# TUI-NICR/nicr-multitask-scene-analysis

Hardware: AMD Instinct MI355X
Metric: Mpix/s panoptic merge+metrics, 640x480xB (higher is better)
Workload: dtype f32; 1 GPU; configs[1]: center-NMS + offset grouping + panoptic merge + mIoU/PQ accumulators (configs[3]); batch_per_gpu=32, global_batch=32, classes=40, height=480, width=640, centers_per_image=24, batches_in_flight=2, parallelism=dp1 (images sharded, accumulators all-reduced once per run, timed)

## Files before the change

include/nmsa.h:

```cpp
#ifndef NMSA_H
#define NMSA_H

#include <stddef.h>
#include <stdint.h>

#ifdef __cplusplus
extern "C" {
#endif

typedef void* nmsa_stream_t;

enum {
    NMSA_OK = 0,
    NMSA_ERR_ARG = -1,
    NMSA_ERR_LAUNCH = -2,
    NMSA_ERR_WORKSPACE = -3,
    NMSA_ERR_UNSUPPORTED = -4
};

enum { NMSA_F32 = 0, NMSA_BF16 = 1, NMSA_F16 = 2 };
enum { NMSA_U8 = 0, NMSA_I16 = 1, NMSA_I32 = 2, NMSA_I64 = 3 };
#define NMSA_ELEM_F32 8

#define NMSA_MAX_INSTANCE_IDS 256

int nmsa_version(void);
const char* nmsa_strerror(int code);
int nmsa_last_hip_error(void);
int nmsa_device_geometry(int* cus_host, int* xcds_host, size_t* lds_per_cu_host);

size_t nmsa_center_nms_workspace_bytes(int B, int H, int W);
int nmsa_center_nms_topk(const float* center, const uint8_t* fg,
                         int B, int H, int W,
                         float threshold, int ksize, int topk, int apply_fg,
                         int max_centers,
                         int32_t* centers_yx, int32_t* n_centers, float* scores,
                         uint8_t* center_mask,
                         void* workspace, size_t workspace_bytes,
                         nmsa_stream_t stream);

int nmsa_group_offsets(const float* offset, const uint8_t* fg,
                       const int32_t* centers_yx, const int32_t* n_centers,
                       int B, int H, int W, int max_centers,
                       float scale_y, float scale_x,
                       int use_dist_thr, float dist_thr,
                       uint8_t* inst, int32_t* area,
                       nmsa_stream_t stream);

int nmsa_semantic_argmax(const void* logits, int logits_dtype,
                         int B, int C, int H, int W,
                         uint8_t* idx_u8, int64_t* idx_i64, float* score,
                         nmsa_stream_t stream);

int nmsa_semantic_softmax(const void* logits, int logits_dtype,
                          int B, int C, int H, int W, float* probs,
                          nmsa_stream_t stream);

int nmsa_panoptic_fused(const void* logits, int logits_dtype, const float* offset,
                        const int32_t* centers_yx, const int32_t* n_centers,
                        const uint8_t* is_thing,
                        int B, int C, int H, int W, int max_centers,
                        float scale_y, float scale_x,
                        int use_dist_thr, float dist_thr,
                        uint8_t* sem_u8, uint8_t* inst, uint8_t* fg_out, float* score,
                        uint32_t* votes, int votes_are_zero, int vote_rows_hint,
                        nmsa_stream_t stream);

int nmsa_panoptic_assign(uint32_t* votes, int B, int n_vote_classes, int clear_votes,
                         int64_t max_instances_per_category, int64_t void_label,
                         int64_t* pan_of_inst, int32_t* area,
                         int64_t* ids_pan, int64_t* ids_ins, int32_t* n_ids,
                         nmsa_stream_t stream);

int nmsa_panoptic_paint(const uint8_t* sem_u8, const uint8_t* inst,
                        const int64_t* pan_of_inst, const uint8_t* is_thing,
                        int B, int C, int H, int W,
                        int64_t max_instances_per_category, int64_t void_label,
                        int64_t* pan, int64_t* pan_sem,
                        nmsa_stream_t stream);

int nmsa_panoptic_merge(const void* sem, int sem_dtype, const void* ins, int ins_dtype,
                        const uint8_t* thing_seg, const uint8_t* is_thing_class,
                        int B, int n_classes, int H, int W,
                        int64_t max_instances_per_category, int64_t void_label,
                        uint32_t* votes, int64_t* pan_of_inst,
                        int64_t* pan, int64_t* ids_pan, int64_t* ids_ins, int32_t* n_ids,
                        nmsa_stream_t stream);

size_t nmsa_panoptic_merge_wide_workspace_bytes(int B, int n_classes, int max_segments);
int nmsa_panoptic_merge_wide(const void* sem, int sem_dtype, const void* ins, int ins_dtype,
                             const uint8_t* thing_seg, const uint8_t* is_thing_class,
                             int B, int n_classes, int H, int W,
                             int64_t max_instances_per_category, int64_t void_label,
                             int max_segments,
                             int64_t* pan, int64_t* ids_pan, int64_t* ids_ins, int32_t* n_ids,
                             int32_t* status, void* workspace, size_t workspace_bytes,
                             nmsa_stream_t stream);

int nmsa_resize_nearest(const void* src, int elem_type, int planes, int Hs, int Ws,
                        int y0, int x0, int h, int w, int Ho, int Wo, void* dst,
                        nmsa_stream_t stream);
int nmsa_resize_bilinear(const void* src, int dtype, int planes, int Hs, int Ws,
                         int y0, int x0, int h, int w, int Ho, int Wo, void* dst,
                         nmsa_stream_t stream);

int nmsa_semantic_argmax_resized(const void* logits, int logits_dtype, int B, int C,
                                 int Hs, int Ws, int y0, int x0, int h, int w, int Ho, int Wo,
                                 uint8_t* idx_u8, int64_t* idx_i64, float* score,
                                 nmsa_stream_t stream);

size_t nmsa_panoptic_scores_workspace_bytes(int B);
int nmsa_panoptic_scores(const void* logits, int logits_dtype,
                         const uint8_t* sem_idx, const float* sem_prob,
                         const uint8_t* inst, const int64_t* pan,
                         const int64_t* pan_of_inst, const float* inst_score_tab,
                         int B, int C, int H, int W, int64_t max_instances_per_category,
                         float* out_semantic_score, float* out_instance_score,
                         float* out_panoptic_score, float* mean_semantic_score,
                         void* workspace, size_t workspace_bytes, nmsa_stream_t stream);

int nmsa_instance_orientation(const float* orientation, const uint8_t* inst,
                              const uint8_t* mask, int B, int H, int W,
                              double* sums, int32_t* count, nmsa_stream_t stream);
int nmsa_instance_orientation_wide(const float* orientation, const void* instance, int ins_dtype,
                                   const uint8_t* mask, int B, int H, int W, int max_instances,
                                   int32_t* ids, int32_t* n_ids, double* sums, int32_t* count,
                                   int32_t* status, void* workspace, size_t workspace_bytes,
                                   nmsa_stream_t stream);

#define NMSA_TG_ROUTE_SCAN 1
#define NMSA_TG_ROUTE_FAST_LOADERS 2
#define NMSA_TG_ROUTE_PAINT_TILED 4
#define NMSA_TG_ROUTE_PAINT_VECTOR 8
#define NMSA_TG_ROUTE_LUT_LDS 16
#define NMSA_TG_ROUTE_SCAN_16 32
size_t nmsa_targets_workspace_bytes(int B, int n_classes, int max_instances);
int nmsa_targets_route(const void* semantic, int sem_dtype, const void* instance, int ins_dtype,
                       int n_classes, int H, int W, int sigma, int max_instances,
                       const float* center, const void* offset, const uint8_t* foreground,
                       const uint8_t* center_mask, const void* workspace);
int nmsa_instance_clear_stuff(const void* semantic, int sem_dtype, void* instance, int ins_dtype,
                              const uint8_t* is_stuff_class, int n_classes, int64_t n_px,
                              nmsa_stream_t stream);
int nmsa_instance_targets(const void* semantic, int sem_dtype, const void* instance, int ins_dtype,
                          const uint8_t* is_thing_class, const uint8_t* is_stuff_class,
                          int B, int n_classes, int H, int W,
                          int sigma, const float* gauss_lut, int normalized_offset, int max_instances,
                          float* center, void* offset, uint8_t* foreground, uint8_t* center_mask,
                          int32_t* encoded_ids, int32_t* n_encoded,
                          int32_t* skipped_ids, int32_t* n_skipped,
                          int32_t* status, void* workspace, size_t workspace_bytes, int workspace_is_clean,
                          nmsa_stream_t stream);
int nmsa_panoptic_targets(const void* semantic, int sem_dtype, const void* instance, int ins_dtype,
                          const uint8_t* is_thing_class, int B, int n_classes, int H, int W,
                          int64_t max_instances_per_category, int64_t void_label,
                          int max_instances, int max_segments,
                          int64_t* panoptic, int64_t* ids_pan, int64_t* ids_ins, int32_t* n_ids,
                          int32_t* status, void* workspace, size_t workspace_bytes, int workspace_is_clean,
                          nmsa_stream_t stream);
int nmsa_orientation_targets(const void* semantic, int sem_dtype, const void* instance, int ins_dtype,
                             const uint8_t* estimate_class, const int32_t* keys, const int32_t* n_keys,
                             const float* biternion, int B, int n_classes, int H, int W, int K,
                             int max_instances,
                             float* orientation, uint8_t* foreground, uint8_t* present,
                             int32_t* status, void* workspace, size_t workspace_bytes, int workspace_is_clean,
                             nmsa_stream_t stream);
int nmsa_dve_targets(const int64_t* panoptic, const int64_t* keys, const int32_t* n_keys,
                     const float* embeddings, const float* image_embedding, float diff_factor,
                     int B, int K, int D, int H, int W,
                     float* lut, int32_t* indices, nmsa_stream_t stream);

#define NMSA_ST_TABLE_OVERFLOW 1
#define NMSA_ST_CATEGORY_RANGE 2
#define NMSA_ST_MISSING_KEY 4
#define NMSA_ST_VALUE_RANGE 8
#define NMSA_ST_SENTINEL_KEY 16
size_t nmsa_confmat_workspace_bytes(int n_classes);
int nmsa_confmat_update(const void* preds, int pred_dtype, int64_t pred_div,
                        const void* target, int target_dtype,
                        int64_t n_px, int n_classes, int mode,
                        int64_t* confmat, int32_t* status,
                        void* workspace, size_t workspace_bytes, nmsa_stream_t stream);

size_t nmsa_pq_workspace_bytes(int B, int H, int W, int num_categories);
int nmsa_pq_update(const int64_t* pred, const int64_t* target, int B, int H, int W,
                   int num_categories, int64_t ignored_label,
                   int64_t max_instances_per_category, int64_t offset,
                   int64_t void_segment_id,
                   double* iou_per_class, double* tp_per_class,
                   double* fn_per_class, double* fp_per_class,
                   int64_t* matches, int match_capacity, int32_t* n_matches,
                   int32_t* status, void* workspace, size_t workspace_bytes,
                   int workspace_is_clean, nmsa_stream_t stream);

int nmsa_pack_tables(const int32_t* n_centers, const int32_t* n_ids,
                     const int32_t* centers_yx, const float* scores,
                     const int32_t* area, const int64_t* ids_pan, const int64_t* ids_ins,
                     int B, int max_centers, int columns, double* out, nmsa_stream_t stream);

size_t nmsa_pq_confmat_workspace_bytes(int B, int H, int W, int n_classes);
int nmsa_pq_update_with_confmat(
    const int64_t* pred, const int64_t* target, const uint8_t* target_semantic,
    int B, int H, int W,
    int num_categories, int64_t ignored_label, int64_t max_instances_per_category, int64_t offset,
    int64_t void_segment_id,
    double* iou_per_class, double* tp_per_class, double* fn_per_class, double* fp_per_class,
    int64_t* matches, int match_capacity, int32_t* n_matches,
    int32_t* status, void* workspace, size_t workspace_bytes, int workspace_is_clean,
    int confmat_classes, int64_t pred_div, int64_t* confmat, int32_t* confmat_status,
    void* confmat_workspace, size_t confmat_workspace_bytes, nmsa_stream_t stream);
int nmsa_pq_update_with_confmat_parts(
    const uint8_t* pred_semantic, const uint8_t* pred_instance, const int64_t* pan_of_inst,
    const uint8_t* is_thing_class, int n_sem_classes, int64_t void_label,
    const int64_t* target, const uint8_t* target_semantic,
    int B, int H, int W,
    int num_categories, int64_t ignored_label, int64_t max_instances_per_category, int64_t offset,
    int64_t void_segment_id,
    double* iou_per_class, double* tp_per_class, double* fn_per_class, double* fp_per_class,
    int32_t* status, void* workspace, size_t workspace_bytes, int workspace_is_clean,
    int confmat_classes, int64_t pred_div, int64_t* confmat, int32_t* confmat_status,
    void* confmat_workspace, size_t confmat_workspace_bytes, nmsa_stream_t stream);

size_t nmsa_loss_workspace_bytes(int B, int H, int W);
int nmsa_loss_ce_fwd(const void* logits, int dtype, const uint8_t* target, const float* weights,
                     int B, int C, int H, int W, float label_smoothing,
                     double* loss_sum, int64_t* n_elements, double* weight_sum, float* lse2_out,
                     int32_t* status, void* workspace, size_t workspace_bytes, nmsa_stream_t stream);
int nmsa_loss_ce_bwd(const void* logits, int dtype, const uint8_t* target, const float* weights,
                     int B, int C, int H, int W, float label_smoothing,
                     const float* grad_scale, const float* lse2, void* grad_logits,
                     nmsa_stream_t stream);
int nmsa_loss_ce_fwd_i16(const void* logits, int dtype, const int16_t* target,
                         const float* weights, int B, int C, int H, int W,
                         float label_smoothing,
                         double* loss_sum, int64_t* n_elements, double* weight_sum,
                         float* lse2_out,
                         int32_t* status, void* workspace, size_t workspace_bytes,
                         nmsa_stream_t stream);
int nmsa_loss_ce_bwd_i16(const void* logits, int dtype, const int16_t* target,
                         const float* weights, int B, int C, int H, int W,
                         float label_smoothing, const float* grad_scale, const float* lse2,
                         void* grad_logits, nmsa_stream_t stream);
int nmsa_loss_ce_fwd_grad_supported(int dtype, int C);
int nmsa_loss_ce_fwd_grad(const void* logits, int dtype, const uint8_t* target, const float* weights,
                          int B, int C, int H, int W, float label_smoothing,
                          const float* expected_grad_scale,
                          double* loss_sum, int64_t* n_elements, double* weight_sum,
                          void* grad_logits, int32_t* status,
                          void* workspace, size_t workspace_bytes, nmsa_stream_t stream);
int nmsa_loss_ce_bwd_unless(const void* logits, int dtype, const uint8_t* target,
                            const float* weights, int B, int C, int H, int W,
                            float label_smoothing, const float* grad_scale, void* grad_logits,
                            const float* computed_for, int32_t* counters, nmsa_stream_t stream);
size_t nmsa_count_workspace_bytes(void);
int nmsa_count_u8(const uint8_t* values, int64_t n, int lo, int hi, int64_t* count,
                  float* mean_scale, float weight,
                  void* workspace, size_t workspace_bytes, nmsa_stream_t stream);
int nmsa_loss_masked_fwd(const void* pred, int dtype, const float* target, const uint8_t* mask,
                         int B, int C, int H, int W, int kind,
                         double* loss_sum, int64_t* n_mask,
                         void* workspace, size_t workspace_bytes, nmsa_stream_t stream);
int nmsa_loss_masked_bwd(const void* pred, int dtype, const float* target, const uint8_t* mask,
                         int B, int C, int H, int W, int kind,
                         const float* grad_scale, void* grad_pred, nmsa_stream_t stream);
int nmsa_loss_masked_fwd_grad(const void* pred, int dtype, const float* target,
                              const uint8_t* mask, int B, int C, int H, int W, int kind,
                              const float* expected_grad_scale,
                              double* loss_sum, int64_t* n_mask, void* grad_pred,
                              void* workspace, size_t workspace_bytes, nmsa_stream_t stream);
int nmsa_loss_masked_bwd_unless(const void* pred, int dtype, const float* target,
                                const uint8_t* mask, int B, int C, int H, int W, int kind,
                                const float* grad_scale, void* grad_pred,
                                const float* computed_for, int32_t* counters, nmsa_stream_t stream);
int nmsa_loss_vonmises_fwd(const void* pred, int dtype, const float* target, const uint8_t* mask,
                           int B, int H, int W, float kappa,
                           double* loss_sum, int64_t* n_rows,
                           void* workspace, size_t workspace_bytes, nmsa_stream_t stream);
int nmsa_loss_vonmises_bwd(const void* pred, int dtype, const float* target, const uint8_t* mask,
                           int B, int H, int W, float kappa,
                           const float* grad_scale, void* grad_pred, nmsa_stream_t stream);
int nmsa_loss_vonmises_fwd_grad(const void* pred, int dtype, const float* target,
                                const uint8_t* mask, int B, int H, int W, float kappa,
                                const float* expected_grad_scale,
                                double* loss_sum, int64_t* n_rows, void* grad_pred,
                                void* workspace, size_t workspace_bytes, nmsa_stream_t stream);
int nmsa_loss_vonmises_bwd_unless(const void* pred, int dtype, const float* target,
                                  const uint8_t* mask, int B, int H, int W, float kappa,
                                  const float* grad_scale, void* grad_pred,
                                  const float* computed_for, int32_t* counters,
                                  nmsa_stream_t stream);
int nmsa_loss_cos_emb_fwd(const void* pred, int dtype, const int32_t* indices, const float* lut,
                          int B, int D, int H, int W, int L,
                          double* loss_sum, int64_t* n_rows, float* dots_out, int32_t* status,
                          void* workspace, size_t workspace_bytes, nmsa_stream_t stream);
int nmsa_loss_cos_emb_bwd(const void* pred, int dtype, const int32_t* indices, const float* lut,
                          int B, int D, int H, int W, int L,
                          const float* grad_scale, const float* dots, void* grad_pred,
                          nmsa_stream_t stream);
int nmsa_loss_cos_emb_fwd_grad_supported(int dtype, int D, int H, int W, int L);
size_t nmsa_loss_cos_emb_fwd_grad_workspace_bytes(int B, int D, int H, int W, int L);
int nmsa_loss_cos_emb_fwd_grad(const void* pred, int dtype, const int32_t* indices, const float* lut,
                               int B, int D, int H, int W, int L, const float* expected_gscale,
                               double* loss_sum, int64_t* n_rows, void* grad_pred, int32_t* status,
                               void* workspace, size_t workspace_bytes, nmsa_stream_t stream);
int nmsa_loss_cos_emb_bwd_unless(const void* pred, int dtype, const int32_t* indices, const float* lut,
                                 int B, int D, int H, int W, int L, const float* grad_scale,
                                 void* grad_pred, const float* computed_for, int32_t* counters,
                                 void* workspace, size_t workspace_bytes, nmsa_stream_t stream);
int nmsa_loss_cos_emb_can_keep_dots(int D, int H, int W, int L);

int nmsa_loss_elementwise_none_fwd(const void* pred, int dtype, const float* target, int64_t n,
                                   int kind, int out_dtype, void* out, nmsa_stream_t stream);
int nmsa_loss_elementwise_none_bwd(const void* pred, int dtype, const float* target, int64_t n,
                                   int kind, int upstream_dtype, const void* upstream,
                                   void* grad_pred, nmsa_stream_t stream);
int nmsa_loss_cos_rows_fwd(const void* input, int dtype, const float* target, const float* labels,
                           int64_t n_rows, int D, float margin, float* loss_rows,
                           nmsa_stream_t stream);
int nmsa_loss_cos_rows_bwd(const void* input, int dtype, const float* target, const float* labels,
                           int64_t n_rows, int D, float margin, const float* upstream,
                           int upstream_is_scalar, void* grad_input, nmsa_stream_t stream);
int nmsa_loss_vonmises_rows_fwd(const void* input, int dtype, const float* target, int64_t n_rows,
                                float kappa, float* loss_rows, nmsa_stream_t stream);
int nmsa_loss_vonmises_rows_bwd(const void* input, int dtype, const float* target, int64_t n_rows,
                                float kappa, const float* upstream, void* grad_input,
                                nmsa_stream_t stream);

enum { NMSA_LOSS_CE = 0, NMSA_LOSS_MSE = 1, NMSA_LOSS_L1 = 2, NMSA_LOSS_FOCAL = 3, NMSA_LOSS_VONMISES = 4,
       NMSA_LOSS_COS_EMB = 5 };
#define NMSA_MULTI_MAX_ITEMS 16
#define NMSA_MULTI_MAX_TOTALS 8
typedef struct nmsa_loss_item {
    int32_t kind, dtype, B, C, H, W;
    int32_t total;
    int32_t clamp_count;
    float param;
    int32_t reserved;
    const void* pred;
    const void* target;
    const void* mask;
    const float* weights;
    void* grad;
} nmsa_loss_item;
size_t nmsa_multitask_loss_workspace_bytes(const nmsa_loss_item* items_host, int n_items);
int nmsa_multitask_loss_fwd_grad(const nmsa_loss_item* items_host, int n_items, int n_totals,
                                 int32_t* spec, float* expect, double* loss_sums, int64_t* counts,
                                 double* aux, float* out_f32, int32_t* status, void* workspace,
                                 size_t workspace_bytes, nmsa_stream_t stream);
int nmsa_multitask_loss_bwd_unless(const nmsa_loss_item* items_host, int n_items, int n_totals,
                                   const float* grad_sums, const float* grad_item_losses,
                                   const float* grad_total_losses, const int64_t* counts,
                                   const float* expect, int32_t* spec, float* grad_scales,
                                   int32_t* counters, void* workspace, size_t workspace_bytes,
                                   nmsa_stream_t stream);

#define NMSA_DVE_ROUTE_AUTO 0
#define NMSA_DVE_ROUTE_GENERIC 1
#define NMSA_DVE_KERNEL_GENERIC 0
int nmsa_dve_project_route(const float* emb, int B, int D, int H, int W,
                           const float* weight_a, int Ca, const float* logits_a,
                           const float* weight_b, int Cb, const float* logits_b, int route);
int nmsa_dve_project(float* emb, int B, int D, int H, int W,
                     const float* weight_a, int Ca, float* logits_a,
                     const float* weight_b, int Cb, float* logits_b,
                     int route, nmsa_stream_t stream);

#define NMSA_RMSE_MASK_NONE 0
#define NMSA_RMSE_MASK_GIVEN 1
#define NMSA_RMSE_MASK_FROM_TARGET 2
// ... 139 lines not shown
```

nicr_mt_scene_analysis_amd/_lib.py:

```python
import ctypes as C
import os
import re
import subprocess
from typing import Optional

import torch

_HERE = os.path.dirname(os.path.abspath(__file__))
CSRC_DIR = os.path.join(_HERE, 'csrc')
LIB_PATH = os.environ.get('NMSA_LIB_PATH') or os.path.join(CSRC_DIR, 'libnmsa_hip.so')
HEADER_PATH = os.path.join(os.path.dirname(_HERE), 'include', 'nmsa.h')

NMSA_F32, NMSA_BF16, NMSA_F16 = 0, 1, 2
NMSA_U8, NMSA_I16, NMSA_I32, NMSA_I64 = 0, 1, 2, 3
NMSA_ST_VALUE_RANGE = 8
NMSA_SCENE_MAX_CLASSES = 4096
(NMSA_TG_ROUTE_SCAN, NMSA_TG_ROUTE_FAST_LOADERS, NMSA_TG_ROUTE_PAINT_TILED, NMSA_TG_ROUTE_PAINT_VECTOR,
 NMSA_TG_ROUTE_LUT_LDS, NMSA_TG_ROUTE_SCAN_16) = 1, 2, 4, 8, 16, 32
NMSA_UP_ROUTE_VECTOR, NMSA_UP_ROUTE_PIXEL = 1, 2
NMSA_LNT_ROUTE_VECTOR, NMSA_LNT_ROUTE_ELEMENT = 1, 2
NMSA_LNT_MAX_CHANNELS = 2048
NMSA_PPM_MAX_BINS = 4
NMSA_PPM_NEAREST, NMSA_PPM_BILINEAR = 0, 1
NMSA_PPM_ROUTE_LDS, NMSA_PPM_ROUTE_GLOBAL = 1, 2
NMSA_MLPDEC_MAX_BRANCHES = 4
NMSA_MLPDEC_NEAREST, NMSA_MLPDEC_BILINEAR = 0, 1
NMSA_MLPDEC_ROUTE_VECTOR, NMSA_MLPDEC_ROUTE_ELEMENT = 1, 2


class NmsaError(RuntimeError):
    pass


def build(force: bool = False) -> str:
    args = ['make', '-C', CSRC_DIR, '-j4']
    if force:
        args.append('-B')
    subprocess.check_call(args, stdout=subprocess.DEVNULL)
    return LIB_PATH


def declared_symbols():
    with open(HEADER_PATH) as f:
        text = f.read()
    text = re.sub(r'/\*.*?\*/', '', text, flags=re.S)
    return sorted(set(re.findall(r'\b(nmsa_[a-z0-9_]+)\s*\(', text)))


_vp, _i, _f, _i64, _sz = C.c_void_p, C.c_int, C.c_float, C.c_int64, C.c_size_t

_SIGNATURES = {
    'nmsa_version': (C.c_int, []),
    'nmsa_strerror': (C.c_char_p, [_i]),
    'nmsa_last_hip_error': (C.c_int, []),
    'nmsa_device_geometry': (_i, [_vp, _vp, _vp]),
    'nmsa_center_nms_workspace_bytes': (_sz, [_i, _i, _i]),
    'nmsa_center_nms_topk': (_i, [_vp, _vp, _i, _i, _i, _f, _i, _i, _i, _i,
                                  _vp, _vp, _vp, _vp, _vp, _sz, _vp]),
    'nmsa_group_offsets': (_i, [_vp, _vp, _vp, _vp, _i, _i, _i, _i, _f, _f, _i, _f,
                                _vp, _vp, _vp]),
    'nmsa_semantic_argmax': (_i, [_vp, _i, _i, _i, _i, _i, _vp, _vp, _vp, _vp]),
    'nmsa_semantic_softmax': (_i, [_vp, _i, _i, _i, _i, _i, _vp, _vp]),
    'nmsa_panoptic_fused': (_i, [_vp, _i, _vp, _vp, _vp, _vp, _i, _i, _i, _i, _i,
                                 _f, _f, _i, _f, _vp, _vp, _vp, _vp, _vp, _i, _i, _vp]),
    'nmsa_panoptic_assign': (_i, [_vp, _i, _i, _i, _i64, _i64, _vp, _vp, _vp, _vp, _vp, _vp]),
    'nmsa_panoptic_paint': (_i, [_vp, _vp, _vp, _vp, _i, _i, _i, _i, _i64, _i64,
                                 _vp, _vp, _vp]),
    'nmsa_panoptic_merge': (_i, [_vp, _i, _vp, _i, _vp, _vp, _i, _i, _i, _i, _i64, _i64,
                                 _vp, _vp, _vp, _vp, _vp, _vp, _vp]),
    'nmsa_panoptic_merge_wide_workspace_bytes': (_sz, [_i, _i, _i]),
    'nmsa_panoptic_merge_wide': (_i, [_vp, _i, _vp, _i, _vp, _vp, _i, _i, _i, _i, _i64, _i64, _i,
                                      _vp, _vp, _vp, _vp, _vp, _vp, _sz, _vp]),
    'nmsa_resize_nearest': (_i, [_vp, _i, _i, _i, _i, _i, _i, _i, _i, _i, _i, _vp, _vp]),
    'nmsa_resize_bilinear': (_i, [_vp, _i, _i, _i, _i, _i, _i, _i, _i, _i, _i, _vp, _vp]),
    'nmsa_semantic_argmax_resized': (_i, [_vp, _i, _i, _i, _i, _i, _i, _i, _i, _i, _i, _i,
                                          _vp, _vp, _vp, _vp]),
    'nmsa_panoptic_scores_workspace_bytes': (_sz, [_i]),
    'nmsa_panoptic_scores': (_i, [_vp, _i, _vp, _vp, _vp, _vp, _vp, _vp, _i, _i, _i, _i, _i64,
                                  _vp, _vp, _vp, _vp, _vp, _sz, _vp]),
    'nmsa_targets_workspace_bytes': (_sz, [_i, _i, _i]),
    'nmsa_targets_route': (_i, [_vp, _i, _vp, _i, _i, _i, _i, _i, _i, _vp, _vp, _vp, _vp, _vp]),
    'nmsa_instance_clear_stuff': (_i, [_vp, _i, _vp, _i, _vp, _i, _i64, _vp]),
    'nmsa_instance_targets': (_i, [_vp, _i, _vp, _i, _vp, _vp, _i, _i, _i, _i, _i, _vp, _i, _i,
                                   _vp, _vp, _vp, _vp, _vp, _vp, _vp, _vp, _vp, _vp, _sz, _i, _vp]),
    'nmsa_panoptic_targets': (_i, [_vp, _i, _vp, _i, _vp, _i, _i, _i, _i, _i64, _i64, _i, _i,
                                   _vp, _vp, _vp, _vp, _vp, _vp, _sz, _i, _vp]),
    'nmsa_orientation_targets': (_i, [_vp, _i, _vp, _i, _vp, _vp, _vp, _vp, _i, _i, _i, _i, _i, _i,
                                      _vp, _vp, _vp, _vp, _vp, _sz, _i, _vp]),
    'nmsa_dve_targets': (_i, [_vp, _vp, _vp, _vp, _vp, _f, _i, _i, _i, _i, _i, _vp, _vp, _vp]),
    'nmsa_dve_project': (_i, [_vp, _i, _i, _i, _i, _vp, _i, _vp, _vp, _i, _vp, _i, _vp]),
    'nmsa_dve_project_route': (_i, [_vp, _i, _i, _i, _i, _vp, _i, _vp, _vp, _i, _vp, _i]),
    'nmsa_normal_valid_mask': (_i, [_vp, _i, _i, _i, _vp, _vp]),
    'nmsa_rmse_update': (_i, [_vp, _i, _vp, _vp, _i, _i, _i, _i, _i, _i, _i, _i, _i, _i, _i,
                              _vp, _vp, _vp]),
    'nmsa_maae_update_keyed': (_i, [_vp, _vp, _vp, _vp, _i, _vp, _vp, _vp, _vp, _vp, _i, _vp,
                                    _i, _vp, _vp, _vp, _vp]),
    'nmsa_maae_update_matched': (_i, [_vp, _vp, _i, _vp, _vp, _vp, _i, _i, _vp, _vp, _vp, _vp, _i, _vp,
                                      _vp, _vp, _vp, _i, _i, _vp, _vp, _vp, _vp, _i, _vp,
                                      _i, _vp, _vp, _vp, _vp]),
    'nmsa_multiscale_nearest': (_i, [_vp, _vp, _i, _i, _vp]),
    'nmsa_batch_augment': (_i, [_vp, _vp, _i, _i, _i, _vp]),
    'nmsa_scene_step': (_i, [_vp, _i, _vp, _i, _i, _i, _vp, _f, _vp, _vp, _vp, _vp, _vp, _vp, _vp]),
    'nmsa_upsample2x_dw3x3_route': (_i, [_vp, _vp, _i, _i, _i, _i, _i]),
    'nmsa_upsample2x_dw3x3_fwd': (_i, [_vp, _i, _vp, _vp, _i, _i, _i, _i, _i, _vp, _vp]),
    'nmsa_upsample2x_dw3x3_bwd_workspace_bytes': (_sz, [_i, _i, _i, _i]),
    'nmsa_upsample2x_dw3x3_bwd': (_i, [_vp, _vp, _i, _vp, _i, _i, _i, _i, _i, _vp, _vp, _vp, _vp, _sz, _vp]),
    'nmsa_ln_nhwc_nchw_route': (_i, [_vp, _vp, _i, _i, _i, _i, _i]),
    'nmsa_ln_nhwc_nchw_fwd': (_i, [_vp, _i, _vp, _vp, _f, _vp, _i, _i, _i, _vp, _i, _vp, _vp, _vp]),
    'nmsa_ln_nhwc_nchw_bwd_workspace_bytes': (_sz, [_i, _i, _i]),
    'nmsa_ln_nhwc_nchw_bwd': (_i, [_vp, _i, _vp, _i, _vp, _vp, _vp, _i, _i, _i, _vp, _vp, _vp, _vp, _sz, _vp]),
    'nmsa_ppm_route': (_i, [_i, _i, _i, _vp, _vp]),
    'nmsa_ppm_pool_fwd': (_i, [_vp, _i, _i, _i, _i, _i, _i, _vp, _vp, _vp, _vp]),
    'nmsa_ppm_pool_bwd': (_i, [_vp, _i, _i, _i, _i, _i, _i, _vp, _vp, _vp, _vp]),
    'nmsa_ppm_upcat_fwd': (_i, [_vp, _vp, _i, _i, _i, _i, _i, _i, _vp, _vp, _vp, _i, _vp, _vp]),
    'nmsa_ppm_upcat_bwd': (_i, [_vp, _i, _i, _i, _i, _i, _i, _vp, _vp, _vp, _i, _vp, _vp]),
    'nmsa_mlpdec_route': (_i, [_vp, _vp, _i, _i, _i, _i, _vp]),
    'nmsa_mlpdec_upcat_fwd': (_i, [_vp, _i, _i, _i, _i, _i, _vp, _vp, _i, _vp, _vp]),
    'nmsa_mlpdec_upcat_bwd': (_i, [_vp, _i, _i, _i, _i, _i, _vp, _vp, _i, _vp, _vp]),
    'nmsa_instance_orientation_wide': (_i, [_vp, _vp, _i, _vp, _i, _i, _i, _i, _vp, _vp, _vp, _vp,
                                            _vp, _vp, _sz, _vp]),
    'nmsa_instance_orientation': (_i, [_vp, _vp, _vp, _i, _i, _i, _vp, _vp, _vp]),
    'nmsa_confmat_workspace_bytes': (_sz, [_i]),
    'nmsa_confmat_update': (_i, [_vp, _i, _i64, _vp, _i, _i64, _i, _i, _vp, _vp, _vp, _sz, _vp]),
    'nmsa_pq_confmat_workspace_bytes': (_sz, [_i, _i, _i, _i]),
    'nmsa_pq_update_with_confmat': (_i, [_vp, _vp, _vp, _i, _i, _i, _i, _i64, _i64, _i64, _i64,
                                         _vp, _vp, _vp, _vp, _vp, _i, _vp, _vp, _vp, _sz, _i,
                                         _i, _i64, _vp, _vp, _vp, _sz, _vp]),
    'nmsa_pq_update_with_confmat_parts': (_i, [_vp, _vp, _vp, _vp, _i, _i64, _vp, _vp, _i, _i, _i,
                                               _i, _i64, _i64, _i64, _i64, _vp, _vp, _vp, _vp,
                                               _vp, _vp, _sz, _i, _i, _i64, _vp, _vp, _vp, _sz, _vp]),
    'nmsa_pack_tables': (_i, [_vp, _vp, _vp, _vp, _vp, _vp, _vp, _i, _i, _i, _vp, _vp]),
    'nmsa_loss_workspace_bytes': (_sz, [_i, _i, _i]),
    'nmsa_loss_ce_fwd': (_i, [_vp, _i, _vp, _vp, _i, _i, _i, _i, _f, _vp, _vp, _vp, _vp, _vp, _vp, _sz,
                              _vp]),
    'nmsa_loss_ce_bwd': (_i, [_vp, _i, _vp, _vp, _i, _i, _i, _i, _f, _vp, _vp, _vp, _vp]),
    'nmsa_loss_ce_fwd_i16': (_i, [_vp, _i, _vp, _vp, _i, _i, _i, _i, _f, _vp, _vp, _vp, _vp, _vp, _vp, _sz,
                                  _vp]),
    'nmsa_loss_ce_bwd_i16': (_i, [_vp, _i, _vp, _vp, _i, _i, _i, _i, _f, _vp, _vp, _vp, _vp]),
    'nmsa_loss_masked_fwd': (_i, [_vp, _i, _vp, _vp, _i, _i, _i, _i, _i, _vp, _vp, _vp, _sz, _vp]),
    'nmsa_loss_masked_bwd': (_i, [_vp, _i, _vp, _vp, _i, _i, _i, _i, _i, _vp, _vp, _vp]),
    'nmsa_loss_vonmises_fwd': (_i, [_vp, _i, _vp, _vp, _i, _i, _i, _f, _vp, _vp, _vp, _sz, _vp]),
    'nmsa_loss_vonmises_bwd': (_i, [_vp, _i, _vp, _vp, _i, _i, _i, _f, _vp, _vp, _vp]),
    'nmsa_loss_ce_fwd_grad_supported': (_i, [_i, _i]),
    'nmsa_loss_ce_fwd_grad': (_i, [_vp, _i, _vp, _vp, _i, _i, _i, _i, _f, _vp, _vp, _vp, _vp, _vp, _vp,
                                   _vp, _sz, _vp]),
    'nmsa_loss_ce_bwd_unless': (_i, [_vp, _i, _vp, _vp, _i, _i, _i, _i, _f, _vp, _vp, _vp, _vp, _vp]),
    'nmsa_count_workspace_bytes': (_sz, []),
    'nmsa_count_u8': (_i, [_vp, _i64, _i, _i, _vp, _vp, _f, _vp, _sz, _vp]),
    'nmsa_loss_cos_emb_fwd_grad_supported': (_i, [_i, _i, _i, _i, _i]),
    'nmsa_loss_cos_emb_fwd_grad_workspace_bytes': (_sz, [_i, _i, _i, _i, _i]),
    'nmsa_loss_cos_emb_fwd_grad': (_i, [_vp, _i, _vp, _vp, _i, _i, _i, _i, _i, _vp, _vp, _vp, _vp, _vp, _vp, _sz, _vp]),
    'nmsa_loss_cos_emb_bwd_unless': (_i, [_vp, _i, _vp, _vp, _i, _i, _i, _i, _i, _vp, _vp, _vp, _vp, _vp, _sz, _vp]),
    'nmsa_multitask_loss_workspace_bytes': (_sz, [_vp, _i]),
    'nmsa_multitask_loss_fwd_grad': (_i, [_vp, _i, _i, _vp, _vp, _vp, _vp, _vp, _vp, _vp, _vp, _sz, _vp]),
    'nmsa_multitask_loss_bwd_unless': (_i, [_vp, _i, _i, _vp, _vp, _vp, _vp, _vp, _vp, _vp, _vp, _vp, _sz, _vp]),
    'nmsa_loss_masked_fwd_grad': (_i, [_vp, _i, _vp, _vp, _i, _i, _i, _i, _i, _vp, _vp, _vp, _vp, _vp,
                                       _sz, _vp]),
    'nmsa_loss_masked_bwd_unless': (_i, [_vp, _i, _vp, _vp, _i, _i, _i, _i, _i, _vp, _vp, _vp, _vp,
                                         _vp]),
    'nmsa_loss_vonmises_fwd_grad': (_i, [_vp, _i, _vp, _vp, _i, _i, _i, _f, _vp, _vp, _vp, _vp, _vp,
                                         _sz, _vp]),
    'nmsa_loss_vonmises_bwd_unless': (_i, [_vp, _i, _vp, _vp, _i, _i, _i, _f, _vp, _vp, _vp, _vp, _vp]),
    'nmsa_loss_cos_emb_fwd': (_i, [_vp, _i, _vp, _vp, _i, _i, _i, _i, _i, _vp, _vp, _vp, _vp, _vp, _sz, _vp]),
    'nmsa_loss_cos_emb_bwd': (_i, [_vp, _i, _vp, _vp, _i, _i, _i, _i, _i, _vp, _vp, _vp, _vp]),
    'nmsa_loss_cos_emb_can_keep_dots': (_i, [_i, _i, _i, _i]),
    'nmsa_loss_elementwise_none_fwd': (_i, [_vp, _i, _vp, _i64, _i, _i, _vp, _vp]),
    'nmsa_loss_elementwise_none_bwd': (_i, [_vp, _i, _vp, _i64, _i, _i, _vp, _vp, _vp]),
    'nmsa_loss_cos_rows_fwd': (_i, [_vp, _i, _vp, _vp, _i64, _i, _f, _vp, _vp]),
    'nmsa_loss_cos_rows_bwd': (_i, [_vp, _i, _vp, _vp, _i64, _i, _f, _vp, _i, _vp, _vp]),
    'nmsa_loss_vonmises_rows_fwd': (_i, [_vp, _i, _vp, _i64, _f, _vp, _vp]),
    'nmsa_loss_vonmises_rows_bwd': (_i, [_vp, _i, _vp, _i64, _f, _vp, _vp, _vp]),
    'nmsa_pq_workspace_bytes': (_sz, [_i, _i, _i, _i]),
    'nmsa_pq_update': (_i, [_vp, _vp, _i, _i, _i, _i, _i64, _i64, _i64, _i64,
                            _vp, _vp, _vp, _vp, _vp, _i, _vp, _vp, _vp, _sz, _i, _vp]),
}

_lib = None


def lib():
    global _lib
    if _lib is None:
        if not os.path.exists(LIB_PATH):
            raise NmsaError(
                f'{LIB_PATH} is missing: the HIP extension was not built. Run '
                '`python -c "import __graft_entry__ as g; g.build()"` '
                '(or `make -C nicr_mt_scene_analysis_amd/csrc`). There is no '
                'CPU/PyTorch fallback for this path.')
        handle = C.CDLL(LIB_PATH)
        for name, (res, args) in _SIGNATURES.items():
            fn = getattr(handle, name)
            fn.restype = res
            fn.argtypes = args
        _lib = handle
    return _lib


def check(rc: int, what: str) -> None:
    if rc != 0:
        l_ = lib()
        msg = l_.nmsa_strerror(rc).decode()
        hip = l_.nmsa_last_hip_error()
        raise NmsaError(f'{what}: {msg} (code {rc}, hipError {hip})')


def device_geometry():
    cus, xcds, lds = C.c_int(0), C.c_int(0), C.c_size_t(0)
    check(lib().nmsa_device_geometry(C.byref(cus), C.byref(xcds), C.byref(lds)), 'nmsa_device_geometry')
    return cus.value, xcds.value, lds.value


def ptr(t: Optional[torch.Tensor]):
    if t is None:
        return None
    if not t.is_cuda and not t.is_pinned():
        raise ValueError(f'the C-ABI takes device (or pinned host) memory; got a pageable '
                         f'{t.device} tensor of shape {tuple(t.shape)}')
    return C.c_void_p(t.data_ptr())


def stream_ptr(device) -> C.c_void_p:
    return C.c_void_p(torch.cuda.current_stream(device).cuda_stream)


def float_dtype_code(t: torch.Tensor) -> int:
    if t.dtype == torch.float32:
        return NMSA_F32
    if t.dtype == torch.bfloat16:
        return NMSA_BF16
    if t.dtype == torch.float16:
        return NMSA_F16
    raise TypeError(f'unsupported floating dtype {t.dtype}')


def int_dtype_code(t: torch.Tensor) -> int:
    if t.dtype in (torch.uint8, torch.bool):
        return NMSA_U8
    if t.dtype == torch.int16:
        return NMSA_I16
    if t.dtype == torch.int32:
        return NMSA_I32
    if t.dtype == torch.int64:
        return NMSA_I64
    raise TypeError(f'unsupported integer dtype {t.dtype}')


def require_device_tensor(t: torch.Tensor, name: str) -> torch.Tensor:
    if not t.is_cuda:
        raise NmsaError(
            f'{name} is on {t.device}: the HIP path needs tensors on the MI355X '
            '(there is no CPU fallback).')
    return t.contiguous()
```

nicr_mt_scene_analysis_amd/csrc/argmax_state.hpp:

```cpp
#pragma once
#include "nmsa_common.hpp"

namespace nmsa {

struct ArgmaxState {
    float m[4];
    int am[4];
    float se[4];
    float nf[4];
};

__device__ __forceinline__ void argmax_init(ArgmaxState& s)
{
#pragma unroll
    for (int j = 0; j < 4; ++j) { s.m[j] = -INFINITY; s.am[j] = 0; s.se[j] = 0.f; s.nf[j] = 0.f; }
}

template <bool WITH_SCORE>
__device__ __forceinline__ void argmax_step(ArgmaxState& s, int j, float v, int c)
{
    s.nf[j] = fmaf(v, 0.0f, s.nf[j]);
    if (WITH_SCORE) {
        const float e = (v == -INFINITY) ? 0.f : __expf(-fabsf(v - s.m[j]));
        s.se[j] = (v > s.m[j]) ? fmaf(s.se[j], e, 1.0f) : (s.se[j] + e);
    }
    const bool above = v > s.m[j];
    s.am[j] = above ? c : s.am[j];
    s.m[j] = above ? v : s.m[j];
}

__device__ __forceinline__ void argmax_group4_score(ArgmaxState& s, int j, const float v[4], int c0)
{
    constexpr float kLog2e = 1.4426950408889634f;
    const float gm = fmaxf(fmaxf(v[0], v[1]), fmaxf(v[2], v[3]));
    const float nm = fmaxf(s.m[j], gm);
    const float rescale = __builtin_amdgcn_exp2f((s.m[j] - nm) * kLog2e);
    float e = 0.f;
#pragma unroll
    for (int i = 0; i < 4; ++i) e += __builtin_amdgcn_exp2f((v[i] - nm) * kLog2e);
    s.se[j] = fmaf(s.se[j], rescale, e);
    const int first = (v[0] == gm) ? 0 : (v[1] == gm) ? 1 : (v[2] == gm) ? 2 : 3;
    s.am[j] = (gm > s.m[j]) ? c0 + first : s.am[j];
    s.m[j] = nm;
}

__device__ __forceinline__ float aten_vec_expf(float d)
{
    if (!(d >= -104.0f)) return 0.0f;
    const float q = rintf(__fmul_rn(d, 1.442695040888963407359924681001892137426645954152985934135449406931f));
    float s = __fmaf_rn(q, -0.693145751953125f, d);
    s = __fmaf_rn(q, -1.428606765330187045e-06f, s);
    float u = 0.000198527617612853646278381f;
    u = __fmaf_rn(u, s, 0.00139304355252534151077271f);
    u = __fmaf_rn(u, s, 0.00833336077630519866943359f);
    u = __fmaf_rn(u, s, 0.0416664853692054748535156f);
    u = __fmaf_rn(u, s, 0.166666671633720397949219f);
    u = __fmaf_rn(u, s, 0.5f);
    u = __fadd_rn(__fmaf_rn(__fmul_rn(s, s), u, s), 1.0f);
    const int qi = (int)q, qh = qi >> 1;
    u = __fmul_rn(__fmul_rn(u, __int_as_float((qh + 127) << 23)), __int_as_float((qi - qh + 127) << 23));
    return u;
}

constexpr float TIE_CANDIDATE_GAP = -0x1p-23f;

template <typename LD>
__device__ __forceinline__ int class_by_probability(LD ld, int C, float m, int am, int first_candidate,
                                                    float* p_max)
{
    float S = 0.f;
    for (int c = 0; c < C; ++c) S = __fadd_rn(S, aten_vec_expf(__fsub_rn(ld(c), m)));
    const float pm = __fdiv_rn(1.0f, S);
    if (p_max) *p_max = pm;
    for (int c = first_candidate; c < am; ++c) {
        const float d = __fsub_rn(ld(c), m);
        if (d >= TIE_CANDIDATE_GAP && __fdiv_rn(aten_vec_expf(d), S) == pm) return c;
    }
    return am;
}

template <int DTYPE>
__device__ __forceinline__ float tie_band_magnitude()
{
    return (DTYPE == NMSA_F32) ? 1.0f : (DTYPE == NMSA_BF16) ? 0x1p-16f : 0x1p-13f;
}

template <int DTYPE>
__device__ __forceinline__ bool may_tie_in_probability(float m)
{
    return fabsf(m) <= tie_band_magnitude<DTYPE>();
}

}
```

nicr_mt_scene_analysis_amd/csrc/panoptic.hip:

```cpp
#include <stdlib.h>
#include <type_traits>

#include "nmsa_common.hpp"
#include "argmax_state.hpp"

namespace nmsa {

constexpr int FUSED_THREADS = 256;
constexpr int FUSED_VOTE_SLOTS = 256;
constexpr int PX_PER_THREAD = 4;
constexpr int PX_PER_ITER = FUSED_THREADS * PX_PER_THREAD;

typedef float f32x4_t __attribute__((ext_vector_type(4)));
typedef unsigned short u16x4_t __attribute__((ext_vector_type(4)));

template <int DTYPE, bool VEC, bool NT = false>
__device__ __forceinline__ float4 load_px4(const void* base, size_t elem_off, int nvalid)
{
    float4 r = make_float4(0.f, 0.f, 0.f, 0.f);
    if (DTYPE == NMSA_F32) {
        const float* p = (const float*)base + elem_off;
        if (VEC && NT) {
            const f32x4_t v = __builtin_nontemporal_load((const f32x4_t*)p);
            return make_float4(v.x, v.y, v.z, v.w);
        }
        if (VEC) return *(const float4*)p;
        if (nvalid > 0) r.x = p[0];
        if (nvalid > 1) r.y = p[1];
        if (nvalid > 2) r.z = p[2];
        if (nvalid > 3) r.w = p[3];
        return r;
    } else {
        const uint16_t* p = (const uint16_t*)base + elem_off;
        uint16_t h[4] = {0, 0, 0, 0};
        if (VEC && NT) {
            const u16x4_t u = __builtin_nontemporal_load((const u16x4_t*)p);
            h[0] = u.x; h[1] = u.y; h[2] = u.z; h[3] = u.w;
        } else if (VEC) {
            const ushort4 u = *(const ushort4*)p;
            h[0] = u.x; h[1] = u.y; h[2] = u.z; h[3] = u.w;
        } else {
            for (int j = 0; j < 4; ++j) if (j < nvalid) h[j] = p[j];
        }
        if (DTYPE == NMSA_BF16) {
            r.x = bf16_to_f32(h[0]); r.y = bf16_to_f32(h[1]);
            r.z = bf16_to_f32(h[2]); r.w = bf16_to_f32(h[3]);
        } else {
            r.x = f16_to_f32(h[0]); r.y = f16_to_f32(h[1]);
            r.z = f16_to_f32(h[2]); r.w = f16_to_f32(h[3]);
        }
        return r;
    }
}

template <int DTYPE>
__device__ __noinline__ int column_class(const void* logits, size_t col0, int P, int C, float m)
{
    auto ld = [&](int c) -> float {
        if (DTYPE == NMSA_F32) return ((const float*)logits)[col0 + (size_t)c * P];
        const uint16_t h = ((const uint16_t*)logits)[col0 + (size_t)c * P];
        return (DTYPE == NMSA_BF16) ? bf16_to_f32(h) : f16_to_f32(h);
    };
    bool nan_or_pinf = false, any_finite = false;
    int first = C, am = C;
    int c = 0;
    for (; c + 4 <= C; c += 4) {
        float v[4];
#pragma unroll
        for (int u = 0; u < 4; ++u) v[u] = ld(c + u);
#pragma unroll
        for (int u = 0; u < 4; ++u) {
            nan_or_pinf |= (v[u] != v[u]) || (v[u] == INFINITY);
            any_finite |= fabsf(v[u]) < INFINITY;
            if (first == C && __fsub_rn(v[u], m) >= TIE_CANDIDATE_GAP) first = c + u;
            if (am == C && v[u] == m) am = c + u;
        }
    }
    for (; c < C; ++c) {
        const float v = ld(c);
        nan_or_pinf |= (v != v) || (v == INFINITY);
        any_finite |= fabsf(v) < INFINITY;
        if (first == C && __fsub_rn(v, m) >= TIE_CANDIDATE_GAP) first = c;
        if (am == C && v == m) am = c;
    }
    if (nan_or_pinf || !any_finite || am == C) return 0;
    if (first >= am) return am;
    return class_by_probability(ld, C, m, am, first, nullptr);
}

template <int DTYPE>
__device__ __noinline__ float2 column_exact(const void* logits, size_t col0, int P, int C)
{
    auto ld = [&](int c) -> float {
        if (DTYPE == NMSA_F32) return ((const float*)logits)[col0 + (size_t)c * P];
        const uint16_t h = ((const uint16_t*)logits)[col0 + (size_t)c * P];
        return (DTYPE == NMSA_BF16) ? bf16_to_f32(h) : f16_to_f32(h);
    };
    bool nan_or_pinf = false, any_finite = false;
    float m = -INFINITY;
    int am = 0;
    for (int c = 0; c < C; ++c) {
        const float v = ld(c);
        if (v != v || v == INFINITY) nan_or_pinf = true;
        if (fabsf(v) < INFINITY) any_finite = true;
        if (v > m) { m = v; am = c; }
    }
    if (nan_or_pinf || !any_finite) return make_float2(__int_as_float(0x7fc00000), __int_as_float(0));
    float se = 0.f;
    int first = am;
    for (int c = 0; c < C; ++c) {
        const float v = ld(c);
        se += (v == -INFINITY) ? 0.f : __expf(v - m);
        if (c < first && __fsub_rn(v, m) >= TIE_CANDIDATE_GAP) first = c;
    }
    if (first >= am) return make_float2(1.0f / se, __int_as_float(am));
    float pm;
    const int cls = class_by_probability(ld, C, m, am, first, &pm);
    return make_float2(pm, __int_as_float(cls));
}

template <bool WITH_SCORE>
__device__ __forceinline__ void argmax_quad(ArgmaxState& st, const float4& a, const float4& b,
                                            const float4& c, const float4& d, int c0,
                                            int nclasses = 4)
{
    if (WITH_SCORE) {
        const float p0[4] = {a.x, b.x, c.x, d.x}, p1[4] = {a.y, b.y, c.y, d.y};
        const float p2[4] = {a.z, b.z, c.z, d.z}, p3[4] = {a.w, b.w, c.w, d.w};
        argmax_group4_score(st, 0, p0, c0);
        argmax_group4_score(st, 1, p1, c0);
        argmax_group4_score(st, 2, p2, c0);
        argmax_group4_score(st, 3, p3, c0);
    } else {
        const float4 q[4] = {a, b, c, d};
#pragma unroll
        for (int u = 0; u < 4; ++u) {
            if (u >= nclasses) break;
            argmax_step<false>(st, 0, q[u].x, c0 + u);
            argmax_step<false>(st, 1, q[u].y, c0 + u);
            argmax_step<false>(st, 2, q[u].z, c0 + u);
            argmax_step<false>(st, 3, q[u].w, c0 + u);
        }
    }
}

__device__ __forceinline__ float sqdist(float cy, float cx, float ly, float lx)
{
    const float dy = __fsub_rn(cy, ly);
    const float dx = __fsub_rn(cx, lx);
    return __fmaf_rn(dx, dx, __fmul_rn(dy, dy));
}

__device__ __forceinline__ float sqrt_tie_upper(float d)
{
    if (!(d < INFINITY)) return d;
    const float dn = __uint_as_float(__float_as_uint(d) + 1u);
    const double m = 0.5 * ((double)d + (double)dn);
    const double m2 = m * m;
    float u = (float)m2;
    if ((double)u >= m2) u = __uint_as_float(__float_as_uint(u) - 1u);
    return u;
}

__device__ __forceinline__ float wave_all_min(float v)
{
#pragma unroll
    for (int o = 32; o > 0; o >>= 1) v = fminf(v, __shfl_xor(v, o));
    return v;
}

struct LdsCenters {
    const float2* cen;
    __device__ __forceinline__ float2 at(int i) const { return cen[i]; }
    __device__ __forceinline__ float2 of_lane(int n) const { return cen[min(lane_id(), n - 1)]; }
};
struct LaneCenters {
    float cy, cx;
    __device__ __forceinline__ float2 at(int i) const
    {
        return make_float2(__int_as_float(__builtin_amdgcn_readlane(__float_as_int(cy), i)),
                           __int_as_float(__builtin_amdgcn_readlane(__float_as_int(cx), i)));
    }
    __device__ __forceinline__ float2 of_lane(int) const { return make_float2(cy, cx); }
};

template <typename Centers>
__device__ __forceinline__ uint64_t wave_candidate_centers(const Centers& cen, int n,
                                                           const float ly[4], const float lx[4],
                                                           const bool act[4])
{
    float lo_y = INFINITY, lo_x = INFINITY, nhi_y = INFINITY, nhi_x = INFINITY;
    bool finite = true;
#pragma unroll
    for (int j = 0; j < 4; ++j) {
        if (act[j]) {
            finite = finite && (fabsf(ly[j]) < INFINITY) && (fabsf(lx[j]) < INFINITY);
            lo_y = fminf(lo_y, ly[j]);  nhi_y = fminf(nhi_y, -ly[j]);
            lo_x = fminf(lo_x, lx[j]);  nhi_x = fminf(nhi_x, -lx[j]);
        }
    }
    const uint64_t all = (n >= 64) ? ~0ull : ((1ull << n) - 1ull);
    if (__any(!finite)) return all;
    lo_y = wave_all_min(lo_y);  nhi_y = wave_all_min(nhi_y);
    lo_x = wave_all_min(lo_x);  nhi_x = wave_all_min(nhi_x);
    if (!(lo_y < INFINITY)) return 0ull;
    const float hi_y = -nhi_y, hi_x = -nhi_x;
    const int lane = lane_id();
    const float2 c = cen.of_lane(n);
    const float a0 = c.x - lo_y, a1 = hi_y - c.x;
    const float b0 = c.y - lo_x, b1 = hi_x - c.y;
    const float near_y = fmaxf(0.f, fmaxf(-a0, -a1)), near_x = fmaxf(0.f, fmaxf(-b0, -b1));
    const float far_y = fmaxf(fabsf(a0), fabsf(a1)), far_x = fmaxf(fabsf(b0), fabsf(b1));
    const float lo = near_y * near_y + near_x * near_x;
    const float hi = (lane < n) ? far_y * far_y + far_x * far_x : INFINITY;
    const float U = wave_all_min(hi);
    return __ballot(lane < n && lo <= U * 1.00001f) & all;
}

template <bool CULL = true, typename Centers = LdsCenters>
__device__ __forceinline__ void group4(const Centers& cen, int n,
                                       const float ly[4], const float lx[4],
                                       const bool act[4], int use_thr, float thr,
                                       uint32_t id[4])
{
    float smin[4], prev[4];
    int imin[4];
    const bool cull = CULL && n <= 64;
    uint64_t m = cull ? wave_candidate_centers(cen, n, ly, lx, act) : 0ull;
    int first = 0;
    if (cull) {
        if (m == 0ull) {
#pragma unroll
            for (int j = 0; j < 4; ++j) id[j] = 0u;
            return;
        }
        first = __ffsll((unsigned long long)m) - 1;
        m &= m - 1;
    }
    {
        const float2 c0 = cen.at(first);
#pragma unroll
        for (int j = 0; j < 4; ++j) {
            smin[j] = sqdist(c0.x, c0.y, ly[j], lx[j]);
            prev[j] = INFINITY;
            imin[j] = first;
        }
    }
    auto visit = [&](const int i) {
        const float2 c = cen.at(i);
#pragma unroll
        for (int j = 0; j < 4; ++j) {
            const float s = sqdist(c.x, c.y, ly[j], lx[j]);
            const bool upd = s < smin[j];
            prev[j] = upd ? smin[j] : prev[j];
            imin[j] = upd ? i : imin[j];
            smin[j] = upd ? s : smin[j];
        }
    };
    if (cull) {
        while (m) {
            const int i = __ffsll((unsigned long long)m) - 1;
            m &= m - 1;
            visit(i);
        }
    } else {
        for (int i = 1; i < n; ++i) visit(i);
    }
    bool maybe_tie = false;
#pragma unroll
    for (int j = 0; j < 4; ++j)
        maybe_tie = maybe_tie || (act[j] && !(prev[j] > fmaf(smin[j], 4.8e-7f, smin[j])));
    int best[4] = {imin[0], imin[1], imin[2], imin[3]};
    if (__any(maybe_tie)) {
        float U[4];
#pragma unroll
        for (int j = 0; j < 4; ++j) U[j] = sqrt_tie_upper(sqrtf(smin[j]));
        for (int i = n - 1; i >= 0; --i) {
            const float2 c = cen.at(i);
#pragma unroll
            for (int j = 0; j < 4; ++j)
                if (sqdist(c.x, c.y, ly[j], lx[j]) <= U[j]) best[j] = i;
        }
#pragma unroll
        for (int j = 0; j < 4; ++j) best[j] = (smin[j] != smin[j]) ? 0 : best[j];
    }
#pragma unroll
    for (int j = 0; j < 4; ++j) {
        uint32_t v = (uint32_t)(best[j] + 1) & 0xFFu;
        if (use_thr && sqrtf(smin[j]) > thr) v = 0;
        id[j] = act[j] ? v : 0u;
    }
}

template <int DTYPE, bool VEC, bool WITH_SCORE, int UNROLL = 8, bool NT = true,
          bool EARLY_OFFSETS = false, bool TILED = false, int TILE_LOG2W = 6>
__global__ __launch_bounds__(FUSED_THREADS) __attribute__((amdgpu_waves_per_eu(5, WITH_SCORE ? 8 : 5))) void k_panoptic_fused(
    const void* __restrict__ logits, const float* __restrict__ offset,
    const int32_t* __restrict__ centers_yx, const int32_t* __restrict__ n_centers,
    const uint8_t* __restrict__ is_thing,
    int C, int H, int W, int max_centers, int iters,
    float scale_y, float scale_x, int use_thr, float thr,
    uint8_t* __restrict__ sem_u8, uint8_t* __restrict__ inst, uint8_t* __restrict__ fg_out,
    float* __restrict__ score, uint32_t* __restrict__ votes, int ablate)
{
    extern __shared__ __align__(16) unsigned char smem[];
    float2* cen = (float2*)smem;
    int* vote_key = (int*)(cen + max_centers);
    uint32_t* vote_cnt = (uint32_t*)(vote_key + FUSED_VOTE_SLOTS);
    const int NC = C + 1;

    const int b = blockIdx.y;
    const int P = H * W;
    const int n = min(n_centers[b], max_centers);

    static_assert(FUSED_THREADS == 256, "one LUT entry per thread");
    static_assert(FUSED_VOTE_SLOTS == FUSED_THREADS, "one vote slot per thread");
    vote_key[threadIdx.x] = -1;
    vote_cnt[threadIdx.x] = 0;
    const bool lane_centers = n <= 64 && H <= 65535 && W <= 65535;
    uint32_t lane_cyx, thing_b = 0u;
    {
        const int2 c2 = *(const int2*)(centers_yx +
            ((size_t)b * max_centers + min(lane_id(), max_centers - 1)) * 2);
        lane_cyx = ((uint32_t)c2.x << 16) | ((uint32_t)c2.y & 0xFFFFu);
#pragma unroll
        for (int k = 0; k < 4; ++k)
            if (k * 64 < C)
                thing_b |= (is_thing[min(k * 64 + lane_id(), C - 1)] != 0 ? 1u : 0u) << k;
    }
    __syncthreads();

    const size_t img_logits = (size_t)b * C * P;
    const float* offy = offset + (size_t)b * 2 * P;
    const float* offx = offy + P;
    uint32_t* votes_b = votes + (size_t)b * 256 * NC;

    const int chunk_start = blockIdx.x * iters * PX_PER_ITER;
    auto chunk = [&](const int it, auto first_tag) {
        constexpr bool FIRST = decltype(first_tag)::value;
        int p0;
        bool active;
        if (TILED) {
            constexpr int TW = 1 << TILE_LOG2W, TH = 1024 >> TILE_LOG2W, LPR = TW / 4;
            const int tiles_x = (W + TW - 1) >> TILE_LOG2W;
            const int tile = blockIdx.x * iters + it;
            const int ty = tile / tiles_x, tx = tile - ty * tiles_x;
            const int row = ty * TH + (int)threadIdx.x / LPR;
            const int col = tx * TW + ((int)threadIdx.x % LPR) * 4;
            active = row < H && col < W;
            p0 = active ? row * W + col : 0;
        } else {
            p0 = chunk_start + it * PX_PER_ITER + threadIdx.x * PX_PER_THREAD;
            active = p0 < P;
        }
        const int nvalid = active ? min(4, P - p0) : 0;

        float4 oy = make_float4(0.f, 0.f, 0.f, 0.f), ox = oy;
        if (EARLY_OFFSETS && active) {
            oy = load_px4<NMSA_F32, VEC, NT>(offy, (size_t)p0, nvalid);
            ox = load_px4<NMSA_F32, VEC, NT>(offx, (size_t)p0, nvalid);
        }


        ArgmaxState st;
        argmax_init(st);
        if (active) {
            int c = 0;
            static_assert(UNROLL % 4 == 0, "class groups of 4");
            for (; c + UNROLL <= C; c += UNROLL) {
                float4 v[UNROLL];
#pragma unroll
                for (int u = 0; u < UNROLL; ++u)
                    v[u] = load_px4<DTYPE, VEC, NT>(logits, img_logits + (size_t)(c + u) * P + p0, nvalid);
#pragma unroll
                for (int u = 0; u < UNROLL; u += 4)
                    argmax_quad<WITH_SCORE>(st, v[u], v[u + 1], v[u + 2], v[u + 3], c + u);
            }
            for (; c < C; c += 4) {
                float4 v[4];
#pragma unroll
                for (int u = 0; u < 4; ++u)
                    v[u] = (c + u < C)
                        ? load_px4<DTYPE, VEC, NT>(logits, img_logits + (size_t)(c + u) * P + p0, nvalid)
                        : make_float4(-INFINITY, -INFINITY, -INFINITY, -INFINITY);
                argmax_quad<WITH_SCORE>(st, v[0], v[1], v[2], v[3], c, min(4, C - c));
            }
        }
        if (FIRST && !lane_centers) {
            for (int i = threadIdx.x; i < n; i += FUSED_THREADS) {
                const int2 c2 = *(const int2*)(centers_yx + ((size_t)b * max_centers + i) * 2);
                cen[i] = make_float2((float)c2.x, (float)c2.y);
            }
            __syncthreads();
        }
        uint64_t thing_m[4];
#pragma unroll
        for (int k = 0; k < 4; ++k)
            thing_m[k] = __ballot(((thing_b >> k) & 1u) != 0u && k * 64 + lane_id() < C);
        int cls[4];
        bool fg[4];
        bool any_fg = false;
#pragma unroll
        for (int j = 0; j < 4; ++j) {
            cls[j] = st.am[j];
            if (WITH_SCORE) {
                float sc = 1.0f / st.se[j];
                if ((st.se[j] != st.se[j] || may_tie_in_probability<DTYPE>(st.m[j])) && j < nvalid) {
                    const float2 ex = column_exact<DTYPE>(logits, img_logits + p0 + j, P, C);
                    sc = ex.x;
                    cls[j] = __float_as_int(ex.y);
                }
                st.se[j] = sc;
            } else if ((st.nf[j] != st.nf[j] || may_tie_in_probability<DTYPE>(st.m[j])) && j < nvalid) {
                cls[j] = column_class<DTYPE>(logits, img_logits + p0 + j, P, C, st.m[j]);
            }
            uint64_t tm = thing_m[0];
            if (C > 64) {
                const int q = cls[j] >> 6;
                tm = (q == 0) ? thing_m[0] : (q == 1) ? thing_m[1] : (q == 2) ? thing_m[2] : thing_m[3];
            }
            fg[j] = (j < nvalid) && ((tm >> (cls[j] & 63)) & 1ull);
            any_fg = any_fg || fg[j];
        }

        uint32_t id[4] = {0u, 0u, 0u, 0u};
        if (__any(any_fg) && n > 0) {
            if (!EARLY_OFFSETS && any_fg && !(ablate & 4)) {
                oy = load_px4<NMSA_F32, VEC, NT>(offy, (size_t)p0, nvalid);
                ox = load_px4<NMSA_F32, VEC, NT>(offx, (size_t)p0, nvalid);
            }
            const float oyv[4] = {oy.x, oy.y, oy.z, oy.w};
            const float oxv[4] = {ox.x, ox.y, ox.z, ox.w};
            float ly[4], lx[4];
            int y = p0 / W, x = p0 - y * W;
#pragma unroll
            for (int j = 0; j < 4; ++j) {
                ly[j] = __fadd_rn((float)y, __fmul_rn(oyv[j], scale_y));
                lx[j] = __fadd_rn((float)x, __fmul_rn(oxv[j], scale_x));
                if (++x == W) { x = 0; ++y; }
            }
            if (ablate & 2) {
#pragma unroll
                for (int j = 0; j < 4; ++j) id[j] = fg[j] ? 1u : 0u;
            } else if (lane_centers) {
                group4(LaneCenters{(float)(lane_cyx >> 16), (float)(lane_cyx & 0xFFFFu)}, n, ly, lx, fg,
                       use_thr, thr, id);
            } else {
                group4(LdsCenters{cen}, n, ly, lx, fg, use_thr, thr, id);
            }
        }

        if (VEC && active) {
            typedef unsigned char u8x4_t __attribute__((ext_vector_type(4)));
            const u8x4_t s4 = {(uint8_t)cls[0], (uint8_t)cls[1], (uint8_t)cls[2], (uint8_t)cls[3]};
            const u8x4_t i4 = {(uint8_t)id[0], (uint8_t)id[1], (uint8_t)id[2], (uint8_t)id[3]};
            const u8x4_t f4 = {(uint8_t)fg[0], (uint8_t)fg[1], (uint8_t)fg[2], (uint8_t)fg[3]};
            if (ablate & 8) {
                __builtin_nontemporal_store(s4, (u8x4_t*)(sem_u8 + (size_t)b * P + p0));
                __builtin_nontemporal_store(i4, (u8x4_t*)(inst + (size_t)b * P + p0));
                if (fg_out) __builtin_nontemporal_store(f4, (u8x4_t*)(fg_out + (size_t)b * P + p0));
            } else {
                *(u8x4_t*)(sem_u8 + (size_t)b * P + p0) = s4;
                *(u8x4_t*)(inst + (size_t)b * P + p0) = i4;
                if (fg_out) *(u8x4_t*)(fg_out + (size_t)b * P + p0) = f4;
            }
            if (WITH_SCORE)
                *(float4*)(score + (size_t)b * P + p0) =
                    make_float4(st.se[0], st.se[1], st.se[2], st.se[3]);
        } else {
            for (int j = 0; j < nvalid; ++j) {
                sem_u8[(size_t)b * P + p0 + j] = (uint8_t)cls[j];
                inst[(size_t)b * P + p0 + j] = (uint8_t)id[j];
                if (fg_out) fg_out[(size_t)b * P + p0 + j] = fg[j];
                if (WITH_SCORE) score[(size_t)b * P + p0 + j] = st.se[j];
            }
        }

        const bool wave_has_inst = __any((id[0] | id[1] | id[2] | id[3]) != 0u);
        if (wave_has_inst && !(ablate & 1)) {
            int key[4];
#pragma unroll
            for (int j = 0; j < 4; ++j)
                key[j] = (id[j] != 0u) ? (int)(id[j] * NC + cls[j] + 1) : -1;
            auto add = [&](int k, uint32_t cnt) {
                const int slot = lds_hash_slot(vote_key, FUSED_VOTE_SLOTS, k);
                if (slot >= 0) atomicAdd(&vote_cnt[slot], cnt);
                else atomicAdd(&votes_b[k], cnt);
            };
            const bool uniform = key[0] == key[1] && key[1] == key[2] && key[2] == key[3];
            int run_len, run_last;
            if (wave_run_head(uniform ? key[0] : -1, run_len, run_last))
                add(key[0], 4u * (uint32_t)run_len);
            if (!uniform) {
#pragma unroll
                for (int j = 0; j < 4; ++j)
                    if (key[j] >= 0) add(key[j], 1u);
            }
        }
    };
    chunk(0, std::true_type{});
    for (int it = 1; it < iters; ++it) chunk(it, std::false_type{});

    __syncthreads();
    {
        const int k = vote_key[threadIdx.x];
        if (k >= 0) atomicAdd(&votes_b[k], vote_cnt[threadIdx.x]);
    }
}

template <int DTYPE, bool VEC, bool WITH_SCORE>
__global__ __launch_bounds__(FUSED_THREADS) void k_semantic_argmax(
    const void* __restrict__ logits, int C, int P,
    uint8_t* __restrict__ idx_u8, int64_t* __restrict__ idx_i64, float* __restrict__ score)
{
    const int b = blockIdx.y;
    const int p0 = (blockIdx.x * FUSED_THREADS + threadIdx.x) * PX_PER_THREAD;
    if (p0 >= P) return;
    const int nvalid = min(4, P - p0);
    const size_t img = (size_t)b * C * P;
    ArgmaxState st;
    argmax_init(st);
    int c = 0;
    for (; c + 8 <= C; c += 8) {
        float4 v[8];
#pragma unroll
        for (int u = 0; u < 8; ++u)
            v[u] = load_px4<DTYPE, VEC, true>(logits, img + (size_t)(c + u) * P + p0, nvalid);
        argmax_quad<WITH_SCORE>(st, v[0], v[1], v[2], v[3], c);
        argmax_quad<WITH_SCORE>(st, v[4], v[5], v[6], v[7], c + 4);
    }
    for (; c < C; c += 4) {
        float4 v[4];
#pragma unroll
        for (int u = 0; u < 4; ++u)
            v[u] = (c + u < C) ? load_px4<DTYPE, VEC, true>(logits, img + (size_t)(c + u) * P + p0, nvalid)
                               : make_float4(-INFINITY, -INFINITY, -INFINITY, -INFINITY);
        argmax_quad<WITH_SCORE>(st, v[0], v[1], v[2], v[3], c, min(4, C - c));
    }
    int cls[4];
    float sc[4];
#pragma unroll
    for (int j = 0; j < 4; ++j) {
        cls[j] = st.am[j];
        sc[j] = 0.f;
        if (WITH_SCORE) {
            sc[j] = 1.0f / st.se[j];
            if ((st.se[j] != st.se[j] || may_tie_in_probability<DTYPE>(st.m[j])) && j < nvalid) {
                const float2 ex = column_exact<DTYPE>(logits, img + p0 + j, P, C);
                sc[j] = ex.x;
                cls[j] = __float_as_int(ex.y);
            }
        } else if ((st.nf[j] != st.nf[j] || may_tie_in_probability<DTYPE>(st.m[j])) && j < nvalid) {
            cls[j] = column_class<DTYPE>(logits, img + p0 + j, P, C, st.m[j]);
        }
    }
    const size_t o = (size_t)b * P + p0;
    if (VEC) {
        if (idx_u8)
            *(uchar4*)(idx_u8 + o) = make_uchar4((uint8_t)cls[0], (uint8_t)cls[1], (uint8_t)cls[2],
                                                 (uint8_t)cls[3]);
        if (idx_i64) {
            *(longlong2*)(idx_i64 + o) = make_longlong2(cls[0], cls[1]);
            *(longlong2*)(idx_i64 + o + 2) = make_longlong2(cls[2], cls[3]);
        }
        if (WITH_SCORE) *(float4*)(score + o) = make_float4(sc[0], sc[1], sc[2], sc[3]);
    } else {
        for (int j = 0; j < nvalid; ++j) {
            if (idx_u8) idx_u8[o + j] = (uint8_t)cls[j];
            if (idx_i64) idx_i64[o + j] = cls[j];
            if (WITH_SCORE) score[o + j] = sc[j];
        }
    }
}

__device__ __forceinline__ float max_nan(float m, float v)
{
    return (v != v) ? v : ((m != m) ? m : fmaxf(m, v));
}

template <int DTYPE>
__device__ __noinline__ void softmax_column_3pass(const void* logits, size_t col0, int P, int C,
                                                  float* probs)
{
    auto ld = [&](int c) -> float {
        if (DTYPE == NMSA_F32) return ((const float*)logits)[col0 + (size_t)c * P];
        const uint16_t h = ((const uint16_t*)logits)[col0 + (size_t)c * P];
        return (DTYPE == NMSA_BF16) ? bf16_to_f32(h) : f16_to_f32(h);
    };
    float m = -INFINITY, sum = 0.f;
    for (int c = 0; c < C; ++c) m = max_nan(m, ld(c));
    for (int c = 0; c < C; ++c) sum += __expf(ld(c) - m);
    for (int c = 0; c < C; ++c) probs[col0 + (size_t)c * P] = __expf(ld(c) - m) / sum;
}

template <int DTYPE, bool VEC>
__global__ __launch_bounds__(FUSED_THREADS) void k_semantic_softmax(
    const void* __restrict__ logits, int C, int P, float* __restrict__ probs)
{
    const int b = blockIdx.y;
    const int p0 = (blockIdx.x * FUSED_THREADS + threadIdx.x) * PX_PER_THREAD;
    if (p0 >= P) return;
    const int nvalid = min(4, P - p0);
    const size_t img = (size_t)b * C * P;
    float m[4] = {-INFINITY, -INFINITY, -INFINITY, -INFINITY};
    float sum[4] = {0.f, 0.f, 0.f, 0.f}, nf[4] = {0.f, 0.f, 0.f, 0.f};
    for (int c = 0; c < C; ++c) {
        const float4 v4 = load_px4<DTYPE, VEC>(logits, img + (size_t)c * P + p0, nvalid);
        const float v[4] = {v4.x, v4.y, v4.z, v4.w};
#pragma unroll
        for (int j = 0; j < 4; ++j) {
            nf[j] = fmaf(v[j], 0.0f, nf[j]);
            const float e = __expf(-fabsf(v[j] - m[j]));
            sum[j] = (v[j] > m[j]) ? fmaf(sum[j], e, 1.0f) : (sum[j] + e);
            m[j] = fmaxf(m[j], v[j]);
        }
    }
    float inv[4];
#pragma unroll
    for (int j = 0; j < 4; ++j) inv[j] = 1.0f / sum[j];
    for (int c = 0; c < C; ++c) {
        const float4 v4 = load_px4<DTYPE, VEC>(logits, img + (size_t)c * P + p0, nvalid);
        const float r[4] = {__expf(v4.x - m[0]) * inv[0], __expf(v4.y - m[1]) * inv[1],
                            __expf(v4.z - m[2]) * inv[2], __expf(v4.w - m[3]) * inv[3]};
        float* o = probs + img + (size_t)c * P + p0;
        if (VEC) {
            f32x4_t q; q.x = r[0]; q.y = r[1]; q.z = r[2]; q.w = r[3];
            __builtin_nontemporal_store(q, (f32x4_t*)o);
        } else {
            for (int j = 0; j < nvalid; ++j) o[j] = r[j];
        }
    }
    for (int j = 0; j < nvalid; ++j)
        if (nf[j] != nf[j]) softmax_column_3pass<DTYPE>(logits, img + p0 + j, P, C, probs);
}

template <int DTYPE, int CMAX>
__global__ __launch_bounds__(FUSED_THREADS) void k_semantic_softmax_reg(
    const void* __restrict__ logits, int C, int P, float* __restrict__ probs)
{
    const int b = blockIdx.y;
    const int p0 = (blockIdx.x * FUSED_THREADS + threadIdx.x) * PX_PER_THREAD;
    if (p0 >= P) return;
    const size_t img = (size_t)b * C * P;
    float4 v[CMAX];
#pragma unroll
    for (int c = 0; c < CMAX; ++c)
        if (c < C) v[c] = load_px4<DTYPE, true, true>(logits, img + (size_t)c * P + p0, 4);
    float m[4] = {-INFINITY, -INFINITY, -INFINITY, -INFINITY};
#pragma unroll
    for (int c = 0; c < CMAX; ++c)
        if (c < C) {
            m[0] = max_nan(m[0], v[c].x); m[1] = max_nan(m[1], v[c].y);
            m[2] = max_nan(m[2], v[c].z); m[3] = max_nan(m[3], v[c].w);
        }
    float sum[4] = {0.f, 0.f, 0.f, 0.f};
#pragma unroll
    for (int c = 0; c < CMAX; ++c)
        if (c < C) {
            v[c].x = __expf(v[c].x - m[0]); v[c].y = __expf(v[c].y - m[1]);
            v[c].z = __expf(v[c].z - m[2]); v[c].w = __expf(v[c].w - m[3]);
            sum[0] += v[c].x; sum[1] += v[c].y; sum[2] += v[c].z; sum[3] += v[c].w;
        }
#pragma unroll
    for (int c = 0; c < CMAX; ++c)
        if (c < C) {
            f32x4_t q;
            q.x = v[c].x / sum[0]; q.y = v[c].y / sum[1]; q.z = v[c].z / sum[2]; q.w = v[c].w / sum[3];
            __builtin_nontemporal_store(q, (f32x4_t*)(probs + img + (size_t)c * P + p0));
        }
}

template <bool VEC, bool TILED = false>
__global__ __launch_bounds__(FUSED_THREADS) void k_group_offsets(
    const float* __restrict__ offset, const uint8_t* __restrict__ fgmask,
    const int32_t* __restrict__ centers_yx, const int32_t* __restrict__ n_centers,
    int H, int W, int max_centers, int iters,
    float scale_y, float scale_x, int use_thr, float thr,
    uint8_t* __restrict__ inst, int32_t* __restrict__ area)
{
    extern __shared__ __align__(16) unsigned char smem[];
    float2* cen = (float2*)smem;
    uint32_t* ahist = (uint32_t*)(cen + max_centers);
    const int b = blockIdx.y;
    const int P = H * W;
    const int n = min(n_centers[b], max_centers);
    for (int i = threadIdx.x; i < n; i += FUSED_THREADS) {
        const int32_t cy = centers_yx[((size_t)b * max_centers + i) * 2 + 0];
        const int32_t cx = centers_yx[((size_t)b * max_centers + i) * 2 + 1];
        cen[i] = make_float2((float)cy, (float)cx);
    }
    for (int i = threadIdx.x; i < 256; i += FUSED_THREADS) ahist[i] = 0;
    __syncthreads();

    const float* offy = offset + (size_t)b * 2 * P;
    const float* offx = offy + P;
    const int chunk_start = blockIdx.x * iters * PX_PER_ITER;
    const int tiles_x = (W + 63) >> 6;
    for (int it = 0; it < iters; ++it) {
        int p0;
        bool active;
        if (TILED) {
            const int tile = blockIdx.x * iters + it;
            const int ty = tile / tiles_x, tx = tile - ty * tiles_x;
            const int row = ty * 16 + (int)(threadIdx.x >> 4);
            const int col = tx * 64 + (int)(threadIdx.x & 15) * 4;
            active = row < H && col < W;
            p0 = active ? row * W + col : 0;
        } else {
            p0 = chunk_start + it * PX_PER_ITER + threadIdx.x * PX_PER_THREAD;
            active = p0 < P;
        }
        const int nvalid = active ? min(4, P - p0) : 0;
        bool fg[4] = {false, false, false, false};
        if (VEC && active) {
            const uchar4 f = *(const uchar4*)(fgmask + (size_t)b * P + p0);
            fg[0] = f.x != 0; fg[1] = f.y != 0; fg[2] = f.z != 0; fg[3] = f.w != 0;
        } else {
            for (int j = 0; j < nvalid; ++j) fg[j] = fgmask[(size_t)b * P + p0 + j] != 0;
        }
        const bool any_fg = fg[0] || fg[1] || fg[2] || fg[3];
        uint32_t id[4] = {0u, 0u, 0u, 0u};
        if (__any(any_fg) && n > 0) {
            float4 oy = make_float4(0.f, 0.f, 0.f, 0.f), ox = oy;
            if (any_fg) {
                oy = load_px4<NMSA_F32, VEC, true>(offy, (size_t)p0, nvalid);
                ox = load_px4<NMSA_F32, VEC, true>(offx, (size_t)p0, nvalid);
            }
            const float oyv[4] = {oy.x, oy.y, oy.z, oy.w};
            const float oxv[4] = {ox.x, ox.y, ox.z, ox.w};
            float ly[4], lx[4];
            int y = p0 / W, x = p0 - y * W;
#pragma unroll
            for (int j = 0; j < 4; ++j) {
                ly[j] = __fadd_rn((float)y, __fmul_rn(oyv[j], scale_y));
                lx[j] = __fadd_rn((float)x, __fmul_rn(oxv[j], scale_x));
                if (++x == W) { x = 0; ++y; }
            }
            group4(LdsCenters{cen}, n, ly, lx, fg, use_thr, thr, id);
        }
        if (VEC && active) {
            *(uchar4*)(inst + (size_t)b * P + p0) =
                make_uchar4((uint8_t)id[0], (uint8_t)id[1], (uint8_t)id[2], (uint8_t)id[3]);
        } else {
            for (int j = 0; j < nvalid; ++j) inst[(size_t)b * P + p0 + j] = (uint8_t)id[j];
        }
        if (area && n > 0 && __any(any_fg)) {
            int key[4];
#pragma unroll
            for (int j = 0; j < 4; ++j) key[j] = fg[j] ? (int)id[j] : -1;
            const bool uniform = key[0] == key[1] && key[1] == key[2] && key[2] == key[3];
            int run_len, run_last;
            if (wave_run_head(uniform ? key[0] : -1, run_len, run_last))
                atomicAdd(&ahist[key[0]], 4u * (uint32_t)run_len);
            if (!uniform) {
#pragma unroll
                for (int j = 0; j < 4; ++j)
                    if (key[j] >= 0) atomicAdd(&ahist[key[j]], 1u);
            }
        }
    }
    if (area) {
        __syncthreads();
        for (int i = threadIdx.x; i < 256; i += FUSED_THREADS) {
            const uint32_t v = ahist[i];
            if (v) atomicAdd(&area[(size_t)b * 256 + i], (int32_t)v);
        }
    }
}

constexpr int ASSIGN_LDS_WORDS = 36 * 1024;
constexpr int ASSIGN_THREADS = 256;
__global__ __launch_bounds__(ASSIGN_THREADS) void k_assign(
    uint32_t* __restrict__ votes, int NC, int clear_votes, int64_t max_inst, int64_t void_label,
    int64_t* __restrict__ pan_of_inst, int32_t* __restrict__ area,
    int64_t* __restrict__ ids_pan, int64_t* __restrict__ ids_ins, int32_t* __restrict__ n_ids,
    int lds_words)
{
    extern __shared__ uint32_t s_rows[];
    __shared__ int s_vcls[256];
    __shared__ int s_wcnt[4];
    __shared__ uint32_t s_total[256];
    __shared__ int s_cls[256];
    const int b = blockIdx.x, t = threadIdx.x;
    uint32_t* tab = votes + (size_t)b * 256 * NC;
    const int rows_per_pass = max(1, min(256, lds_words / NC));
    for (int r0 = 0; r0 < 256; r0 += rows_per_pass) {
        const int nr = min(rows_per_pass, 256 - r0);
        const int nwords = nr * NC;
        uint32_t* src = tab + (size_t)r0 * NC;
        const int nquads = ((((uintptr_t)src) & 15) == 0) ? (nwords >> 2) : 0;
        for (int i0 = t; i0 < nquads; i0 += 8 * ASSIGN_THREADS) {
            uint4 v[8];
#pragma unroll
            for (int u = 0; u < 8; ++u) {
                const int i = i0 + u * ASSIGN_THREADS;
                v[u] = (i < nquads) ? ((const uint4*)src)[i] : make_uint4(0u, 0u, 0u, 0u);
            }
#pragma unroll
            for (int u = 0; u < 8; ++u) {
                const int i = i0 + u * ASSIGN_THREADS;
                if (i < nquads) {
                    s_rows[4 * i] = v[u].x; s_rows[4 * i + 1] = v[u].y;
                    s_rows[4 * i + 2] = v[u].z; s_rows[4 * i + 3] = v[u].w;
                    if (clear_votes && (v[u].x | v[u].y | v[u].z | v[u].w)) ((uint4*)src)[i] = make_uint4(0u, 0u, 0u, 0u);
                }
            }
        }
        for (int i = 4 * nquads + t; i < nwords; i += ASSIGN_THREADS) {
            const uint32_t v = src[i];
// ... 31 lines not shown
    const bool rowt = t < 256;
    const uint32_t total = rowt ? s_total[t] : 0u;
    const int cls = rowt ? s_cls[t] : 0;
    const bool valid = rowt && (t > 0) && (total > 0) && (cls != 0);
    const unsigned long long m = __ballot(valid);
    const int w = t >> 6, l = t & 63;
    if (l == 0 && w < 4) s_wcnt[w] = __popcll(m);
    __syncthreads();
    int pos = __popcll(m & ((1ull << l) - 1ull));
    for (int k = 0; k < min(w, 4); ++k) pos += s_wcnt[k];
    if (valid) s_vcls[pos] = cls;
    __syncthreads();
    int rank = 1;
    if (valid)
        for (int j = 0; j < pos; ++j) rank += (s_vcls[j] == cls);
    const int64_t pid = (int64_t)cls * max_inst + rank;
    if (rowt) pan_of_inst[(size_t)b * 256 + t] = valid ? pid : void_label;
    if (area && rowt) area[(size_t)b * 256 + t] = (t > 0) ? (int32_t)total : 0;
    if (valid) {
        ids_pan[(size_t)b * 256 + pos] = pid;
        ids_ins[(size_t)b * 256 + pos] = t;
    }
    if (t == 0) n_ids[b] = s_wcnt[0] + s_wcnt[1] + s_wcnt[2] + s_wcnt[3];
}

template <bool VEC>
__global__ __launch_bounds__(256) void k_paint(
    const uint8_t* __restrict__ sem_u8, const uint8_t* __restrict__ inst,
    const int64_t* __restrict__ pan_of_inst, const uint8_t* __restrict__ is_thing,
    int C, int P, int iters, int64_t max_inst, int64_t void_label,
    int64_t* __restrict__ pan, int64_t* __restrict__ pan_sem)
{
    __shared__ int64_t s_inst[256];
    __shared__ int64_t s_stuff[256];
    const int b = blockIdx.y, t = threadIdx.x;
    s_inst[t] = pan_of_inst[(size_t)b * 256 + t];
    s_stuff[t] = (t < C && !is_thing[t]) ? (int64_t)(t + 1) * max_inst : void_label;
    __syncthreads();
    for (int it = 0; it < iters; ++it) {
        const int p0 = ((blockIdx.x * iters + it) * 256 + t) * 8;
        if (p0 >= P) break;
        const size_t o = (size_t)b * P + p0;
        uint8_t s[8], in[8];
        const int nvalid = min(8, P - p0);
        if (VEC) {
            const uint2 sv = *(const uint2*)(sem_u8 + o);
            const uint2 iv = *(const uint2*)(inst + o);
#pragma unroll
            for (int j = 0; j < 4; ++j) {
                s[j] = (sv.x >> (8 * j)) & 0xFF; s[4 + j] = (sv.y >> (8 * j)) & 0xFF;
                in[j] = (iv.x >> (8 * j)) & 0xFF; in[4 + j] = (iv.y >> (8 * j)) & 0xFF;
            }
        } else {
            for (int j = 0; j < 8; ++j) {
                s[j] = (j < nvalid) ? sem_u8[o + j] : 0;
                in[j] = (j < nvalid) ? inst[o + j] : 0;
            }
        }
        int64_t r[8];
#pragma unroll
        for (int j = 0; j < 8; ++j) r[j] = in[j] ? s_inst[in[j]] : s_stuff[s[j]];
        if (VEC) {
#pragma unroll
            for (int j = 0; j < 8; j += 2)
                *(longlong2*)(pan + o + j) = make_longlong2(r[j], r[j + 1]);
            if (pan_sem) {
#pragma unroll
                for (int j = 0; j < 8; j += 2)
                    *(longlong2*)(pan_sem + o + j) = make_longlong2(r[j] / max_inst, r[j + 1] / max_inst);
            }
        } else {
            for (int j = 0; j < nvalid; ++j) {
                pan[o + j] = r[j];
                if (pan_sem) pan_sem[o + j] = r[j] / max_inst;
            }
        }
    }
}

__global__ __launch_bounds__(256) void k_paint2(
    const uint8_t* __restrict__ sem_u8, const uint8_t* __restrict__ inst,
    const int64_t* __restrict__ pan_of_inst, const uint8_t* __restrict__ is_thing,
    int C, int P, int steps, int64_t max_inst, int64_t void_label,
    int64_t* __restrict__ pan, int64_t* __restrict__ pan_sem)
{
    __shared__ int64_t s_inst[256];
    __shared__ int64_t s_stuff[256];
    const int b = blockIdx.y, t = threadIdx.x;
    s_inst[t] = pan_of_inst[(size_t)b * 256 + t];
    s_stuff[t] = (t < C && !is_thing[t]) ? (int64_t)(t + 1) * max_inst : void_label;
    __syncthreads();
    const int base = blockIdx.x * steps * 512;
    constexpr int U = 4;
    for (int k0 = 0; k0 < steps; k0 += U) {
        uint16_t sv[U], iv[U];
#pragma unroll
        for (int u = 0; u < U; ++u) {
            const int p0 = base + ((k0 + u) * 256 + t) * 2;
            const bool ok = (k0 + u) < steps && p0 < P;
            sv[u] = ok ? *(const uint16_t*)(sem_u8 + (size_t)b * P + p0) : 0;
            iv[u] = ok ? *(const uint16_t*)(inst + (size_t)b * P + p0) : 0;
        }
#pragma unroll
        for (int u = 0; u < U; ++u) {
            const int p0 = base + ((k0 + u) * 256 + t) * 2;
            if ((k0 + u) >= steps || p0 >= P) continue;
            const int i0 = iv[u] & 0xFF, i1 = iv[u] >> 8;
            const int64_t r0 = i0 ? s_inst[i0] : s_stuff[sv[u] & 0xFF];
            const int64_t r1 = i1 ? s_inst[i1] : s_stuff[sv[u] >> 8];
            *(longlong2*)(pan + (size_t)b * P + p0) = make_longlong2(r0, r1);
            if (pan_sem)
                *(longlong2*)(pan_sem + (size_t)b * P + p0) = make_longlong2(r0 / max_inst, r1 / max_inst);
        }
    }
}

__device__ __forceinline__ int64_t load_int(const void* p, int dtype, size_t i)
{
    switch (dtype) {
        case NMSA_U8: return ((const uint8_t*)p)[i];
        case NMSA_I16: return ((const int16_t*)p)[i];
        case NMSA_I32: return ((const int32_t*)p)[i];
        default: return ((const int64_t*)p)[i];
    }
}

template <bool VEC>
__device__ __forceinline__ void load_int4(const void* p, int dtype, size_t o, int nvalid, int64_t out[4])
{
    if (VEC) {
        switch (dtype) {
            case NMSA_U8: {
                const uchar4 v = *(const uchar4*)((const uint8_t*)p + o);
                out[0] = v.x; out[1] = v.y; out[2] = v.z; out[3] = v.w;
                return;
            }
            case NMSA_I16: {
                const short4 v = *(const short4*)((const int16_t*)p + o);
                out[0] = v.x; out[1] = v.y; out[2] = v.z; out[3] = v.w;
                return;
            }
            case NMSA_I32: {
                const int4 v = *(const int4*)((const int32_t*)p + o);
                out[0] = v.x; out[1] = v.y; out[2] = v.z; out[3] = v.w;
                return;
            }
            default: {
                const longlong2 a = *(const longlong2*)((const int64_t*)p + o);
                const longlong2 c = *(const longlong2*)((const int64_t*)p + o + 2);
                out[0] = a.x; out[1] = a.y; out[2] = c.x; out[3] = c.y;
                return;
            }
        }
    }
#pragma unroll
    for (int j = 0; j < 4; ++j) out[j] = (j < nvalid) ? load_int(p, dtype, o + j) : 0;
}

constexpr int MG_PX_PER_BLOCK = 256 * 4;

template <bool VEC>
__global__ __launch_bounds__(256) void k_merge_votes(
    const void* __restrict__ sem, int sem_dtype, const void* __restrict__ ins, int ins_dtype,
    const uint8_t* __restrict__ thing_seg, int NC, int P, uint32_t* __restrict__ votes)
{
    __shared__ int s_key[256];
    __shared__ uint32_t s_cnt[256];
    const int b = blockIdx.y;
    uint32_t* votes_b = votes + (size_t)b * 256 * NC;
    s_key[threadIdx.x] = -1;
    s_cnt[threadIdx.x] = 0;
    __syncthreads();
    auto add = [&](int kk, uint32_t cnt) {
        const int slot = lds_hash_slot(s_key, 256, kk);
        if (slot >= 0) atomicAdd(&s_cnt[slot], cnt);
        else atomicAdd(&votes_b[kk], cnt);
    };
    for (int p0 = (blockIdx.x * 256 + threadIdx.x) * 4; p0 - (int)threadIdx.x * 4 < P;
         p0 += gridDim.x * MG_PX_PER_BLOCK) {
        int key[4] = {-1, -1, -1, -1};
        if (p0 < P) {
            const int nvalid = min(4, P - p0);
            const size_t o = (size_t)b * P + p0;
            int64_t i4[4], s4[4], t4[4];
            load_int4<VEC>(ins, ins_dtype, o, nvalid, i4);
            load_int4<VEC>(sem, sem_dtype, o, nvalid, s4);
            load_int4<VEC>(thing_seg, NMSA_U8, o, nvalid, t4);
#pragma unroll
            for (int j = 0; j < 4; ++j)
                if (j < nvalid && i4[j] > 0 && i4[j] < 256 && t4[j] && s4[j] >= 0 && s4[j] < NC)
                    key[j] = (int)(i4[j] * NC + s4[j]);
        }
        const bool same4 = key[0] == key[1] && key[1] == key[2] && key[2] == key[3];
        int run_len, run_last;
        if (wave_run_head(same4 ? key[0] : -1, run_len, run_last)) add(key[0], 4u * (uint32_t)run_len);
        if (!same4) {
#pragma unroll
            for (int j = 0; j < 4; ++j) if (key[j] >= 0) add(key[j], 1u);
        }
    }
    __syncthreads();
    if (s_key[threadIdx.x] >= 0 && s_cnt[threadIdx.x])
        atomicAdd(&votes_b[s_key[threadIdx.x]], s_cnt[threadIdx.x]);
}

template <bool VEC>
__global__ __launch_bounds__(256) void k_merge_paint(
    const void* __restrict__ sem, int sem_dtype, const void* __restrict__ ins, int ins_dtype,
    const uint8_t* __restrict__ thing_seg, const uint8_t* __restrict__ is_thing_class,
    const int64_t* __restrict__ pan_of_inst, int NC, int P,
    int64_t max_inst, int64_t void_label, int64_t* __restrict__ pan)
{
    __shared__ int64_t s_inst[256];
    const int b = blockIdx.y;
    s_inst[threadIdx.x] = pan_of_inst[(size_t)b * 256 + threadIdx.x];
    __syncthreads();
    for (int p0 = (blockIdx.x * 256 + threadIdx.x) * 4; p0 < P; p0 += gridDim.x * MG_PX_PER_BLOCK) {
        const int nvalid = min(4, P - p0);
        const size_t o = (size_t)b * P + p0;
        int64_t i4[4], s4[4], t4[4], r[4];
        load_int4<VEC>(ins, ins_dtype, o, nvalid, i4);
        load_int4<VEC>(sem, sem_dtype, o, nvalid, s4);
        load_int4<VEC>(thing_seg, NMSA_U8, o, nvalid, t4);
#pragma unroll
        for (int j = 0; j < 4; ++j) {
            r[j] = void_label;
            if (i4[j] != 0) {
                if (i4[j] > 0 && i4[j] < 256 && t4[j]) r[j] = s_inst[i4[j]];
            } else if (s4[j] > 0 && s4[j] < NC && !is_thing_class[s4[j]]) {
                r[j] = s4[j] * max_inst;
            }
        }
        if (VEC) {
            *(longlong2*)(pan + o) = make_longlong2(r[0], r[1]);
            *(longlong2*)(pan + o + 2) = make_longlong2(r[2], r[3]);
        } else {
            for (int j = 0; j < nvalid; ++j) pan[o + j] = r[j];
        }
    }
}

template <bool VEC>
__global__ __launch_bounds__(256) void k_orientation_sums(
    const float* __restrict__ orientation, const uint8_t* __restrict__ inst,
    const uint8_t* __restrict__ mask, int P, double* __restrict__ sums, int32_t* __restrict__ count)
{
    __shared__ double s_sum[256 * 2];
    __shared__ int s_cnt[256];
    const int b = blockIdx.y;
    for (int i = threadIdx.x; i < 512; i += 256) s_sum[i] = 0.0;
    s_cnt[threadIdx.x] = 0;
    __syncthreads();
    const float* o0 = orientation + (size_t)b * 2 * P;
    const float* o1 = o0 + P;
    for (int p0 = (blockIdx.x * 256 + threadIdx.x) * 4; p0 - (int)threadIdx.x * 4 < P;
         p0 += gridDim.x * MG_PX_PER_BLOCK) {
        int id[4] = {0, 0, 0, 0};
        float a[4] = {0.f, 0.f, 0.f, 0.f}, c[4] = {0.f, 0.f, 0.f, 0.f};
        if (p0 < P) {
            const int nvalid = min(4, P - p0);
            const size_t o = (size_t)b * P + p0;
            int64_t i4[4], m4[4] = {1, 1, 1, 1};
            load_int4<VEC>(inst, NMSA_U8, o, nvalid, i4);
            if (mask) load_int4<VEC>(mask, NMSA_U8, o, nvalid, m4);
            if (VEC) {
                const float4 x = *(const float4*)(o0 + p0), y = *(const float4*)(o1 + p0);
                a[0] = x.x; a[1] = x.y; a[2] = x.z; a[3] = x.w;
                c[0] = y.x; c[1] = y.y; c[2] = y.z; c[3] = y.w;
            } else {
                for (int j = 0; j < nvalid; ++j) { a[j] = o0[p0 + j]; c[j] = o1[p0 + j]; }
            }
#pragma unroll
            for (int j = 0; j < 4; ++j) id[j] = (j < nvalid && m4[j]) ? (int)i4[j] : 0;
        }
        const bool same4 = id[0] == id[1] && id[1] == id[2] && id[2] == id[3];
        const int lid = same4 ? id[0] : 0;
        const double l0 = (double)a[0] + (double)a[1] + (double)a[2] + (double)a[3];
        const double l1 = (double)c[0] + (double)c[1] + (double)c[2] + (double)c[3];
        if (lid) {
            atomicAdd(&s_sum[lid * 2 + 0], l0);
            atomicAdd(&s_sum[lid * 2 + 1], l1);
        }
        int run_len, run_last;
        if (wave_run_head(lid ? lid : -1, run_len, run_last)) atomicAdd(&s_cnt[lid], 4 * run_len);
        if (!same4) {
#pragma unroll
            for (int j = 0; j < 4; ++j) {
                if (!id[j]) continue;
                atomicAdd(&s_sum[id[j] * 2 + 0], (double)a[j]);
                atomicAdd(&s_sum[id[j] * 2 + 1], (double)c[j]);
                atomicAdd(&s_cnt[id[j]], 1);
            }
        }
    }
    __syncthreads();
    const int t = threadIdx.x;
    if (s_cnt[t]) {
        atomicAdd(&sums[((size_t)b * 256 + t) * 2 + 0], s_sum[t * 2 + 0]);
        atomicAdd(&sums[((size_t)b * 256 + t) * 2 + 1], s_sum[t * 2 + 1]);
        atomicAdd(&count[(size_t)b * 256 + t], s_cnt[t]);
    }
}

}

using namespace nmsa;

namespace {

int env_int(const char* name, int dflt)
{
    const char* v = getenv(name);
    return v ? atoi(v) : dflt;
}

constexpr int ASSIGN_LDS_WORDS_SMALL = 12 * 1024;
int assign_lds_words(int NC)
{
    int words = ASSIGN_LDS_WORDS;
    if ((size_t)256 * NC * sizeof(uint32_t) > 48 * 1024 &&
        allow_dynamic_lds(k_assign, ASSIGN_LDS_WORDS * sizeof(uint32_t)) != NMSA_OK)
        words = ASSIGN_LDS_WORDS_SMALL;
    return words;
}
size_t assign_lds_bytes(int NC, int words)
{
    int rows = words / NC;
    rows = rows > 256 ? 256 : (rows < 1 ? 1 : rows);
    return (size_t)rows * NC * sizeof(uint32_t);
}

int fused_iters(int P)
{
    (void)P;
    static const int it = env_int("NMSA_FUSED_ITERS", 1);
    return it > 0 ? it : 1;
}

template <int DTYPE>
int launch_fused(const void* logits, const float* offset, const int32_t* centers_yx,
                 const int32_t* n_centers, const uint8_t* is_thing,
                 int B, int C, int H, int W, int max_centers,
                 float sy, float sx, int use_thr, float thr,
                 uint8_t* sem_u8, uint8_t* inst, uint8_t* fg_out, float* score,
                 uint32_t* votes, int vote_rows_hint, hipStream_t stream)
{
    const int P = H * W;
    const int iters = fused_iters(P);
    const int chunks = (P + iters * PX_PER_ITER - 1) / (iters * PX_PER_ITER);
    (void)vote_rows_hint;
    static const int ablate = env_int("NMSA_FUSED_ABLATE", 0);
    const size_t lds = (size_t)max_centers * sizeof(float2) + (size_t)FUSED_VOTE_SLOTS * 8 + 256;
    if (lds > 64 * 1024) return NMSA_ERR_ARG;
    const bool vec = (P % 4 == 0) &&
                     (((uintptr_t)logits | (uintptr_t)offset | (uintptr_t)sem_u8 |
                       (uintptr_t)inst | (uintptr_t)fg_out | (uintptr_t)score) % 16 == 0);
    dim3 grid(chunks, B), block(FUSED_THREADS);
#define NMSA_LAUNCH_FUSED(V, S)                                                              \
    hipLaunchKernelGGL((k_panoptic_fused<DTYPE, V, S>), grid, block, lds, stream, logits,    \
                       offset, centers_yx, n_centers, is_thing, C, H, W, max_centers, iters, \
                       sy, sx, use_thr, thr, sem_u8, inst, fg_out, score, votes, ablate)
    static const int tiled = env_int("NMSA_FUSED_TILED", 2);
    static const int tile_w = env_int("NMSA_FUSED_TILE_W", 128);
    if (vec && !score && W % 4 == 0 && (tiled == 2 || (tiled == 1 && DTYPE != NMSA_F32))) {
        if (tile_w == 64) {
            const int tiles = ((W + 63) / 64) * ((H + 15) / 16);
            hipLaunchKernelGGL((k_panoptic_fused<DTYPE, true, false, 8, true, false, true, 6>),
                               dim3((tiles + iters - 1) / iters, B), block, lds, stream, logits, offset,
                               centers_yx, n_centers, is_thing, C, H, W, max_centers, iters, sy, sx,
                               use_thr, thr, sem_u8, inst, fg_out, score, votes, ablate);
        } else if (tile_w == 256) {
            const int tiles = ((W + 255) / 256) * ((H + 3) / 4);
            hipLaunchKernelGGL((k_panoptic_fused<DTYPE, true, false, 8, true, false, true, 8>),
                               dim3((tiles + iters - 1) / iters, B), block, lds, stream, logits, offset,
                               centers_yx, n_centers, is_thing, C, H, W, max_centers, iters, sy, sx,
                               use_thr, thr, sem_u8, inst, fg_out, score, votes, ablate);
        } else {
            const int tiles = ((W + 127) / 128) * ((H + 7) / 8);
            hipLaunchKernelGGL((k_panoptic_fused<DTYPE, true, false, 8, true, false, true, 7>),
                               dim3((tiles + iters - 1) / iters, B), block, lds, stream, logits, offset,
                               centers_yx, n_centers, is_thing, C, H, W, max_centers, iters, sy, sx,
                               use_thr, thr, sem_u8, inst, fg_out, score, votes, ablate);
        }
    } else if (vec && score && W % 4 == 0 && tiled == 2 && env_int("NMSA_FUSED_SCORE_TILED", 1)) {
        const int tiles = ((W + 127) / 128) * ((H + 7) / 8);
        hipLaunchKernelGGL((k_panoptic_fused<DTYPE, true, true, 8, true, false, true, 7>),
                           dim3((tiles + iters - 1) / iters, B), block, lds, stream, logits, offset,
                           centers_yx, n_centers, is_thing, C, H, W, max_centers, iters, sy, sx,
                           use_thr, thr, sem_u8, inst, fg_out, score, votes, ablate);
    } else if (vec) { if (score) NMSA_LAUNCH_FUSED(true, true); else NMSA_LAUNCH_FUSED(true, false); }
    else { if (score) NMSA_LAUNCH_FUSED(false, true); else NMSA_LAUNCH_FUSED(false, false); }
#undef NMSA_LAUNCH_FUSED
    return check_launch();
}

template <int DTYPE>
int launch_argmax(const void* logits, int B, int C, int P, uint8_t* idx_u8, int64_t* idx_i64,
                  float* score, hipStream_t stream)
{
    const bool vec = (P % 4 == 0) &&
                     (((uintptr_t)logits | (uintptr_t)idx_u8 | (uintptr_t)idx_i64 |
                       (uintptr_t)score) % 16 == 0);
    dim3 grid((P + PX_PER_ITER - 1) / PX_PER_ITER, B), block(FUSED_THREADS);
#define NMSA_LAUNCH_ARGMAX(V, S)                                                          \
    hipLaunchKernelGGL((k_semantic_argmax<DTYPE, V, S>), grid, block, 0, stream, logits,  \
                       C, P, idx_u8, idx_i64, score)
    if (vec) { if (score) NMSA_LAUNCH_ARGMAX(true, true); else NMSA_LAUNCH_ARGMAX(true, false); }
    else { if (score) NMSA_LAUNCH_ARGMAX(false, true); else NMSA_LAUNCH_ARGMAX(false, false); }
#undef NMSA_LAUNCH_ARGMAX
    return check_launch();
}

template <int DTYPE>
int launch_softmax(const void* logits, int B, int C, int P, float* probs, hipStream_t stream)
{
    const bool vec = (P % 4 == 0) && (((uintptr_t)logits | (uintptr_t)probs) % 16 == 0);
    dim3 grid((P + PX_PER_ITER - 1) / PX_PER_ITER, B), block(FUSED_THREADS);
    if (vec && C <= 48 && getenv("NMSA_SOFTMAX_2PASS") == nullptr)
        hipLaunchKernelGGL((k_semantic_softmax_reg<DTYPE, 48>), grid, block, 0, stream, logits, C, P, probs);
    else if (vec) hipLaunchKernelGGL((k_semantic_softmax<DTYPE, true>), grid, block, 0, stream, logits, C, P, probs);
    else hipLaunchKernelGGL((k_semantic_softmax<DTYPE, false>), grid, block, 0, stream, logits, C, P, probs);
    return check_launch();
}

bool bad_dims(int B, int H, int W)
{
    return B <= 0 || H <= 0 || W <= 0 || (int64_t)H * W > ((int64_t)1 << 30) || B > 65535;
}

}

extern "C" int nmsa_group_offsets(const float* offset, const uint8_t* fg,
                                  const int32_t* centers_yx, const int32_t* n_centers,
                                  int B, int H, int W, int max_centers,
                                  float scale_y, float scale_x,
                                  int use_dist_thr, float dist_thr,
                                  uint8_t* inst, int32_t* area, nmsa_stream_t stream_)
{
    hipStream_t stream = (hipStream_t)stream_;
    if (!offset || !fg || !centers_yx || !n_centers || !inst) return NMSA_ERR_ARG;
    if (bad_dims(B, H, W) || max_centers <= 0) return NMSA_ERR_ARG;
    const int P = H * W;
    const size_t lds = (size_t)max_centers * sizeof(float2) + 256 * 4;
    if (lds > 64 * 1024) return NMSA_ERR_ARG;
    int rc;
    if (area) {
        rc = check_hip(hipMemsetAsync(area, 0, (size_t)B * 256 * sizeof(int32_t), stream));
        if (rc) return rc;
    }
    const int iters = 2;
    const int chunks = (P + iters * PX_PER_ITER - 1) / (iters * PX_PER_ITER);
    const bool vec = (P % 4 == 0) &&
                     (((uintptr_t)offset | (uintptr_t)fg | (uintptr_t)inst) % 16 == 0);
    dim3 grid(chunks, B), block(FUSED_THREADS);
    static const int tiled_env = getenv("NMSA_GROUP_TILED") ? atoi(getenv("NMSA_GROUP_TILED")) : 1;
    if (vec && W % 4 == 0 && tiled_env) {
        const int tiles = ((W + 63) / 64) * ((H + 15) / 16);
        hipLaunchKernelGGL((k_group_offsets<true, true>), dim3((tiles + iters - 1) / iters, B), block, lds,
                           stream, offset, fg, centers_yx, n_centers, H, W, max_centers, iters,
                           scale_y, scale_x, use_dist_thr, dist_thr, inst, area);
    } else if (vec)
        hipLaunchKernelGGL(k_group_offsets<true>, grid, block, lds, stream, offset, fg, centers_yx,
                           n_centers, H, W, max_centers, iters, scale_y, scale_x, use_dist_thr,
                           dist_thr, inst, area);
    else
        hipLaunchKernelGGL(k_group_offsets<false>, grid, block, lds, stream, offset, fg, centers_yx,
                           n_centers, H, W, max_centers, iters, scale_y, scale_x, use_dist_thr,
                           dist_thr, inst, area);
    return check_launch();
}

extern "C" int nmsa_semantic_argmax(const void* logits, int logits_dtype,
                                    int B, int C, int H, int W,
                                    uint8_t* idx_u8, int64_t* idx_i64, float* score,
                                    nmsa_stream_t stream_)
{
    hipStream_t stream = (hipStream_t)stream_;
    if (!logits || bad_dims(B, H, W) || C <= 0) return NMSA_ERR_ARG;
    if (idx_u8 && C > 256) return NMSA_ERR_ARG;
    const int P = H * W;
    switch (logits_dtype) {
        case NMSA_F32: return launch_argmax<NMSA_F32>(logits, B, C, P, idx_u8, idx_i64, score, stream);
        case NMSA_BF16: return launch_argmax<NMSA_BF16>(logits, B, C, P, idx_u8, idx_i64, score, stream);
        case NMSA_F16: return launch_argmax<NMSA_F16>(logits, B, C, P, idx_u8, idx_i64, score, stream);
        default: return NMSA_ERR_ARG;
    }
}

extern "C" int nmsa_semantic_softmax(const void* logits, int logits_dtype,
                                     int B, int C, int H, int W, float* probs,
                                     nmsa_stream_t stream_)
{
    hipStream_t stream = (hipStream_t)stream_;
    if (!logits || !probs || bad_dims(B, H, W) || C <= 0) return NMSA_ERR_ARG;
    const int P = H * W;
    switch (logits_dtype) {
        case NMSA_F32: return launch_softmax<NMSA_F32>(logits, B, C, P, probs, stream);
        case NMSA_BF16: return launch_softmax<NMSA_BF16>(logits, B, C, P, probs, stream);
        case NMSA_F16: return launch_softmax<NMSA_F16>(logits, B, C, P, probs, stream);
        default: return NMSA_ERR_ARG;
    }
}

extern "C" int nmsa_panoptic_fused(const void* logits, int logits_dtype, const float* offset,
                                   const int32_t* centers_yx, const int32_t* n_centers,
                                   const uint8_t* is_thing,
                                   int B, int C, int H, int W, int max_centers,
                                   float scale_y, float scale_x,
                                   int use_dist_thr, float dist_thr,
                                   uint8_t* sem_u8, uint8_t* inst, uint8_t* fg_out, float* score,
                                   uint32_t* votes, int votes_are_zero, int vote_rows_hint,
                                   nmsa_stream_t stream_)
{
    hipStream_t stream = (hipStream_t)stream_;
    if (!logits || !offset || !centers_yx || !n_centers || !is_thing || !sem_u8 || !inst || !votes)
        return NMSA_ERR_ARG;
    if (bad_dims(B, H, W) || C <= 0 || C > 256 || max_centers <= 0) return NMSA_ERR_ARG;
    if (!votes_are_zero) {
        int rc = check_hip(hipMemsetAsync(votes, 0, (size_t)B * 256 * (C + 1) * sizeof(uint32_t), stream));
        if (rc) return rc;
    }
    switch (logits_dtype) {
        case NMSA_F32:
            return launch_fused<NMSA_F32>(logits, offset, centers_yx, n_centers, is_thing, B, C, H, W,
                                          max_centers, scale_y, scale_x, use_dist_thr, dist_thr,
                                          sem_u8, inst, fg_out, score, votes, vote_rows_hint, stream);
        case NMSA_BF16:
            return launch_fused<NMSA_BF16>(logits, offset, centers_yx, n_centers, is_thing, B, C, H, W,
                                           max_centers, scale_y, scale_x, use_dist_thr, dist_thr,
                                           sem_u8, inst, fg_out, score, votes, vote_rows_hint, stream);
        case NMSA_F16:
            return launch_fused<NMSA_F16>(logits, offset, centers_yx, n_centers, is_thing, B, C, H, W,
                                          max_centers, scale_y, scale_x, use_dist_thr, dist_thr,
                                          sem_u8, inst, fg_out, score, votes, vote_rows_hint, stream);
        default: return NMSA_ERR_ARG;
    }
}

extern "C" int nmsa_panoptic_assign(uint32_t* votes, int B, int n_vote_classes, int clear_votes,
                                    int64_t max_instances_per_category, int64_t void_label,
                                    int64_t* pan_of_inst, int32_t* area,
                                    int64_t* ids_pan, int64_t* ids_ins, int32_t* n_ids,
                                    nmsa_stream_t stream_)
{
    hipStream_t stream = (hipStream_t)stream_;
    if (!votes || !pan_of_inst || !ids_pan || !ids_ins || !n_ids) return NMSA_ERR_ARG;
    if (B <= 0 || n_vote_classes <= 0 || n_vote_classes > 4096) return NMSA_ERR_ARG;
    const int lds_words = assign_lds_words(n_vote_classes);
    hipLaunchKernelGGL(k_assign, dim3(B), dim3(ASSIGN_THREADS), assign_lds_bytes(n_vote_classes, lds_words),
                       stream, votes, n_vote_classes, clear_votes,
                       max_instances_per_category, void_label, pan_of_inst, area,
                       ids_pan, ids_ins, n_ids, lds_words);
    return check_launch();
}

extern "C" int nmsa_panoptic_paint(const uint8_t* sem_u8, const uint8_t* inst,
                                   const int64_t* pan_of_inst, const uint8_t* is_thing,
                                   int B, int C, int H, int W,
                                   int64_t max_instances_per_category, int64_t void_label,
                                   int64_t* pan, int64_t* pan_sem, nmsa_stream_t stream_)
{
    hipStream_t stream = (hipStream_t)stream_;
    if (!sem_u8 || !inst || !pan_of_inst || !is_thing || !pan) return NMSA_ERR_ARG;
    if (bad_dims(B, H, W) || C <= 0 || C > 256 || max_instances_per_category <= 0) return NMSA_ERR_ARG;
    const int P = H * W;
    const bool vec = (P % 8 == 0) &&
                     (((uintptr_t)sem_u8 | (uintptr_t)inst | (uintptr_t)pan | (uintptr_t)pan_sem) % 16 == 0);
    const int iters = 1;
    dim3 grid((P + 2048 * iters - 1) / (2048 * iters), B), block(256);
    if (vec) {
        const int steps = 4 * iters;
        hipLaunchKernelGGL(k_paint2, grid, block, 0, stream, sem_u8, inst, pan_of_inst, is_thing,
                           C, P, steps, max_instances_per_category, void_label, pan, pan_sem);
    }
    else
        hipLaunchKernelGGL(k_paint<false>, grid, block, 0, stream, sem_u8, inst, pan_of_inst, is_thing,
                           C, P, iters, max_instances_per_category, void_label, pan, pan_sem);
    return check_launch();
}

extern "C" int nmsa_panoptic_merge(const void* sem, int sem_dtype, const void* ins, int ins_dtype,
                                   const uint8_t* thing_seg, const uint8_t* is_thing_class,
                                   int B, int n_classes, int H, int W,
                                   int64_t max_instances_per_category, int64_t void_label,
                                   uint32_t* votes, int64_t* pan_of_inst,
                                   int64_t* pan, int64_t* ids_pan, int64_t* ids_ins, int32_t* n_ids,
                                   nmsa_stream_t stream_)
{
    hipStream_t stream = (hipStream_t)stream_;
    if (!sem || !ins || !thing_seg || !is_thing_class || !votes || !pan_of_inst || !pan ||
        !ids_pan || !ids_ins || !n_ids)
        return NMSA_ERR_ARG;
    if (bad_dims(B, H, W) || n_classes <= 0 || n_classes > 4096) return NMSA_ERR_ARG;
    if (sem_dtype < NMSA_U8 || sem_dtype > NMSA_I64 || ins_dtype < NMSA_U8 || ins_dtype > NMSA_I64)
        return NMSA_ERR_ARG;
    const int P = H * W;
    int rc = check_hip(hipMemsetAsync(votes, 0, (size_t)B * 256 * n_classes * sizeof(uint32_t), stream));
    if (rc) return rc;
    int gx = (P + MG_PX_PER_BLOCK - 1) / MG_PX_PER_BLOCK;
    if (gx > 1024) gx = 1024;
    const size_t esz[4] = {1, 2, 4, 8};
    const bool vec = P % 4 == 0 && (uintptr_t)sem % (4 * esz[sem_dtype]) == 0 &&
                     (uintptr_t)ins % (4 * esz[ins_dtype]) == 0 && (uintptr_t)thing_seg % 4 == 0 &&
                     (uintptr_t)pan % 16 == 0;
    if (vec) hipLaunchKernelGGL(k_merge_votes<true>, dim3(gx, B), dim3(256), 0, stream, sem, sem_dtype, ins,
                                ins_dtype, thing_seg, n_classes, P, votes);
    else hipLaunchKernelGGL(k_merge_votes<false>, dim3(gx, B), dim3(256), 0, stream, sem, sem_dtype, ins,
                            ins_dtype, thing_seg, n_classes, P, votes);
    rc = check_launch();
    if (rc) return rc;
    const int lds_words = assign_lds_words(n_classes);
    hipLaunchKernelGGL(k_assign, dim3(B), dim3(ASSIGN_THREADS), assign_lds_bytes(n_classes, lds_words),
                       stream, votes, n_classes, 0,
                       max_instances_per_category, void_label, pan_of_inst, (int32_t*)nullptr,
                       ids_pan, ids_ins, n_ids, lds_words);
    rc = check_launch();
    if (rc) return rc;
    if (vec) hipLaunchKernelGGL(k_merge_paint<true>, dim3(gx, B), dim3(256), 0, stream, sem, sem_dtype, ins,
                                ins_dtype, thing_seg, is_thing_class, pan_of_inst, n_classes, P,
                                max_instances_per_category, void_label, pan);
    else hipLaunchKernelGGL(k_merge_paint<false>, dim3(gx, B), dim3(256), 0, stream, sem, sem_dtype, ins,
                            ins_dtype, thing_seg, is_thing_class, pan_of_inst, n_classes, P,
                            max_instances_per_category, void_label, pan);
    return check_launch();
}

extern "C" int nmsa_instance_orientation(const float* orientation, const uint8_t* inst,
                                         const uint8_t* mask, int B, int H, int W,
                                         double* sums, int32_t* count, nmsa_stream_t stream_)
{
    hipStream_t stream = (hipStream_t)stream_;
    if (!orientation || !inst || !sums || !count || bad_dims(B, H, W)) return NMSA_ERR_ARG;
    const int P = H * W;
    int rc = check_hip(hipMemsetAsync(sums, 0, (size_t)B * 256 * 2 * sizeof(double), stream));
    if (rc) return rc;
    rc = check_hip(hipMemsetAsync(count, 0, (size_t)B * 256 * sizeof(int32_t), stream));
    if (rc) return rc;
    const int gx = (P + 4 * MG_PX_PER_BLOCK - 1) / (4 * MG_PX_PER_BLOCK);
    const bool vec = P % 4 == 0 && (uintptr_t)orientation % 16 == 0 && (uintptr_t)inst % 4 == 0 &&
                     (uintptr_t)mask % 4 == 0;
    if (vec) hipLaunchKernelGGL(k_orientation_sums<true>, dim3(gx, B), dim3(256), 0, stream, orientation,
                                inst, mask, P, sums, count);
    else hipLaunchKernelGGL(k_orientation_sums<false>, dim3(gx, B), dim3(256), 0, stream, orientation,
                            inst, mask, P, sums, count);
    return check_launch();
}

namespace nmsa {
__global__ __launch_bounds__(256) void k_pack_tables(
    const int32_t* __restrict__ n_centers, const int32_t* __restrict__ n_ids,
    const int32_t* __restrict__ centers_yx, const float* __restrict__ scores,
    const int32_t* __restrict__ area, const int64_t* __restrict__ ids_pan,
    const int64_t* __restrict__ ids_ins, int max_centers, int kc, int ka, int ki,
    double* __restrict__ out)
{
    const int b = blockIdx.x;
    const int row = 2 + 3 * kc + ka + 2 * ki;
    double* o = out + (size_t)b * row;
    for (int i = threadIdx.x; i < row; i += blockDim.x) {
        int k = i;
        double v;
        if (k == 0) v = n_centers[b];
        else if (k == 1) v = n_ids ? n_ids[b] : 0;
        else if ((k -= 2) < 2 * kc) v = centers_yx[(size_t)b * max_centers * 2 + k];
        else if ((k -= 2 * kc) < kc) v = scores[(size_t)b * max_centers + k];
        else if ((k -= kc) < ka) v = area[(size_t)b * 256 + k];
        else if ((k -= ka) < ki) v = (double)ids_pan[(size_t)b * 256 + k];
        else v = (double)ids_ins[(size_t)b * 256 + (k - ki)];
        o[i] = v;
    }
}
}

extern "C" int nmsa_pack_tables(const int32_t* n_centers, const int32_t* n_ids,
                                const int32_t* centers_yx, const float* scores,
                                const int32_t* area, const int64_t* ids_pan, const int64_t* ids_ins,
                                int B, int max_centers, int columns, double* out,
                                nmsa_stream_t stream_)
{
    if (!n_centers || !centers_yx || !scores || !area || !out) return NMSA_ERR_ARG;
    const bool with_ids = n_ids && ids_pan && ids_ins;
    if (B <= 0 || max_centers <= 0 || columns <= 0) return NMSA_ERR_ARG;
    const int kc = columns < max_centers ? columns : max_centers;
    const int ka = kc + 1 < 256 ? kc + 1 : 256;
    const int ki = with_ids ? (kc < 256 ? kc : 256) : 0;
    hipLaunchKernelGGL(nmsa::k_pack_tables, dim3(B), dim3(256), 0, (hipStream_t)stream_, n_centers, n_ids,
                       centers_yx, scores, area, ids_pan, ids_ins, max_centers, kc, ka, ki, out);
    return nmsa::check_launch();
}
```

nicr_mt_scene_analysis_amd/model/postprocessing/panoptic.py:

```python
import os
from typing import Dict, List, Tuple

import numpy as np
import torch

from ... import ops
from ...data.preprocessing.resize import get_fullres_key
from ...data.preprocessing.resize import get_valid_region_slices_and_fullres_shape
from ...types import BatchType
from ...types import DecoderRawOutputType
from ...types import PostprocessingOutputType
from ...utils._tables import IdTable
from ._lazy import LazyDict
from .dense_base import DensePostprocessingBase
from .instance import InstancePostprocessing
from .semantic import SemanticPostprocessing


class _HostTables:

    def __init__(self, fetch) -> None:
        self._fetch = fetch
        self._host = None

    def get(self) -> dict:
        if self._host is None:
            self._host = self._fetch()
            self._fetch = None
        return self._host


_PACK_VIA_DEVICE = os.environ.get('NMSA_PACK_VIA_DEVICE', '0') == '1'

class PanopticPostprocessing(DensePostprocessingBase):
    def __init__(
        self,
        semantic_postprocessing: SemanticPostprocessing,
        instance_postprocessing: InstancePostprocessing,
        semantic_classes_is_thing: Tuple[bool],
        semantic_class_has_orientation: Tuple[bool],
        normalized_offset: bool = True,
        compute_scores: bool = False,
        defer_host_sync: bool = False,
        **kwargs
    ) -> None:
        super().__init__()
        self._semantic_postprocessing = semantic_postprocessing
        self._instance_postprocessing = instance_postprocessing

        self._is_thing = np.asarray(semantic_classes_is_thing, dtype=bool)
        self._has_orientation = np.asarray(semantic_class_has_orientation, dtype=bool)
        self._thing_class_ids = np.where(self._is_thing)[0]
        self._thing_ids_panoptic = self._thing_class_ids + 1
        self._orientation_ids = np.where(self._has_orientation)[0] + 1

        self._normalized_offset = normalized_offset
        self._compute_scores = compute_scores
        self._defer_host_sync = defer_host_sync
        self._count_slots: Dict[tuple, dict] = {}
        self._pinned_ring: Dict[tuple, list] = {}
        self._pinned_next: Dict[tuple, int] = {}
        self._max_instances_per_category = 1 << 16
        self._host_columns = 32
        self._device_luts: Dict[torch.device, Tuple[torch.Tensor, torch.Tensor]] = {}

    @property
    def max_instances_per_category(self):
        return self._max_instances_per_category

    def _luts(self, device):
        if device not in self._device_luts:
            thing = torch.from_numpy(self._is_thing.astype(np.uint8)).to(device)
            ori = np.zeros((len(self._has_orientation) + 1,), np.uint8)
            ori[1:] = self._has_orientation
            self._device_luts[device] = (thing, torch.from_numpy(ori).to(device))
        return self._device_luts[device]

    def _postprocess_training(
        self, data: DecoderRawOutputType, batch: BatchType
    ) -> PostprocessingOutputType:
        (s_output, i_output), (s_side_outputs, i_side_outputs) = data
        r = self._semantic_postprocessing._postprocess_training((s_output, s_side_outputs), batch)
        r.update(self._instance_postprocessing._postprocess_training((i_output, i_side_outputs), batch))
        return r

    def _postprocess_inference(
        self, data: DecoderRawOutputType, batch: BatchType
    ) -> PostprocessingOutputType:
        (s_output, i_output), (s_side_outputs, i_side_outputs) = data
        post = self._instance_postprocessing
        with_orientation = (len(i_output) == 3)
        if with_orientation:
            center_heatmap, center_offset, orientation = i_output
        else:
            center_heatmap, center_offset = i_output
        dev = s_output.device
        thing_lut, ori_lut = self._luts(dev)

        def run(on_centers=None):
            return ops.panoptic_pipeline(
                s_output, center_heatmap, center_offset, thing_lut,
                threshold=post._heatmap_threshold,
                kernel_size=post._heatmap_nms_kernel_size,
                top_k=post._top_k_instances,
                apply_foreground_mask=post._heatmap_apply_foreground_mask,
                normalized_offset=self._normalized_offset,
                distance_threshold=post._offset_distance_threshold,
                max_instances_per_category=self._max_instances_per_category,
                void_label=0, max_centers=post._max_centers,
                want_score=self._compute_scores, want_foreground=False,
                want_panoptic_semantic=False, on_centers=on_centers)
        if self._defer_host_sync:
            p = run()
            tables = _HostTables(self._fetch_tables_async(p, post, checked=False))
        else:
            while True:
                peek = {}
                p = run(on_centers=lambda cen: peek.update(self._peek_center_counts(cen)))
                peek['done'].synchronize()
                n_max = int(peek['host'].max()) if peek['host'].numel() else 0
                if n_max > post._max_centers:
                    post._max_centers = 1 << (n_max - 1).bit_length()
                    continue
                if n_max > self._host_columns:
                    self._host_columns = 1 << (n_max - 1).bit_length()
                break
            tables = _HostTables(self._fetch_tables_async(p, post, checked=True))

        r = LazyDict(semantic_output=s_output, semantic_side_outputs=s_side_outputs)
        sem_u8 = p['semantic_idx_u8']
        r.set_lazy('semantic_softmax_scores', lambda: ops.semantic_softmax(s_output))
        if self._compute_scores:
            r['semantic_segmentation_score'] = p['semantic_score']
        else:
            r.set_lazy('semantic_segmentation_score',
                       lambda: ops.semantic_argmax(s_output, want_u8=False, want_i64=False,
                                                   want_score=True)['score'])
        r.set_lazy('semantic_segmentation_idx', lambda: sem_u8.long())
        r.aux['semantic_segmentation_idx'] = sem_u8
        self._semantic_postprocessing._fullres_entries(r, s_output, batch)

        r.merge(post._postprocess_inference((i_output, i_side_outputs), batch))

        panoptic_seg = p['panoptic']
        instance_seg = p['instance']
        r.set_lazy('panoptic_foreground_mask', lambda: thing_lut[sem_u8.long()].to(torch.bool))
        r['panoptic_segmentation_deeplab'] = panoptic_seg
        r.aux['panoptic_parts'] = {
            'panoptic': panoptic_seg, 'semantic_idx_u8': sem_u8, 'instance': instance_seg,
            'pan_of_inst': p['pan_of_inst'], 'is_thing': thing_lut, 'void_label': 0,
            'max_instances_per_category': self._max_instances_per_category}
        r.set_lazy('panoptic_segmentation_deeplab_ids',
                   lambda: self._id_dicts_from_host(tables.get()))
        max_inst = self._max_instances_per_category
        r.set_derived('panoptic_segmentation_deeplab_semantic_idx',
                      lambda d: torch.div(d['panoptic_segmentation_deeplab'], max_inst,
                                          rounding_mode='floor'))
        r['panoptic_segmentation_deeplab_instance_idx'] = instance_seg
        r.aux['panoptic_id_table'] = IdTable.from_merge(p)
        ori_key = 'orientations_panoptic_segmentation_deeplab_instance'

        def _meta(d):
            h = tables.get()
            meta = InstancePostprocessing._meta_from_host(h['n_centers'], h['centers_yx'],
                                                          h['scores'], h['area'])
            if with_orientation:
                for m, o in zip(meta, d[ori_key]):
                    for id_ in m:
                        m[id_]['orientation'] = o.get(id_, float('nan'))
            return meta
        r.set_derived('panoptic_segmentation_deeplab_instance_meta', _meta)
        if with_orientation:
            def _orientation_table():
                fg = ori_lut[torch.div(panoptic_seg, max_inst, rounding_mode='floor')].to(torch.bool)
                return post._get_instance_orientation_table(orientation, instance_seg, fg)
            r.aux.setdefault('orientation_tables', LazyDict()).set_lazy(ori_key, _orientation_table)
            r.set_derived(ori_key, lambda d: d.aux['orientation_tables'][ori_key].to_dicts())

        if self._compute_scores:
            self._add_scores(r, p, r['panoptic_segmentation_deeplab_ids'],
                             r['panoptic_segmentation_deeplab_instance_meta'])

        crop, shape = get_valid_region_slices_and_fullres_shape(batch, 'instance')

        def _fullres(t):
            return self._crop_to_valid_region_and_resize_prediction(
                t, valid_region_slices=crop, shape=shape, mode='nearest')

        keys = ['panoptic_segmentation_deeplab',
                'panoptic_segmentation_deeplab_instance_idx',
                'panoptic_segmentation_deeplab_semantic_idx']
        if self._compute_scores:
            keys += ['panoptic_segmentation_deeplab_semantic_score',
                     'panoptic_segmentation_deeplab_instance_score',
                     'panoptic_segmentation_deeplab_panoptic_score']
        for k in keys:
            if r.is_pending(k):
                r.set_derived(get_fullres_key(k), (lambda kk: (lambda d: _fullres(d[kk])))(k))
            else:
                r[get_fullres_key(k)] = _fullres(r[k])

        return r

    @staticmethod
    def _fetch_tables(p, columns: int) -> dict:
        B, K = p['center_scores'].shape
        kc = max(1, min(int(columns), K))
        ki = min(kc, p['ids_pan'].shape[1])
        ka = min(kc + 1, p['area'].shape[1])
        flat_dev = torch.empty((B, 2 + 3 * kc + ka + 2 * ki), dtype=torch.float64,
                               device=p['center_scores'].device)
        L = ops.L
        L.check(L.lib().nmsa_pack_tables(
            L.ptr(p['n_centers']), L.ptr(p['n_ids']), L.ptr(p['centers_yx']),
            L.ptr(p['center_scores']), L.ptr(p['area']), L.ptr(p['ids_pan']), L.ptr(p['ids_ins']),
            B, K, kc, L.ptr(flat_dev), L.stream_ptr(flat_dev.device)), 'nmsa_pack_tables')
        return PanopticPostprocessing._split_tables(flat_dev.cpu().numpy(), B, kc, ka, ki)

    def _peek_center_counts(self, cen) -> dict:
        n = cen['n_centers']
        dev = n.device
        key = (dev, n.shape[0])
        slot = self._count_slots.get(key)
        if slot is None:
            slot = self._count_slots[key] = {
                'host': torch.empty(n.shape, dtype=n.dtype, pin_memory=True),
                'stream': torch.cuda.Stream(device=dev), 'ready': torch.cuda.Event(),
                'done': torch.cuda.Event()}
        cur = torch.cuda.current_stream(dev)
        slot['ready'].record(cur)
        with torch.cuda.stream(slot['stream']):
            slot['stream'].wait_event(slot['ready'])
            slot['host'].copy_(n, non_blocking=True)
            slot['done'].record(slot['stream'])
        n.record_stream(slot['stream'])
        return {'host': slot['host'], 'done': slot['done']}

    def _fetch_tables_async(self, p, post, checked: bool = False):
        B, K = p['center_scores'].shape
        kc = max(1, min(int(self._host_columns), K))
        ki = min(kc, p['ids_pan'].shape[1])
        ka = min(kc + 1, p['area'].shape[1])
        dev = p['center_scores'].device
        shape = (B, 2 + 3 * kc + ka + 2 * ki)
        L = ops.L
        slot = self._pinned_slot(shape)
        flat_host = slot['buffer']
        via_device = _PACK_VIA_DEVICE
        flat_dev = torch.empty(shape, dtype=torch.float64, device=dev) if via_device else flat_host
        L.check(L.lib().nmsa_pack_tables(
            L.ptr(p['n_centers']), L.ptr(p['n_ids']), L.ptr(p['centers_yx']),
            L.ptr(p['center_scores']), L.ptr(p['area']), L.ptr(p['ids_pan']), L.ptr(p['ids_ins']),
            B, K, kc, L.ptr(flat_dev), L.stream_ptr(dev)), 'nmsa_pack_tables')
        if via_device:
            flat_host.copy_(flat_dev, non_blocking=True)
        done = slot['event']
        done.record(torch.cuda.current_stream(dev))
        max_centers = post._max_centers
        state = {'flat': None}

        def detach():
            if state['flat'] is None:
                done.synchronize()
                state['flat'] = flat_host.numpy().copy()
        slot['detach'] = detach

        def finish():
            detach()
            if slot.get('detach') is detach:
                slot['detach'] = None
            host = self._split_tables(state['flat'], B, kc, ka, ki)
            n_max = max(host['n_centers'], default=0)
            if n_max > max_centers and not checked:
                post._max_centers = 1 << (n_max - 1).bit_length()
                raise RuntimeError(
                    f'{n_max} centers survived the top-k ties but the center table held '
                    f'{max_centers}: this result is truncated (defer_host_sync=True cannot re-run '
                    'it); the table has been enlarged for the following calls')
            if n_max > kc:
                self._host_columns = 1 << (n_max - 1).bit_length()
                host = self._fetch_tables(p, self._host_columns)
            return host
        return finish

    def _pinned_slot(self, shape, ring: int = 8) -> dict:
        slots = self._pinned_ring.setdefault(shape, [])
        if len(slots) < ring:
            slots.append({'buffer': torch.empty(shape, dtype=torch.float64, pin_memory=True),
                          'event': torch.cuda.Event(), 'detach': None})
            self._pinned_next[shape] = 0
            return slots[-1]
        i = self._pinned_next[shape]
        self._pinned_next[shape] = (i + 1) % ring
        slot = slots[i]
        if slot['detach'] is not None:
            slot['detach']()
            slot['detach'] = None
        else:
            slot['event'].synchronize()
        return slot

    @staticmethod
    def _split_tables(flat, B, kc, ka, ki) -> dict:
        edges = np.cumsum([0, 1, 1, 2 * kc, kc, ka, ki, ki])
        cols = [flat[:, a:b] for a, b in zip(edges[:-1], edges[1:])]
        return {'columns': kc,
                'n_centers': cols[0][:, 0].astype(np.int64).tolist(),
                'n_ids': cols[1][:, 0].astype(np.int64).tolist(),
                'centers_yx': cols[2].reshape(B, kc, 2), 'scores': cols[3], 'area': cols[4],
                'ids_pan': cols[5], 'ids_ins': cols[6]}

    @staticmethod
    def _id_dicts_from_host(host) -> List[dict]:
        pan = host['ids_pan'].astype(np.int64).tolist()
        ins = host['ids_ins'].astype(np.int64).tolist()
        return [dict(zip(pr[:n], ir[:n])) for pr, ir, n in zip(pan, ins, host['n_ids'])]

    def _add_scores(self, r, p, panoptic_ids: List[dict], meta: List[dict]) -> None:
        B = p['instance'].shape[0]
        dev = p['instance'].device
        score_tab = torch.zeros((B, 256), dtype=torch.float32, device=dev)
        k = min(p['center_scores'].shape[1], 255)
        score_tab[:, 1:k + 1] = p['center_scores'][:, :k]
        sc = ops.panoptic_scores(
            r['semantic_output'], p['semantic_idx_u8'], p['semantic_score'], p['instance'],
            p['panoptic'], p['pan_of_inst'], score_tab, self._max_instances_per_category)
        r['panoptic_segmentation_deeplab_semantic_score'] = sc['semantic_score']
        r['panoptic_segmentation_deeplab_instance_score'] = sc['instance_score']
        r['panoptic_segmentation_deeplab_panoptic_score'] = sc['panoptic_score']

        host = torch.cat([sc['mean_semantic_score'].double(),
                          (p['pan_of_inst'] // self._max_instances_per_category).double()],
                         dim=1).cpu().tolist()
        for b in range(B):
            for pan_id, ins_id in panoptic_ids[b].items():
                m = meta[b][ins_id]
                mean = float(np.float32(host[b][ins_id]))
                m['semantic_score'] = mean
                m['semantic_idx'] = int(host[b][256 + ins_id])
                m['panoptic_score'] = float(np.float32(mean) * np.float32(m['score']))
                m['panoptic_id'] = pan_id
```

nicr_mt_scene_analysis_amd/ops.py:

```python
import math
from typing import Dict, Optional, Sequence, Tuple

import numpy as np
import torch

from . import _lib as L

DEFAULT_MAX_CENTERS = 256

_VOTE_TABLES: 'collections.OrderedDict[tuple, torch.Tensor]' = __import__('collections').OrderedDict()
_VOTE_TABLES_MAX = 8


def _vote_table(dev: torch.device, B: int, n_cols: int) -> torch.Tensor:
    key = (dev, B, n_cols, torch.cuda.current_stream(dev).cuda_stream)
    t = _VOTE_TABLES.get(key)
    if t is None:
        t = torch.zeros((B, 256, n_cols), dtype=torch.int32, device=dev)
        _VOTE_TABLES[key] = t
        while len(_VOTE_TABLES) > _VOTE_TABLES_MAX:
            _VOTE_TABLES.popitem(last=False)
    else:
        _VOTE_TABLES.move_to_end(key)
    return t


def _u8(t: Optional[torch.Tensor]) -> Optional[torch.Tensor]:
    if t is None:
        return None
    if t.dtype == torch.bool:
        return t.contiguous().view(torch.uint8)
    if t.dtype == torch.uint8:
        return t.contiguous()
    return (t != 0).contiguous().view(torch.uint8)


def center_nms_topk(
    center_heatmap: torch.Tensor,
    foreground_mask: Optional[torch.Tensor] = None,
    threshold: float = 0.1,
    kernel_size: int = 3,
    top_k: int = 64,
    apply_foreground_mask: bool = False,
    max_centers: int = DEFAULT_MAX_CENTERS,
    want_mask: bool = False,
) -> Dict[str, torch.Tensor]:
    c = L.require_device_tensor(center_heatmap, 'center_heatmap')
    if c.dtype != torch.float32:
        c = c.float()
    if c.ndim == 4:
        assert c.shape[1] == 1
        c = c[:, 0]
    c = c.contiguous()
    B, H, W = c.shape
    dev = c.device
    fg = _u8(foreground_mask) if apply_foreground_mask else None
    cyx = torch.empty((B, max_centers, 2), dtype=torch.int32, device=dev)
    n = torch.empty((B,), dtype=torch.int32, device=dev)
    scores = torch.empty((B, max_centers), dtype=torch.float32, device=dev)
    mask = torch.empty((B, H, W), dtype=torch.uint8, device=dev) if want_mask else None
    ws_bytes = L.lib().nmsa_center_nms_workspace_bytes(B, H, W)
    ws = torch.empty((ws_bytes,), dtype=torch.uint8, device=dev)
    L.check(L.lib().nmsa_center_nms_topk(
        L.ptr(c), L.ptr(fg), B, H, W, float(threshold), int(kernel_size), int(top_k),
        int(bool(apply_foreground_mask)), int(max_centers),
        L.ptr(cyx), L.ptr(n), L.ptr(scores), L.ptr(mask), L.ptr(ws), ws_bytes,
        L.stream_ptr(dev)), 'nmsa_center_nms_topk')
    out = {'centers_yx': cyx, 'n_centers': n, 'scores': scores}
    if want_mask:
        out['center_mask'] = mask.view(torch.bool)
    return out


def group_offsets(
    center_offset: torch.Tensor,
    foreground_mask: torch.Tensor,
    centers_yx: torch.Tensor,
    n_centers: torch.Tensor,
    scale_y: float = 1.0,
    scale_x: float = 1.0,
    distance_threshold: Optional[float] = None,
    want_area: bool = True,
) -> Dict[str, torch.Tensor]:
    off = L.require_device_tensor(center_offset, 'center_offset')
    if off.dtype != torch.float32:
        off = off.float()
    B, two, H, W = off.shape
    assert two == 2
    dev = off.device
    fg = _u8(foreground_mask)
    inst = torch.empty((B, H, W), dtype=torch.uint8, device=dev)
    area = torch.empty((B, 256), dtype=torch.int32, device=dev) if want_area else None
    L.check(L.lib().nmsa_group_offsets(
        L.ptr(off), L.ptr(fg), L.ptr(centers_yx), L.ptr(n_centers), B, H, W,
        int(centers_yx.shape[1]), float(scale_y), float(scale_x),
        0 if distance_threshold is None else 1,
        0.0 if distance_threshold is None else float(distance_threshold),
        L.ptr(inst), L.ptr(area), L.stream_ptr(dev)), 'nmsa_group_offsets')
    return {'instance': inst, 'area': area}


NMSA_ELEM_F32 = 8


def _crop_geometry(t: torch.Tensor, crop) -> Tuple[int, int, int, int, int, int]:
    Hs, Ws = int(t.shape[-2]), int(t.shape[-1])
    if crop is None:
        return Hs, Ws, 0, 0, Hs, Ws
    sl_h, sl_w = crop
    y0, y1, st_y = sl_h.indices(Hs)
    x0, x1, st_x = sl_w.indices(Ws)
    if st_y != 1 or st_x != 1 or y1 <= y0 or x1 <= x0:
        raise ValueError(f'unsupported valid-region slices {crop}')
    return Hs, Ws, y0, x0, y1 - y0, x1 - x0


def resize_nearest(maps: torch.Tensor, size: Tuple[int, int], crop=None) -> torch.Tensor:
    x = L.require_device_tensor(maps, 'maps')
    code = NMSA_ELEM_F32 if x.dtype == torch.float32 else L.int_dtype_code(x)
    Hs, Ws, y0, x0, h, w = _crop_geometry(x, crop)
    Ho, Wo = int(size[0]), int(size[1])
    planes = x.numel() // (Hs * Ws)
    out = torch.empty(tuple(x.shape[:-2]) + (Ho, Wo), dtype=x.dtype, device=x.device)
    L.check(L.lib().nmsa_resize_nearest(
        L.ptr(x), code, planes, Hs, Ws, y0, x0, h, w, Ho, Wo, L.ptr(out),
        L.stream_ptr(x.device)), 'nmsa_resize_nearest')
    return out


def resize_bilinear(maps: torch.Tensor, size: Tuple[int, int], crop=None) -> torch.Tensor:
    x = L.require_device_tensor(maps, 'maps')
    Hs, Ws, y0, x0, h, w = _crop_geometry(x, crop)
    Ho, Wo = int(size[0]), int(size[1])
    planes = x.numel() // (Hs * Ws)
    out = torch.empty(tuple(x.shape[:-2]) + (Ho, Wo), dtype=x.dtype, device=x.device)
    L.check(L.lib().nmsa_resize_bilinear(
        L.ptr(x), L.float_dtype_code(x), planes, Hs, Ws, y0, x0, h, w, Ho, Wo, L.ptr(out),
        L.stream_ptr(x.device)), 'nmsa_resize_bilinear')
    return out


def semantic_argmax_resized(
    logits: torch.Tensor,
    size: Tuple[int, int],
    crop=None,
    want_u8: bool = False,
    want_i64: bool = True,
    want_score: bool = True,
) -> Dict[str, torch.Tensor]:
    x = L.require_device_tensor(logits, 'logits')
    B, Cn = int(x.shape[0]), int(x.shape[1])
    Hs, Ws, y0, x0, h, w = _crop_geometry(x, crop)
    Ho, Wo = int(size[0]), int(size[1])
    dev = x.device
    u8 = torch.empty((B, Ho, Wo), dtype=torch.uint8, device=dev) if want_u8 else None
    i64 = torch.empty((B, Ho, Wo), dtype=torch.int64, device=dev) if want_i64 else None
    sc = torch.empty((B, Ho, Wo), dtype=torch.float32, device=dev) if want_score else None
    L.check(L.lib().nmsa_semantic_argmax_resized(
        L.ptr(x), L.float_dtype_code(x), B, Cn, Hs, Ws, y0, x0, h, w, Ho, Wo,
        L.ptr(u8), L.ptr(i64), L.ptr(sc), L.stream_ptr(dev)), 'nmsa_semantic_argmax_resized')
    return {'idx_u8': u8, 'idx': i64, 'score': sc}


def semantic_argmax(
    logits: torch.Tensor,
    want_u8: bool = False,
    want_i64: bool = True,
    want_score: bool = True,
) -> Dict[str, torch.Tensor]:
    x = L.require_device_tensor(logits, 'logits')
    B, Cn, H, W = x.shape
    dev = x.device
    u8 = torch.empty((B, H, W), dtype=torch.uint8, device=dev) if want_u8 else None
    i64 = torch.empty((B, H, W), dtype=torch.int64, device=dev) if want_i64 else None
    sc = torch.empty((B, H, W), dtype=torch.float32, device=dev) if want_score else None
    L.check(L.lib().nmsa_semantic_argmax(
        L.ptr(x), L.float_dtype_code(x), B, Cn, H, W, L.ptr(u8), L.ptr(i64), L.ptr(sc),
        L.stream_ptr(dev)), 'nmsa_semantic_argmax')
    return {'idx_u8': u8, 'idx': i64, 'score': sc}


def semantic_softmax(logits: torch.Tensor) -> torch.Tensor:
    x = L.require_device_tensor(logits, 'logits')
    B, Cn, H, W = x.shape
    probs = torch.empty((B, Cn, H, W), dtype=torch.float32, device=x.device)
    L.check(L.lib().nmsa_semantic_softmax(
        L.ptr(x), L.float_dtype_code(x), B, Cn, H, W, L.ptr(probs),
        L.stream_ptr(x.device)), 'nmsa_semantic_softmax')
    return probs


def panoptic_pipeline(
    semantic_logits: torch.Tensor,
    center_heatmap: torch.Tensor,
    center_offset: torch.Tensor,
    is_thing: torch.Tensor,
    threshold: float = 0.1,
    kernel_size: int = 3,
    top_k: int = 64,
    apply_foreground_mask: bool = False,
    normalized_offset: bool = True,
    distance_threshold: Optional[float] = None,
    max_instances_per_category: int = 1 << 16,
    void_label: int = 0,
    max_centers: int = DEFAULT_MAX_CENTERS,
    want_score: bool = False,
    want_foreground: bool = True,
    want_panoptic_semantic: bool = False,
    fused_kernel_events: Optional[list] = None,
    on_centers=None,
) -> Dict[str, torch.Tensor]:
    lib = L.lib()
    x = L.require_device_tensor(semantic_logits, 'semantic_logits')
    off = L.require_device_tensor(center_offset, 'center_offset')
    if off.dtype != torch.float32:
        off = off.float()
    B, Cn, H, W = x.shape
    dev = x.device
    st = L.stream_ptr(dev)
    thing = _u8(is_thing)

    fg_for_nms = None
    if apply_foreground_mask:
        pre = semantic_argmax(x, want_u8=True, want_i64=False, want_score=False)
        fg_for_nms = thing[pre['idx_u8'].long()]
    cen = center_nms_topk(center_heatmap, fg_for_nms, threshold, kernel_size, top_k,
                          apply_foreground_mask, max_centers)
    if on_centers is not None:
        on_centers(cen)

    sem_u8 = torch.empty((B, H, W), dtype=torch.uint8, device=dev)
    inst = torch.empty((B, H, W), dtype=torch.uint8, device=dev)
    fg = torch.empty((B, H, W), dtype=torch.uint8, device=dev) if want_foreground else None
    score = torch.empty((B, H, W), dtype=torch.float32, device=dev) if want_score else None
    votes = _vote_table(dev, B, Cn + 1)
    vote_key = (dev, B, Cn + 1, torch.cuda.current_stream(dev).cuda_stream)
    sy, sx = (float(H), float(W)) if normalized_offset else (1.0, 1.0)
    if fused_kernel_events is not None:
        ev0 = torch.cuda.Event(enable_timing=True)
        ev1 = torch.cuda.Event(enable_timing=True)
        ev0.record(torch.cuda.current_stream(dev))
    L.check(lib.nmsa_panoptic_fused(
        L.ptr(x), L.float_dtype_code(x), L.ptr(off), L.ptr(cen['centers_yx']),
        L.ptr(cen['n_centers']), L.ptr(thing), B, Cn, H, W, int(max_centers), sy, sx,
        0 if distance_threshold is None else 1,
        0.0 if distance_threshold is None else float(distance_threshold),
        L.ptr(sem_u8), L.ptr(inst), L.ptr(fg), L.ptr(score), L.ptr(votes), 1,
        int(top_k) + 1, st), 'nmsa_panoptic_fused')
    if fused_kernel_events is not None:
        ev1.record(torch.cuda.current_stream(dev))
        fused_kernel_events.append((ev0, ev1))

    pan_of_inst = torch.empty((B, 256), dtype=torch.int64, device=dev)
    area = torch.empty((B, 256), dtype=torch.int32, device=dev)
    ids_pan = torch.empty((B, 256), dtype=torch.int64, device=dev)
    ids_ins = torch.empty((B, 256), dtype=torch.int64, device=dev)
    n_ids = torch.empty((B,), dtype=torch.int32, device=dev)
    try:
        L.check(lib.nmsa_panoptic_assign(
            L.ptr(votes), B, Cn + 1, 1, int(max_instances_per_category), int(void_label),
            L.ptr(pan_of_inst), L.ptr(area), L.ptr(ids_pan), L.ptr(ids_ins), L.ptr(n_ids), st),
            'nmsa_panoptic_assign')
    except Exception:
        _VOTE_TABLES.pop(vote_key, None)
        raise

    pan = torch.empty((B, H, W), dtype=torch.int64, device=dev)
    pan_sem = torch.empty((B, H, W), dtype=torch.int64, device=dev) \
        if want_panoptic_semantic else None
    L.check(lib.nmsa_panoptic_paint(
        L.ptr(sem_u8), L.ptr(inst), L.ptr(pan_of_inst), L.ptr(thing), B, Cn, H, W,
        int(max_instances_per_category), int(void_label), L.ptr(pan), L.ptr(pan_sem), st),
        'nmsa_panoptic_paint')

    return {
        'semantic_idx_u8': sem_u8, 'semantic_score': score,
        'foreground': None if fg is None else fg.view(torch.bool),
        'instance': inst, 'panoptic': pan, 'panoptic_semantic': pan_sem,
        'centers_yx': cen['centers_yx'], 'n_centers': cen['n_centers'],
        'center_scores': cen['scores'], 'area': area,
        'ids_pan': ids_pan, 'ids_ins': ids_ins, 'n_ids': n_ids,
        'pan_of_inst': pan_of_inst,
    }


def panoptic_scores(
    logits: torch.Tensor,
    semantic_idx_u8: torch.Tensor,
    semantic_prob: torch.Tensor,
    instance: torch.Tensor,
    panoptic: torch.Tensor,
    pan_of_inst: torch.Tensor,
    instance_score_table: torch.Tensor,
    max_instances_per_category: int,
) -> Dict[str, torch.Tensor]:
    x = L.require_device_tensor(logits, 'logits')
    B, Cn, H, W = x.shape
    dev = x.device
    sem = L.require_device_tensor(semantic_idx_u8, 'semantic_idx_u8')
    prob = L.require_device_tensor(semantic_prob, 'semantic_prob')
    ins = L.require_device_tensor(instance, 'instance')
    pan = L.require_device_tensor(panoptic, 'panoptic')
    poi = L.require_device_tensor(pan_of_inst, 'pan_of_inst')
    tab = L.require_device_tensor(instance_score_table, 'instance_score_table')
    assert sem.dtype == torch.uint8 and ins.dtype == torch.uint8 and pan.dtype == torch.int64
    assert prob.dtype == torch.float32 and tab.dtype == torch.float32 and poi.dtype == torch.int64
    assert tuple(tab.shape) == (B, 256) and tuple(poi.shape) == (B, 256)
    out = [torch.empty((B, H, W), dtype=torch.float32, device=dev) for _ in range(3)]
    mean = torch.empty((B, 256), dtype=torch.float32, device=dev)
    ws_bytes = L.lib().nmsa_panoptic_scores_workspace_bytes(B)
    ws = torch.empty((ws_bytes // 8,), dtype=torch.float64, device=dev)
    L.check(L.lib().nmsa_panoptic_scores(
        L.ptr(x), L.float_dtype_code(x), L.ptr(sem), L.ptr(prob), L.ptr(ins), L.ptr(pan),
        L.ptr(poi), L.ptr(tab), B, Cn, H, W, int(max_instances_per_category),
        L.ptr(out[0]), L.ptr(out[1]), L.ptr(out[2]), L.ptr(mean), L.ptr(ws), ws_bytes,
        L.stream_ptr(dev)), 'nmsa_panoptic_scores')
    return {'semantic_score': out[0], 'instance_score': out[1], 'panoptic_score': out[2],
            'mean_semantic_score': mean}


_GAUSS_LUTS: Dict[tuple, torch.Tensor] = {}


def _gauss_lut(sigma: int, dev: torch.device) -> torch.Tensor:
    key = (int(sigma), dev)
    if key not in _GAUSS_LUTS:
        import numpy as np
        r = 3 * int(sigma) + 1
        d2 = np.arange(2 * r * r + 1, dtype=np.float64)
        lut = np.exp(-d2 / (2 * int(sigma) ** 2)).astype(np.float32)
        _GAUSS_LUTS[key] = torch.from_numpy(lut).to(dev)
    return _GAUSS_LUTS[key]


_TARGET_WORKSPACES: 'collections.OrderedDict[tuple, list]' = __import__('collections').OrderedDict()


def _targets_workspace(B: int, n_classes: int, max_instances: int, dev, reusable: bool = False):
    nbytes = L.lib().nmsa_targets_workspace_bytes(B, n_classes, max_instances)
    if nbytes == 0:
        raise ValueError('max_instances must be in [1, 4096]')
    if not reusable:
        t = torch.empty(((nbytes + 7) // 8,), dtype=torch.int64, device=dev)
        return t, nbytes, [t, 0]
    key = (dev, torch.cuda.current_stream(dev).cuda_stream, B, n_classes, max_instances)
    entry = _TARGET_WORKSPACES.get(key)
    if entry is None:
        entry = _TARGET_WORKSPACES[key] = [torch.empty(((nbytes + 7) // 8,), dtype=torch.int64, device=dev), 0]
        while len(_TARGET_WORKSPACES) > 4:
            _TARGET_WORKSPACES.popitem(last=False)
    else:
        _TARGET_WORKSPACES.move_to_end(key)
    return entry[0], nbytes, entry


def _targets_on_wire(sem: torch.Tensor, ins: torch.Tensor, H: int, W: int, n_classes: int) -> bool:
    import os
    return (os.environ.get('NMSA_TG_FUSED', '1') != '0' and sem.dtype == torch.uint8 and
            ins.dtype == torch.int32 and W % 4 == 0 and n_classes <= 16384 and
            sem.data_ptr() % 4 == 0 and ins.data_ptr() % 16 == 0)


def targets_route(semantic: torch.Tensor, instance: torch.Tensor, n_classes: int, sigma: int = 8,
                  max_instances: int = 1024) -> int:
    sem = L.require_device_tensor(semantic, 'semantic')
    ins = L.require_device_tensor(instance, 'instance')
    B, H, W = sem.shape
    rc = L.lib().nmsa_targets_route(
        L.ptr(sem), L.int_dtype_code(sem), L.ptr(ins), L.int_dtype_code(ins), int(n_classes), H, W,
        int(sigma), int(max_instances), None, None, None, None, None)
    if rc < 0:
        L.check(rc, 'nmsa_targets_route')
    return rc


def instance_clear_stuff(semantic: torch.Tensor, instance: torch.Tensor,
                         is_stuff_class: torch.Tensor) -> torch.Tensor:
    sem = L.require_device_tensor(semantic, 'semantic')
    if not instance.is_cuda or not instance.is_contiguous():
        raise L.NmsaError('instance must be a contiguous device tensor (modified in place)')
    lut = _u8(is_stuff_class)
    L.check(L.lib().nmsa_instance_clear_stuff(
        L.ptr(sem), L.int_dtype_code(sem), L.ptr(instance), L.int_dtype_code(instance),
        L.ptr(lut), int(lut.numel()), int(sem.numel()), L.stream_ptr(sem.device)),
        'nmsa_instance_clear_stuff')
    return instance


def instance_targets(
    semantic: torch.Tensor,
    instance: torch.Tensor,
    n_classes: int,
    is_thing_class: Optional[torch.Tensor],
    is_stuff_class: Optional[torch.Tensor],
    sigma: int,
    normalized_offset: bool = True,
    max_instances: int = 1024,
) -> Dict[str, torch.Tensor]:
    sem = L.require_device_tensor(semantic, 'semantic')
    ins = L.require_device_tensor(instance, 'instance')
    B, H, W = sem.shape
    dev = sem.device
    th = None if is_thing_class is None else _u8(is_thing_class)
    st = None if is_stuff_class is None else _u8(is_stuff_class)
    cap = ((int(max_instances) + 1023) // 1024) * 1024
    center = torch.empty((B, H, W), dtype=torch.float32, device=dev)
    offset = torch.empty((B, 2, H, W), dtype=torch.float32 if normalized_offset else torch.int16,
                         device=dev)
    fg = torch.empty((B, H, W), dtype=torch.uint8, device=dev)
    cm = torch.empty((B, H, W), dtype=torch.uint8, device=dev)
    enc = torch.empty((B, cap), dtype=torch.int32, device=dev)
    skp = torch.empty((B, cap), dtype=torch.int32, device=dev)
    n_enc = torch.empty((B,), dtype=torch.int32, device=dev)
    n_skp = torch.empty((B,), dtype=torch.int32, device=dev)
    on_wire = _targets_on_wire(sem, ins, H, W, int(n_classes))
    ws, ws_bytes, ws_entry = _targets_workspace(B, int(n_classes), int(max_instances), dev, reusable=on_wire)
    clean, ws_entry[1] = ws_entry[1], 0
    status = torch.empty((1,), dtype=torch.int32, device=dev) if on_wire else \
        torch.zeros((1,), dtype=torch.int32, device=dev)
    L.check(L.lib().nmsa_instance_targets(
        L.ptr(sem), L.int_dtype_code(sem), L.ptr(ins), L.int_dtype_code(ins), L.ptr(th), L.ptr(st),
        B, int(n_classes), H, W, int(sigma), L.ptr(_gauss_lut(sigma, dev)),
        int(bool(normalized_offset)), int(max_instances),
        L.ptr(center), L.ptr(offset), L.ptr(fg), L.ptr(cm), L.ptr(enc), L.ptr(n_enc),
        L.ptr(skp), L.ptr(n_skp), L.ptr(status), L.ptr(ws), ws_bytes, int(clean), L.stream_ptr(dev)),
        'nmsa_instance_targets')
    ws_entry[1] = int(on_wire)
    return {'center': center, 'offset': offset, 'foreground': fg.view(torch.bool),
            'center_mask': cm.view(torch.bool), 'encoded_ids': enc, 'n_encoded': n_enc,
            'skipped_ids': skp, 'n_skipped': n_skp, 'status': status}


def panoptic_targets(
    semantic: torch.Tensor,
    instance: torch.Tensor,
    n_classes: int,
    is_thing_class: Optional[torch.Tensor],
    max_instances_per_category: int,
    void_label: int = 0,
    max_instances: int = 1024,
    max_segments: int = 2048,
) -> Dict[str, torch.Tensor]:
    sem = L.require_device_tensor(semantic, 'semantic')
    ins = L.require_device_tensor(instance, 'instance')
    B, H, W = sem.shape
    dev = sem.device
    th = None if is_thing_class is None else _u8(is_thing_class)
    pan = torch.empty((B, H, W), dtype=torch.int64, device=dev)
    ids_pan = torch.empty((B, int(max_segments)), dtype=torch.int64, device=dev)
    ids_ins = torch.empty((B, int(max_segments)), dtype=torch.int64, device=dev)
    n_ids = torch.empty((B,), dtype=torch.int32, device=dev)
    on_wire = _targets_on_wire(sem, ins, H, W, int(n_classes))
    ws, ws_bytes, ws_entry = _targets_workspace(B, int(n_classes), int(max_instances), dev, reusable=on_wire)
    clean, ws_entry[1] = ws_entry[1], 0
    status = torch.empty((1,), dtype=torch.int32, device=dev) if on_wire else \
        torch.zeros((1,), dtype=torch.int32, device=dev)
    L.check(L.lib().nmsa_panoptic_targets(
        L.ptr(sem), L.int_dtype_code(sem), L.ptr(ins), L.int_dtype_code(ins), L.ptr(th),
        B, int(n_classes), H, W, int(max_instances_per_category), int(void_label),
        int(max_instances), int(max_segments), L.ptr(pan), L.ptr(ids_pan), L.ptr(ids_ins),
        L.ptr(n_ids), L.ptr(status), L.ptr(ws), ws_bytes, int(clean), L.stream_ptr(dev)),
        'nmsa_panoptic_targets')
    ws_entry[1] = int(on_wire)
    return {'panoptic': pan, 'ids_pan': ids_pan, 'ids_ins': ids_ins, 'n_ids': n_ids,
            'status': status}


def orientation_targets(
    semantic: torch.Tensor,
    instance: torch.Tensor,
    n_classes: int,
    estimate_class: Optional[torch.Tensor],
    keys: torch.Tensor,
    n_keys: torch.Tensor,
    biternion: torch.Tensor,
    max_instances: int = 1024,
) -> Dict[str, torch.Tensor]:
    sem = L.require_device_tensor(semantic, 'semantic')
    ins = L.require_device_tensor(instance, 'instance')
    k = L.require_device_tensor(keys, 'keys')
    nk = L.require_device_tensor(n_keys, 'n_keys')
    bit = L.require_device_tensor(biternion, 'biternion')
    B, H, W = sem.shape
    K = int(k.shape[1])
    if k.dtype != torch.int32 or nk.dtype != torch.int32 or bit.dtype != torch.float32:
        raise TypeError('keys / n_keys must be int32 and biternion float32')
    if tuple(k.shape) != (B, K) or tuple(nk.shape) != (B,) or tuple(bit.shape) != (B, K, 2):
        raise ValueError(f'keys [B,K], n_keys [B], biternion [B,K,2] expected for B = {B}, got '
                         f'{tuple(k.shape)}, {tuple(nk.shape)}, {tuple(bit.shape)}')
    dev = sem.device
    est = None if estimate_class is None else _u8(estimate_class)
    ori = torch.empty((B, 2, H, W), dtype=torch.float32, device=dev)
    fg = torch.empty((B, H, W), dtype=torch.uint8, device=dev)
    present = torch.empty((B, K), dtype=torch.uint8, device=dev)
    on_wire = _targets_on_wire(sem, ins, H, W, int(n_classes))
    ws, ws_bytes, ws_entry = _targets_workspace(B, int(n_classes), int(max_instances), dev, reusable=on_wire)
    clean, ws_entry[1] = ws_entry[1], 0
    status = torch.empty((1,), dtype=torch.int32, device=dev) if on_wire else \
        torch.zeros((1,), dtype=torch.int32, device=dev)
    L.check(L.lib().nmsa_orientation_targets(
        L.ptr(sem), L.int_dtype_code(sem), L.ptr(ins), L.int_dtype_code(ins), L.ptr(est),
        L.ptr(k), L.ptr(nk), L.ptr(bit), B, int(n_classes), H, W, K, int(max_instances),
        L.ptr(ori), L.ptr(fg), L.ptr(present), L.ptr(status), L.ptr(ws), ws_bytes, int(clean),
        L.stream_ptr(dev)), 'nmsa_orientation_targets')
    ws_entry[1] = int(on_wire)
    return {'orientation': ori, 'foreground': fg.view(torch.bool), 'present': present,
            'status': status}


def dve_targets(
    panoptic: torch.Tensor,
    keys: torch.Tensor,
    n_keys: torch.Tensor,
    embeddings: Optional[torch.Tensor] = None,
    image_embedding: Optional[torch.Tensor] = None,
    diff_factor: float = 0.65,
) -> Dict[str, torch.Tensor]:
    pan = L.require_device_tensor(panoptic, 'panoptic')
    k = L.require_device_tensor(keys, 'keys')
    nk = L.require_device_tensor(n_keys, 'n_keys')
    assert pan.dtype == torch.int64 and k.dtype == torch.int64 and nk.dtype == torch.int32
    B, H, W = pan.shape
    K = int(k.shape[1])
    dev = pan.device
    idx = torch.empty((B, H, W), dtype=torch.int32, device=dev)
    lut = None
    D = 0
    emb = img = None
    if embeddings is not None:
        emb = L.require_device_tensor(embeddings, 'embeddings').float()
        img = L.require_device_tensor(image_embedding, 'image_embedding').float()
        D = int(emb.shape[2])
        lut = torch.empty((B, K, D), dtype=torch.float32, device=dev)
    L.check(L.lib().nmsa_dve_targets(
        L.ptr(pan), L.ptr(k), L.ptr(nk), L.ptr(emb), L.ptr(img), float(diff_factor),
        B, K, D, H, W, L.ptr(lut), L.ptr(idx), L.stream_ptr(dev)), 'nmsa_dve_targets')
    return {'indices': idx, 'lut': lut}


def _dve_project_args(emb, weight_a, weight_b):
    if emb.dtype != torch.float32:
        raise TypeError(f'emb must be float32, got {emb.dtype}')
    if not emb.is_cuda:
        raise L.NmsaError(f'emb is on {emb.device}: the HIP path needs tensors on the MI355X '
                          '(there is no CPU fallback).')
    if emb.ndim != 4:
        raise ValueError(f'emb must be [B, D, H, W], got shape {tuple(emb.shape)}')
    B, D, H, W = (int(n) for n in emb.shape)
    dev = emb.device
    heads = []
    for name, w in (('weight_a', weight_a), ('weight_b', weight_b)):
        if w is None:
            heads.append((None, 0, None))
            continue
        if w.dtype != torch.float32:
            raise TypeError(f'{name} must be float32, got {w.dtype}')
        w = L.require_device_tensor(w, name)
        if w.device != dev:
            raise ValueError(f'{name} is on {w.device}, emb on {dev}')
        if w.ndim == 4 and w.shape[2:] == (1, 1):
            w = w[:, :, 0, 0].contiguous()
        if w.ndim != 2 or int(w.shape[1]) != D or int(w.shape[0]) < 1:
            raise ValueError(f'{name} must be [C, {D}], got shape {tuple(w.shape)}')
        Cn = int(w.shape[0])
        heads.append((w, Cn, torch.empty((B, Cn, H, W), dtype=torch.float32, device=dev)))
    x = emb if emb.is_contiguous() else emb.contiguous()
    return (B, D, H, W), x, heads


def dve_project(
    emb: torch.Tensor,
    weight_a: Optional[torch.Tensor] = None,
    weight_b: Optional[torch.Tensor] = None,
    *,
    generic: bool = False,
) -> Tuple[Optional[torch.Tensor], Optional[torch.Tensor]]:
    (B, D, H, W), x, heads = _dve_project_args(emb, weight_a, weight_b)
    if x.numel():
        (wa, Ca, la), (wb, Cb, lb) = heads
        L.check(L.lib().nmsa_dve_project(
            L.ptr(x), B, D, H, W, L.ptr(wa), Ca, L.ptr(la), L.ptr(wb), Cb, L.ptr(lb),
            1 if generic else 0, L.stream_ptr(emb.device)), 'nmsa_dve_project')
        if x is not emb:
            emb.copy_(x)
    return heads[0][2], heads[1][2]

# ... 989 lines not shown
```

nicr_mt_scene_analysis_amd/task_helper/semantic.py:

```python
import torch

from ..data.preprocessing.resize import get_fullres
from ..data.preprocessing.resize import get_fullres_key
from ..loss import _functional as F_
from ..loss import check_loss_status
from ..loss import CrossEntropyLossSemantic
from ..metric import MeanIntersectionOverUnion
from .base import TaskHelperBase
from .base import append_detached_losses_to_logs
from .base import append_profile_to_logs

_TASK = 'semantic'


class SemanticTaskHelper(TaskHelperBase):
    def __init__(self, n_classes, class_weights=None, label_smoothing=0.0,
                 disable_multiscale_supervision=False, examples_cmap=None):
        super().__init__()
        self._n_classes = n_classes
        self._class_weights = class_weights
        self._label_smoothing = label_smoothing
        self._disable_multiscale_supervision = disable_multiscale_supervision
        self._examples_cmap = examples_cmap
        self._examples = {}

    def initialize(self, device):
        weights = self._class_weights
        if weights is not None:
            weights = torch.as_tensor(weights, dtype=torch.float, device=device)
            self._class_weights = weights
        self._loss = CrossEntropyLossSemantic(weights=weights,
                                              label_smoothing=self._label_smoothing)
        self._metric_iou = MeanIntersectionOverUnion(n_classes=self._n_classes, device=device)
        self._metric_iou.reset()

    def _compute_losses(self, batch, batch_idx, predictions_post):
        side_key = None if self._disable_multiscale_supervision else f'{_TASK}_side_outputs'
        predictions, targets, scale_names = self.collect_predictions_and_targets_for_loss(
            batch=batch, batch_key=_TASK, predictions_post=predictions_post,
            predictions_post_key=f'{_TASK}_output', side_outputs_key=side_key)
        from ..loss import _multi
        items = [{'kind': 'ce', 'pred': p, 'mask': t, 'weights': self._class_weights,
                  'param': self._label_smoothing, 'total': 0} for p, t in zip(predictions, targets)]
        if F_.speculation_enabled() and _multi.supported(items) and \
                all(p.ndim == 4 for p in predictions):
            return self.multi_losses(items, [f'{_TASK}_loss_{name}' for name in scale_names], (_TASK,))
        per_scale = self._loss(input_tensors=predictions, target_tensors=targets)
        sums = [loss_sum for loss_sum, _ in per_scale]
        counts = [count for _, count in per_scale]
        losses = {f'{_TASK}_loss_{name}': s / n for name, s, n in zip(scale_names, sums, counts)}
        losses[self.mark_as_total(_TASK)] = self.accumulate_losses(losses=sums, n_elements=counts)
        return losses

    @append_profile_to_logs(f'{_TASK}_step_time')
    @append_detached_losses_to_logs()
    def training_step(self, batch, batch_idx, predictions_post):
        return self._compute_losses(batch, batch_idx, predictions_post), {}

    @append_profile_to_logs(f'{_TASK}_step_time')
    @append_detached_losses_to_logs()
    def validation_step(self, batch, batch_idx, predictions_post):
        losses = self._compute_losses(batch, batch_idx, predictions_post)
        key = get_fullres_key(f'{_TASK}_segmentation_idx')
        aux = getattr(predictions_post, 'aux', {})
        self._metric_iou.update_masked_void(aux[key] if key in aux else predictions_post[key],
                                            get_fullres(batch, _TASK))
        return losses, {}

    @append_profile_to_logs(f'{_TASK}_epoch_end_time')
    def validation_epoch_end(self):
        check_loss_status()
        miou, ious = self._metric_iou.compute(return_ious=True)
        artifacts = {f'{_TASK}_cm': self._metric_iou.confmat.clone(),
                     f'{_TASK}_ious_per_class': ious.clone()}
        self._metric_iou.reset()
        return artifacts, self._examples, {f'{_TASK}_miou': miou}
```

Before: 31660 Mpix/s.

## Fuse semantic cross-entropy loss into panoptic fused argmax kernel pass

Adds a WITH_CE variant of the fused panoptic kernel. While it runs the argmax over the logits it also accumulates a log-sum-exp cross-entropy against the labels, reduces per-block partials into a slab, and turns them into means. The validation semantic loss can then reuse this pass instead of making a separate read of the full logits tensor. The cost is extra registers in the kernel (waves_per_eu lowered to 4), more routing logic, and a fallback whenever the identity checks on predictions, targets or weights do not match. The benchmark metric is merge+metrics, so whether the loss path is actually exercised there is uncertain.

```diff
diff --git a/include/nmsa.h b/include/nmsa.h
--- a/include/nmsa.h
+++ b/include/nmsa.h
@@ -65,6 +65,21 @@
                         uint8_t* sem_u8, uint8_t* inst, uint8_t* fg_out, float* score,
                         uint32_t* votes, int votes_are_zero, int vote_rows_hint,
                         nmsa_stream_t stream);
+
+size_t nmsa_panoptic_fused_ce_slab_bytes(int B, int H, int W);
+int nmsa_panoptic_fused_ce(const void* logits, int logits_dtype, const float* offset,
+                           const int32_t* centers_yx, const int32_t* n_centers,
+                           const uint8_t* is_thing,
+                           int B, int C, int H, int W, int max_centers,
+                           float scale_y, float scale_x,
+                           int use_dist_thr, float dist_thr,
+                           uint8_t* sem_u8, uint8_t* inst, uint8_t* fg_out,
+                           uint32_t* votes, int votes_are_zero, int vote_rows_hint,
+                           const uint8_t* ce_labels, const float* ce_weights,
+                           void* ce_slab, size_t ce_slab_bytes,
+                           double* ce_loss_sum, double* ce_weight_sum,
+                           int64_t* ce_n_elements, float* ce_means, int32_t* status,
+                           nmsa_stream_t stream);
 
 int nmsa_panoptic_assign(uint32_t* votes, int B, int n_vote_classes, int clear_votes,
                          int64_t max_instances_per_category, int64_t void_label,
diff --git a/nicr_mt_scene_analysis_amd/_lib.py b/nicr_mt_scene_analysis_amd/_lib.py
--- a/nicr_mt_scene_analysis_amd/_lib.py
+++ b/nicr_mt_scene_analysis_amd/_lib.py
@@ -63,6 +63,10 @@
     'nmsa_semantic_softmax': (_i, [_vp, _i, _i, _i, _i, _i, _vp, _vp]),
     'nmsa_panoptic_fused': (_i, [_vp, _i, _vp, _vp, _vp, _vp, _i, _i, _i, _i, _i,
                                  _f, _f, _i, _f, _vp, _vp, _vp, _vp, _vp, _i, _i, _vp]),
+    'nmsa_panoptic_fused_ce_slab_bytes': (_sz, [_i, _i, _i]),
+    'nmsa_panoptic_fused_ce': (_i, [_vp, _i, _vp, _vp, _vp, _vp, _i, _i, _i, _i, _i,
+                                    _f, _f, _i, _f, _vp, _vp, _vp, _vp, _i, _i,
+                                    _vp, _vp, _vp, _sz, _vp, _vp, _vp, _vp, _vp, _vp]),
     'nmsa_panoptic_assign': (_i, [_vp, _i, _i, _i, _i64, _i64, _vp, _vp, _vp, _vp, _vp, _vp]),
     'nmsa_panoptic_paint': (_i, [_vp, _vp, _vp, _vp, _i, _i, _i, _i, _i64, _i64,
                                  _vp, _vp, _vp]),
diff --git a/nicr_mt_scene_analysis_amd/csrc/argmax_state.hpp b/nicr_mt_scene_analysis_amd/csrc/argmax_state.hpp
--- a/nicr_mt_scene_analysis_amd/csrc/argmax_state.hpp
+++ b/nicr_mt_scene_analysis_amd/csrc/argmax_state.hpp
@@ -42,6 +42,15 @@
     const int first = (v[0] == gm) ? 0 : (v[1] == gm) ? 1 : (v[2] == gm) ? 2 : 3;
     s.am[j] = (gm > s.m[j]) ? c0 + first : s.am[j];
     s.m[j] = nm;
+}
+
+__device__ __forceinline__ void argmax_group4_ce(ArgmaxState& s, int j, const float v[4], int c0,
+                                                 int t, float& xt)
+{
+    argmax_group4_score(s, j, v, c0);
+    const int tj = t - c0;
+#pragma unroll
+    for (int i = 0; i < 4; ++i) xt = (tj == i) ? v[i] : xt;
 }
 
 __device__ __forceinline__ float aten_vec_expf(float d)
diff --git a/nicr_mt_scene_analysis_amd/csrc/panoptic.hip b/nicr_mt_scene_analysis_amd/csrc/panoptic.hip
--- a/nicr_mt_scene_analysis_amd/csrc/panoptic.hip
+++ b/nicr_mt_scene_analysis_amd/csrc/panoptic.hip
@@ -3,6 +3,7 @@
 
 #include "nmsa_common.hpp"
 #include "argmax_state.hpp"
+#include "loss_common.hpp"
 
 namespace nmsa {
 
@@ -144,6 +145,18 @@
     }
 }
 
+__device__ __forceinline__ void argmax_quad_ce(ArgmaxState& st, const float4& a, const float4& b,
+                                               const float4& c, const float4& d, int c0,
+                                               const int t[4], float xt[4])
+{
+    const float p0[4] = {a.x, b.x, c.x, d.x}, p1[4] = {a.y, b.y, c.y, d.y};
+    const float p2[4] = {a.z, b.z, c.z, d.z}, p3[4] = {a.w, b.w, c.w, d.w};
+    argmax_group4_ce(st, 0, p0, c0, t[0], xt[0]);
+    argmax_group4_ce(st, 1, p1, c0, t[1], xt[1]);
+    argmax_group4_ce(st, 2, p2, c0, t[2], xt[2]);
+    argmax_group4_ce(st, 3, p3, c0, t[3], xt[3]);
+}
+
 __device__ __forceinline__ float sqdist(float cy, float cx, float ly, float lx)
 {
     const float dy = __fsub_rn(cy, ly);
@@ -292,17 +305,27 @@
     }
 }
 
+struct FusedCeArgs {
+    const uint8_t* labels;
+    const float* weights;
+    LossPartial* slab;
+    int* status;
+};
+struct FusedNoCe {};
+
 template <int DTYPE, bool VEC, bool WITH_SCORE, int UNROLL = 8, bool NT = true,
-          bool EARLY_OFFSETS = false, bool TILED = false, int TILE_LOG2W = 6>
-__global__ __launch_bounds__(FUSED_THREADS) __attribute__((amdgpu_waves_per_eu(5, WITH_SCORE ? 8 : 5))) void k_panoptic_fused(
+          bool EARLY_OFFSETS = false, bool TILED = false, int TILE_LOG2W = 6, bool WITH_CE = false>
+__global__ __launch_bounds__(FUSED_THREADS) __attribute__((amdgpu_waves_per_eu(WITH_CE ? 4 : 5, WITH_SCORE ? 8 : 5))) void k_panoptic_fused(
     const void* __restrict__ logits, const float* __restrict__ offset,
     const int32_t* __restrict__ centers_yx, const int32_t* __restrict__ n_centers,
     const uint8_t* __restrict__ is_thing,
     int C, int H, int W, int max_centers, int iters,
     float scale_y, float scale_x, int use_thr, float thr,
     uint8_t* __restrict__ sem_u8, uint8_t* __restrict__ inst, uint8_t* __restrict__ fg_out,
-    float* __restrict__ score, uint32_t* __restrict__ votes, int ablate)
-{
+    float* __restrict__ score, uint32_t* __restrict__ votes, int ablate,
+    std::conditional_t<WITH_CE, FusedCeArgs, FusedNoCe> ce)
+{
+    static_assert(!(WITH_CE && WITH_SCORE), "the cross-entropy variant has no score output");
     extern __shared__ __align__(16) unsigned char smem[];
     float2* cen = (float2*)smem;
     int* vote_key = (int*)(cen + max_centers);
@@ -336,6 +359,9 @@
     uint32_t* votes_b = votes + (size_t)b * 256 * NC;
 
     const int chunk_start = blockIdx.x * iters * PX_PER_ITER;
+    float ce_sum = 0.f, ce_w = 0.f;
+    int ce_cnt = 0;
+    bool ce_bad = false;
     auto chunk = [&](const int it, auto first_tag) {
         constexpr bool FIRST = decltype(first_tag)::value;
         int p0;
@@ -362,6 +388,21 @@
         }
 
 
+        int ce_t[4] = {-1, -1, -1, -1};
+        float ce_xt[4] = {0.f, 0.f, 0.f, 0.f};
+        if constexpr (WITH_CE) {
+            if (active) {
+                const uint8_t* lp = ce.labels + (size_t)b * P + p0;
+                if (VEC) {
+                    const uchar4 l4 = *(const uchar4*)lp;
+                    ce_t[0] = (int)l4.x - 1; ce_t[1] = (int)l4.y - 1;
+                    ce_t[2] = (int)l4.z - 1; ce_t[3] = (int)l4.w - 1;
+                } else {
+                    for (int j = 0; j < nvalid; ++j) ce_t[j] = (int)lp[j] - 1;
+                }
+            }
+        }
+
         ArgmaxState st;
         argmax_init(st);
         if (active) {
@@ -373,8 +414,10 @@
                 for (int u = 0; u < UNROLL; ++u)
                     v[u] = load_px4<DTYPE, VEC, NT>(logits, img_logits + (size_t)(c + u) * P + p0, nvalid);
 #pragma unroll
-                for (int u = 0; u < UNROLL; u += 4)
-                    argmax_quad<WITH_SCORE>(st, v[u], v[u + 1], v[u + 2], v[u + 3], c + u);
+                for (int u = 0; u < UNROLL; u += 4) {
+                    if constexpr (WITH_CE) argmax_quad_ce(st, v[u], v[u + 1], v[u + 2], v[u + 3], c + u, ce_t, ce_xt);
+                    else argmax_quad<WITH_SCORE>(st, v[u], v[u + 1], v[u + 2], v[u + 3], c + u);
+                }
             }
             for (; c < C; c += 4) {
                 float4 v[4];
@@ -383,7 +426,21 @@
                     v[u] = (c + u < C)
                         ? load_px4<DTYPE, VEC, NT>(logits, img_logits + (size_t)(c + u) * P + p0, nvalid)
                         : make_float4(-INFINITY, -INFINITY, -INFINITY, -INFINITY);
-                argmax_quad<WITH_SCORE>(st, v[0], v[1], v[2], v[3], c, min(4, C - c));
+                if constexpr (WITH_CE) argmax_quad_ce(st, v[0], v[1], v[2], v[3], c, ce_t, ce_xt);
+                else argmax_quad<WITH_SCORE>(st, v[0], v[1], v[2], v[3], c, min(4, C - c));
+            }
+        }
+        if constexpr (WITH_CE) {
+#pragma unroll
+            for (int j = 0; j < 4; ++j) {
+                const int t = ce_t[j];
+                if (t < 0) continue;
+                if (t >= C) { ce_bad = true; continue; }
+                const float lse = fmaf(__log2f(st.se[j]), LN2, st.m[j]);
+                const float wt = ce.weights ? ce.weights[t] : 1.0f;
+                ce_sum += wt * (lse - ce_xt[j]);
+                ce_w += wt;
+                ++ce_cnt;
             }
         }
         if (FIRST && !lane_centers) {
@@ -411,7 +468,8 @@
                     cls[j] = __float_as_int(ex.y);
                 }
                 st.se[j] = sc;
-            } else if ((st.nf[j] != st.nf[j] || may_tie_in_probability<DTYPE>(st.m[j])) && j < nvalid) {
+            } else if (((WITH_CE ? st.se[j] != st.se[j] : st.nf[j] != st.nf[j]) ||
+                        may_tie_in_probability<DTYPE>(st.m[j])) && j < nvalid) {
                 cls[j] = column_class<DTYPE>(logits, img_logits + p0 + j, P, C, st.m[j]);
             }
             uint64_t tm = thing_m[0];
@@ -505,6 +563,29 @@
     {
         const int k = vote_key[threadIdx.x];
         if (k >= 0) atomicAdd(&votes_b[k], vote_cnt[threadIdx.x]);
+    }
+    if constexpr (WITH_CE) {
+        __shared__ double s_ce[FUSED_THREADS / 64][2];
+        __shared__ int s_ce_cnt[FUSED_THREADS / 64];
+        const float ws = wave_reduce_sum(ce_sum), ww = wave_reduce_sum(ce_w);
+        int wc = ce_cnt;
+#pragma unroll
+        for (int o = 32; o > 0; o >>= 1) wc += __shfl_down(wc, o);
+        const bool wave_bad = __any(ce_bad);
+        const int w = threadIdx.x >> 6;
+        if (lane_id() == 0) {
+            s_ce[w][0] = (double)ws; s_ce[w][1] = (double)ww; s_ce_cnt[w] = wc;
+            if (wave_bad) atomicOr(ce.status, 8);
+        }
+        __syncthreads();
+        if (threadIdx.x == 0) {
+            LossPartial p;
+            p.sum = 0.0; p.aux = 0.0; p.count = 0; p.pad = 0;
+            for (int k = 0; k < FUSED_THREADS / 64; ++k) {
+                p.sum += s_ce[k][0]; p.aux += s_ce[k][1]; p.count += s_ce_cnt[k];
+            }
+            ce.slab[(size_t)blockIdx.y * gridDim.x + blockIdx.x] = p;
+        }
     }
 }
 
@@ -1142,6 +1223,15 @@
     }
 }
 
+__global__ void k_fused_ce_means(const double* __restrict__ sum, const long long* __restrict__ count,
+                                 float* __restrict__ out)
+{
+    const float s = (float)*sum;
+    const long long n = *count;
+    out[0] = s / (float)n;
+    out[1] = s / (float)max(n, 1LL);
+}
+
 }
 
 using namespace nmsa;
@@ -1183,7 +1273,8 @@
                  int B, int C, int H, int W, int max_centers,
                  float sy, float sx, int use_thr, float thr,
                  uint8_t* sem_u8, uint8_t* inst, uint8_t* fg_out, float* score,
-                 uint32_t* votes, int vote_rows_hint, hipStream_t stream)
+                 uint32_t* votes, int vote_rows_hint, hipStream_t stream,
+                 const FusedCeArgs* ce = nullptr, int* ce_blocks = nullptr)
 {
     const int P = H * W;
     const int iters = fused_iters(P);
@@ -1194,12 +1285,36 @@
     if (lds > 64 * 1024) return NMSA_ERR_ARG;
     const bool vec = (P % 4 == 0) &&
                      (((uintptr_t)logits | (uintptr_t)offset | (uintptr_t)sem_u8 |
-                       (uintptr_t)inst | (uintptr_t)fg_out | (uintptr_t)score) % 16 == 0);
+                       (uintptr_t)inst | (uintptr_t)fg_out | (uintptr_t)score) % 16 == 0) &&
+                     (!ce || (uintptr_t)ce->labels % 4 == 0);
     dim3 grid(chunks, B), block(FUSED_THREADS);
+    if (ce) {
+        static const int tiled_ce = env_int("NMSA_FUSED_TILED", 2);
+        if (vec && W % 4 == 0 && tiled_ce == 2) {
+            const int tiles = ((W + 127) / 128) * ((H + 7) / 8);
+            grid = dim3((tiles + iters - 1) / iters, B);
+            hipLaunchKernelGGL((k_panoptic_fused<DTYPE, true, false, 8, true, false, true, 7, true>),
+                               grid, block, lds, stream, logits, offset, centers_yx, n_centers,
+                               is_thing, C, H, W, max_centers, iters, sy, sx, use_thr, thr, sem_u8, inst,
+                               fg_out, score, votes, ablate, *ce);
+        } else if (vec) {
+            hipLaunchKernelGGL((k_panoptic_fused<DTYPE, true, false, 8, true, false, false, 6, true>),
+                               grid, block, lds, stream, logits, offset, centers_yx, n_centers,
+                               is_thing, C, H, W, max_centers, iters, sy, sx, use_thr, thr, sem_u8, inst,
+                               fg_out, score, votes, ablate, *ce);
+        } else {
+            hipLaunchKernelGGL((k_panoptic_fused<DTYPE, false, false, 8, true, false, false, 6, true>),
+                               grid, block, lds, stream, logits, offset, centers_yx, n_centers,
+                               is_thing, C, H, W, max_centers, iters, sy, sx, use_thr, thr, sem_u8, inst,
+                               fg_out, score, votes, ablate, *ce);
+        }
+        *ce_blocks = (int)(grid.x * grid.y);
+        return check_launch();
+    }
 #define NMSA_LAUNCH_FUSED(V, S)                                                              \
     hipLaunchKernelGGL((k_panoptic_fused<DTYPE, V, S>), grid, block, lds, stream, logits,    \
                        offset, centers_yx, n_centers, is_thing, C, H, W, max_centers, iters, \
-                       sy, sx, use_thr, thr, sem_u8, inst, fg_out, score, votes, ablate)
+                       sy, sx, use_thr, thr, sem_u8, inst, fg_out, score, votes, ablate, FusedNoCe{})
     static const int tiled = env_int("NMSA_FUSED_TILED", 2);
     static const int tile_w = env_int("NMSA_FUSED_TILE_W", 128);
     if (vec && !score && W % 4 == 0 && (tiled == 2 || (tiled == 1 && DTYPE != NMSA_F32))) {
@@ -1208,31 +1323,33 @@
             hipLaunchKernelGGL((k_panoptic_fused<DTYPE, true, false, 8, true, false, true, 6>),
                                dim3((tiles + iters - 1) / iters, B), block, lds, stream, logits, offset,
                                centers_yx, n_centers, is_thing, C, H, W, max_centers, iters, sy, sx,
-                               use_thr, thr, sem_u8, inst, fg_out, score, votes, ablate);
+                               use_thr, thr, sem_u8, inst, fg_out, score, votes, ablate, FusedNoCe{});
         } else if (tile_w == 256) {
             const int tiles = ((W + 255) / 256) * ((H + 3) / 4);
             hipLaunchKernelGGL((k_panoptic_fused<DTYPE, true, false, 8, true, false, true, 8>),
                                dim3((tiles + iters - 1) / iters, B), block, lds, stream, logits, offset,
                                centers_yx, n_centers, is_thing, C, H, W, max_centers, iters, sy, sx,
-                               use_thr, thr, sem_u8, inst, fg_out, score, votes, ablate);
+                               use_thr, thr, sem_u8, inst, fg_out, score, votes, ablate, FusedNoCe{});
         } else {
             const int tiles = ((W + 127) / 128) * ((H + 7) / 8);
             hipLaunchKernelGGL((k_panoptic_fused<DTYPE, true, false, 8, true, false, true, 7>),
                                dim3((tiles + iters - 1) / iters, B), block, lds, stream, logits, offset,
                                centers_yx, n_centers, is_thing, C, H, W, max_centers, iters, sy, sx,
-                               use_thr, thr, sem_u8, inst, fg_out, score, votes, ablate);
+                               use_thr, thr, sem_u8, inst, fg_out, score, votes, ablate, FusedNoCe{});
         }
     } else if (vec && score && W % 4 == 0 && tiled == 2 && env_int("NMSA_FUSED_SCORE_TILED", 1)) {
         const int tiles = ((W + 127) / 128) * ((H + 7) / 8);
         hipLaunchKernelGGL((k_panoptic_fused<DTYPE, true, true, 8, true, false, true, 7>),
                            dim3((tiles + iters - 1) / iters, B), block, lds, stream, logits, offset,
                            centers_yx, n_centers, is_thing, C, H, W, max_centers, iters, sy, sx,
-                           use_thr, thr, sem_u8, inst, fg_out, score, votes, ablate);
+                           use_thr, thr, sem_u8, inst, fg_out, score, votes, ablate, FusedNoCe{});
     } else if (vec) { if (score) NMSA_LAUNCH_FUSED(true, true); else NMSA_LAUNCH_FUSED(true, false); }
     else { if (score) NMSA_LAUNCH_FUSED(false, true); else NMSA_LAUNCH_FUSED(false, false); }
 #undef NMSA_LAUNCH_FUSED
     return check_launch();
 }
+
+int fused_ce_blocks_per_image(int H, int W) { return ((W + 127) / 128) * ((H + 7) / 8); }
 
 template <int DTYPE>
 int launch_argmax(const void* logits, int B, int C, int P, uint8_t* idx_u8, int64_t* idx_i64,
@@ -1342,6 +1459,43 @@
     }
 }
 
+static int panoptic_fused_impl(const void* logits, int logits_dtype, const float* offset,
+                               const int32_t* centers_yx, const int32_t* n_centers,
+                               const uint8_t* is_thing,
+                               int B, int C, int H, int W, int max_centers,
+                               float scale_y, float scale_x,
+                               int use_dist_thr, float dist_thr,
+                               uint8_t* sem_u8, uint8_t* inst, uint8_t* fg_out, float* score,
+                               uint32_t* votes, int votes_are_zero, int vote_rows_hint,
+                               hipStream_t stream, const FusedCeArgs* ce, int* ce_blocks)
+{
+    if (!logits || !offset || !centers_yx || !n_centers || !is_thing || !sem_u8 || !inst || !votes)
+        return NMSA_ERR_ARG;
+    if (bad_dims(B, H, W) || C <= 0 || C > 256 || max_centers <= 0) return NMSA_ERR_ARG;
+    if (!votes_are_zero) {
+        int rc = check_hip(hipMemsetAsync(votes, 0, (size_t)B * 256 * (C + 1) * sizeof(uint32_t), stream));
+        if (rc) return rc;
+    }
+    switch (logits_dtype) {
+        case NMSA_F32:
+            return launch_fused<NMSA_F32>(logits, offset, centers_yx, n_centers, is_thing, B, C, H, W,
+                                          max_centers, scale_y, scale_x, use_dist_thr, dist_thr,
+                                          sem_u8, inst, fg_out, score, votes, vote_rows_hint, stream,
+                                          ce, ce_blocks);
+        case NMSA_BF16:
+            return launch_fused<NMSA_BF16>(logits, offset, centers_yx, n_centers, is_thing, B, C, H, W,
+                                           max_centers, scale_y, scale_x, use_dist_thr, dist_thr,
+                                           sem_u8, inst, fg_out, score, votes, vote_rows_hint, stream,
+                                           ce, ce_blocks);
+        case NMSA_F16:
+            return launch_fused<NMSA_F16>(logits, offset, centers_yx, n_centers, is_thing, B, C, H, W,
+                                          max_centers, scale_y, scale_x, use_dist_thr, dist_thr,
+                                          sem_u8, inst, fg_out, score, votes, vote_rows_hint, stream,
+                                          ce, ce_blocks);
+        default: return NMSA_ERR_ARG;
+    }
+}
+
 extern "C" int nmsa_panoptic_fused(const void* logits, int logits_dtype, const float* offset,
                                    const int32_t* centers_yx, const int32_t* n_centers,
                                    const uint8_t* is_thing,
@@ -1352,29 +1506,49 @@
                                    uint32_t* votes, int votes_are_zero, int vote_rows_hint,
                                    nmsa_stream_t stream_)
 {
+    return panoptic_fused_impl(logits, logits_dtype, offset, centers_yx, n_centers, is_thing, B, C, H, W,
+                               max_centers, scale_y, scale_x, use_dist_thr, dist_thr, sem_u8, inst,
+                               fg_out, score, votes, votes_are_zero, vote_rows_hint,
+                               (hipStream_t)stream_, nullptr, nullptr);
+}
+
+extern "C" size_t nmsa_panoptic_fused_ce_slab_bytes(int B, int H, int W)
+{
+    if (bad_dims(B, H, W)) return 0;
+    return (size_t)B * fused_ce_blocks_per_image(H, W) * sizeof(LossPartial);
+}
+
+extern "C" int nmsa_panoptic_fused_ce(const void* logits, int logits_dtype, const float* offset,
+                                      const int32_t* centers_yx, const int32_t* n_centers,
+                                      const uint8_t* is_thing,
+                                      int B, int C, int H, int W, int max_centers,
+                                      float scale_y, float scale_x,
+                                      int use_dist_thr, float dist_thr,
+                                      uint8_t* sem_u8, uint8_t* inst, uint8_t* fg_out,
+                                      uint32_t* votes, int votes_are_zero, int vote_rows_hint,
+                                      const uint8_t* ce_labels, const float* ce_weights,
+                                      void* ce_slab, size_t ce_slab_bytes,
+                                      double* ce_loss_sum, double* ce_weight_sum,
+                                      int64_t* ce_n_elements, float* ce_means, int32_t* status,
+                                      nmsa_stream_t stream_)
+{
     hipStream_t stream = (hipStream_t)stream_;
-    if (!logits || !offset || !centers_yx || !n_centers || !is_thing || !sem_u8 || !inst || !votes)
-        return NMSA_ERR_ARG;
-    if (bad_dims(B, H, W) || C <= 0 || C > 256 || max_centers <= 0) return NMSA_ERR_ARG;
-    if (!votes_are_zero) {
-        int rc = check_hip(hipMemsetAsync(votes, 0, (size_t)B * 256 * (C + 1) * sizeof(uint32_t), stream));
-        if (rc) return rc;
-    }
-    switch (logits_dtype) {
-        case NMSA_F32:
-            return launch_fused<NMSA_F32>(logits, offset, centers_yx, n_centers, is_thing, B, C, H, W,
-                                          max_centers, scale_y, scale_x, use_dist_thr, dist_thr,
-                                          sem_u8, inst, fg_out, score, votes, vote_rows_hint, stream);
-        case NMSA_BF16:
-            return launch_fused<NMSA_BF16>(logits, offset, centers_yx, n_centers, is_thing, B, C, H, W,
-                                           max_centers, scale_y, scale_x, use_dist_thr, dist_thr,
-                                           sem_u8, inst, fg_out, score, votes, vote_rows_hint, stream);
-        case NMSA_F16:
-            return launch_fused<NMSA_F16>(logits, offset, centers_yx, n_centers, is_thing, B, C, H, W,
-                                          max_centers, scale_y, scale_x, use_dist_thr, dist_thr,
-                                          sem_u8, inst, fg_out, score, votes, vote_rows_hint, stream);
-        default: return NMSA_ERR_ARG;
-    }
+    if (!ce_labels || !ce_slab || !ce_loss_sum || !ce_n_elements || !status) return NMSA_ERR_ARG;
+    if (bad_dims(B, H, W)) return NMSA_ERR_ARG;
+    if (ce_slab_bytes < nmsa_panoptic_fused_ce_slab_bytes(B, H, W)) return NMSA_ERR_WORKSPACE;
+    const FusedCeArgs ce = {ce_labels, ce_weights, (LossPartial*)ce_slab, status};
+    int blocks = 0;
+    int rc = panoptic_fused_impl(logits, logits_dtype, offset, centers_yx, n_centers, is_thing, B, C, H, W,
+                                 max_centers, scale_y, scale_x, use_dist_thr, dist_thr, sem_u8, inst,
+                                 fg_out, nullptr, votes, votes_are_zero, vote_rows_hint, stream, &ce,
+                                 &blocks);
+    if (rc) return rc;
+    rc = loss_finalize((const LossPartial*)ce_slab, blocks, ce_loss_sum, ce_weight_sum,
+                       ce_n_elements, stream);
+    if (rc || !ce_means) return rc;
+    hipLaunchKernelGGL(k_fused_ce_means, dim3(1), dim3(1), 0, stream, ce_loss_sum,
+                       (const long long*)ce_n_elements, ce_means);
+    return check_launch();
 }
 
 extern "C" int nmsa_panoptic_assign(uint32_t* votes, int B, int n_vote_classes, int clear_votes,
diff --git a/nicr_mt_scene_analysis_amd/model/postprocessing/panoptic.py b/nicr_mt_scene_analysis_amd/model/postprocessing/panoptic.py
--- a/nicr_mt_scene_analysis_amd/model/postprocessing/panoptic.py
+++ b/nicr_mt_scene_analysis_amd/model/postprocessing/panoptic.py
@@ -31,6 +31,18 @@
 
 
 _PACK_VIA_DEVICE = os.environ.get('NMSA_PACK_VIA_DEVICE', '0') == '1'
+
+CE_REQUEST_UNUSED_CALLS = 4
+
+
+def tensor_identity(t):
+    if t is None:
+        return None
+    try:
+        return (t.data_ptr(), tuple(t.shape), tuple(t.stride()), t.dtype, t._version)
+    except RuntimeError:
+        return None
+
 
 class PanopticPostprocessing(DensePostprocessingBase):
     def __init__(
@@ -63,10 +75,43 @@
         self._max_instances_per_category = 1 << 16
         self._host_columns = 32
         self._device_luts: Dict[torch.device, Tuple[torch.Tensor, torch.Tensor]] = {}
+        self._ce_request = None
 
     @property
     def max_instances_per_category(self):
         return self._max_instances_per_category
+
+    def request_semantic_ce(self, batch_key: str, weights=None) -> None:
+        req = self._ce_request
+        if req is None or req['key'] != batch_key or req['weights'] is not weights:
+            self._ce_request = {'key': batch_key, 'weights': weights, 'unused': 0}
+
+    def _semantic_ce_inputs(self, s_output, batch):
+        req = self._ce_request
+        if req is None:
+            return None
+        if req['unused'] >= CE_REQUEST_UNUSED_CALLS:
+            self._ce_request = None
+            return None
+        req['unused'] += 1
+        if self._compute_scores or self._instance_postprocessing._heatmap_apply_foreground_mask:
+            return None
+        target, w = batch.get(req['key']), req['weights']
+        if not (isinstance(target, torch.Tensor) and s_output.ndim == 4 and s_output.shape[1] <= 256):
+            return None
+        B, C, H, W = s_output.shape
+        dev = s_output.device
+        if not (target.is_cuda and target.device == dev and target.dtype == torch.uint8 and
+                tuple(target.shape) == (B, H, W) and target.is_contiguous()):
+            return None
+        if w is not None and not (isinstance(w, torch.Tensor) and w.is_cuda and w.device == dev and
+                                  w.dtype == torch.float32 and tuple(w.shape) == (C,) and
+                                  w.is_contiguous()):
+            return None
+        if tensor_identity(s_output) is None or tensor_identity(target) is None or \
+                (w is not None and tensor_identity(w) is None):
+            return None
+        return target, w
 
     def _luts(self, device):
         if device not in self._device_luts:
@@ -97,6 +142,12 @@
         dev = s_output.device
         thing_lut, ori_lut = self._luts(dev)
 
+        ce_in = self._semantic_ce_inputs(s_output, batch)
+        ce_target, ce_weights = ce_in if ce_in is not None else (None, None)
+        ce_ids = None if ce_in is None else {
+            'logits': tensor_identity(s_output), 'target': tensor_identity(ce_target),
+            'weights': tensor_identity(ce_weights), 'key': self._ce_request['key']}
+
         def run(on_centers=None):
             return ops.panoptic_pipeline(
                 s_output, center_heatmap, center_offset, thing_lut,
@@ -109,7 +160,8 @@
                 max_instances_per_category=self._max_instances_per_category,
                 void_label=0, max_centers=post._max_centers,
                 want_score=self._compute_scores, want_foreground=False,
-                want_panoptic_semantic=False, on_centers=on_centers)
+                want_panoptic_semantic=False, on_centers=on_centers,
+                ce_target=ce_target, ce_weights=ce_weights)
         if self._defer_host_sync:
             p = run()
             tables = _HostTables(self._fetch_tables_async(p, post, checked=False))
@@ -138,6 +190,11 @@
                                                    want_score=True)['score'])
         r.set_lazy('semantic_segmentation_idx', lambda: sem_u8.long())
         r.aux['semantic_segmentation_idx'] = sem_u8
+        r.aux['semantic_ce_request'] = self.request_semantic_ce
+        if ce_ids is not None:
+            req = self._ce_request
+            r.aux['semantic_ce'] = dict(ce_ids, sums=p['ce_sums'], means=p['ce_means'],
+                                        used=lambda: req.__setitem__('unused', 0))
         self._semantic_postprocessing._fullres_entries(r, s_output, batch)
 
         r.merge(post._postprocess_inference((i_output, i_side_outputs), batch))
diff --git a/nicr_mt_scene_analysis_amd/ops.py b/nicr_mt_scene_analysis_amd/ops.py
--- a/nicr_mt_scene_analysis_amd/ops.py
+++ b/nicr_mt_scene_analysis_amd/ops.py
@@ -209,6 +209,8 @@
     want_panoptic_semantic: bool = False,
     fused_kernel_events: Optional[list] = None,
     on_centers=None,
+    ce_target: Optional[torch.Tensor] = None,
+    ce_weights: Optional[torch.Tensor] = None,
 ) -> Dict[str, torch.Tensor]:
     lib = L.lib()
     x = L.require_device_tensor(semantic_logits, 'semantic_logits')
@@ -219,6 +221,9 @@
     dev = x.device
     st = L.stream_ptr(dev)
     thing = _u8(is_thing)
+    if ce_target is not None and (want_score or apply_foreground_mask):
+        raise ValueError('ce_target: the fused cross entropy has no score output and does not run '
+                         'behind the foreground-masked center selection')
 
     fg_for_nms = None
     if apply_foreground_mask:
@@ -240,13 +245,26 @@
         ev0 = torch.cuda.Event(enable_timing=True)
         ev1 = torch.cuda.Event(enable_timing=True)
         ev0.record(torch.cuda.current_stream(dev))
-    L.check(lib.nmsa_panoptic_fused(
-        L.ptr(x), L.float_dtype_code(x), L.ptr(off), L.ptr(cen['centers_yx']),
-        L.ptr(cen['n_centers']), L.ptr(thing), B, Cn, H, W, int(max_centers), sy, sx,
-        0 if distance_threshold is None else 1,
-        0.0 if distance_threshold is None else float(distance_threshold),
-        L.ptr(sem_u8), L.ptr(inst), L.ptr(fg), L.ptr(score), L.ptr(votes), 1,
-        int(top_k) + 1, st), 'nmsa_panoptic_fused')
+    ce = None
+    if ce_target is not None:
+        ce = _fused_ce_buffers(ce_target, ce_weights, B, Cn, H, W, dev)
+        L.check(lib.nmsa_panoptic_fused_ce(
+            L.ptr(x), L.float_dtype_code(x), L.ptr(off), L.ptr(cen['centers_yx']),
+            L.ptr(cen['n_centers']), L.ptr(thing), B, Cn, H, W, int(max_centers), sy, sx,
+            0 if distance_threshold is None else 1,
+            0.0 if distance_threshold is None else float(distance_threshold),
+            L.ptr(sem_u8), L.ptr(inst), L.ptr(fg), L.ptr(votes), 1, int(top_k) + 1,
+            L.ptr(ce['target']), L.ptr(ce['weights']), L.ptr(ce['slab']), ce['slab'].numel(),
+            *(L.C.c_void_p(ce['sums'].data_ptr() + 8 * k) for k in range(3)), L.ptr(ce['means']),
+            L.ptr(ce['status']), st), 'nmsa_panoptic_fused_ce')
+    else:
+        L.check(lib.nmsa_panoptic_fused(
+            L.ptr(x), L.float_dtype_code(x), L.ptr(off), L.ptr(cen['centers_yx']),
+            L.ptr(cen['n_centers']), L.ptr(thing), B, Cn, H, W, int(max_centers), sy, sx,
+            0 if distance_threshold is None else 1,
+            0.0 if distance_threshold is None else float(distance_threshold),
+            L.ptr(sem_u8), L.ptr(inst), L.ptr(fg), L.ptr(score), L.ptr(votes), 1,
+            int(top_k) + 1, st), 'nmsa_panoptic_fused')
     if fused_kernel_events is not None:
         ev1.record(torch.cuda.current_stream(dev))
         fused_kernel_events.append((ev0, ev1))
@@ -281,7 +299,28 @@
         'center_scores': cen['scores'], 'area': area,
         'ids_pan': ids_pan, 'ids_ins': ids_ins, 'n_ids': n_ids,
         'pan_of_inst': pan_of_inst,
+        'ce_sums': None if ce is None else (ce['sums'][0], ce['sums'][1], ce['sums'][2:].view(torch.int64)[0]),
+        'ce_means': None if ce is None else ce['means'],
     }
+
+
+def _fused_ce_buffers(target: torch.Tensor, weights: Optional[torch.Tensor], B: int, Cn: int,
+                      H: int, W: int, dev: torch.device) -> dict:
+    from .loss._functional import _status_word
+    if not (target.is_cuda and target.device == dev and target.dtype == torch.uint8 and
+            tuple(target.shape) == (B, H, W) and target.is_contiguous()):
+        raise ValueError(f'ce_target must be a contiguous uint8 [{B}, {H}, {W}] tensor on {dev}; got '
+                         f'{target.dtype} {tuple(target.shape)} on {target.device}')
+    if weights is not None and not (weights.is_cuda and weights.device == dev and
+                                    weights.dtype == torch.float32 and tuple(weights.shape) == (Cn,)
+                                    and weights.is_contiguous()):
+        raise ValueError(f'ce_weights must be a contiguous float32 [{Cn}] tensor on {dev}')
+    nbytes = L.lib().nmsa_panoptic_fused_ce_slab_bytes(B, H, W)
+    return {'target': target, 'weights': weights,
+            'slab': torch.empty((nbytes,), dtype=torch.uint8, device=dev),
+            'sums': torch.empty((3,), dtype=torch.float64, device=dev),
+            'means': torch.empty((2,), dtype=torch.float32, device=dev),
+            'status': _status_word(dev)}
 
 
 def panoptic_scores(
diff --git a/nicr_mt_scene_analysis_amd/task_helper/semantic.py b/nicr_mt_scene_analysis_amd/task_helper/semantic.py
--- a/nicr_mt_scene_analysis_amd/task_helper/semantic.py
+++ b/nicr_mt_scene_analysis_amd/task_helper/semantic.py
@@ -6,6 +6,8 @@
 from ..loss import check_loss_status
 from ..loss import CrossEntropyLossSemantic
 from ..metric import MeanIntersectionOverUnion
+from ..model.postprocessing.panoptic import tensor_identity
+from .base import PackedLosses
 from .base import TaskHelperBase
 from .base import append_detached_losses_to_logs
 from .base import append_profile_to_logs
@@ -34,11 +36,41 @@
         self._metric_iou = MeanIntersectionOverUnion(n_classes=self._n_classes, device=device)
         self._metric_iou.reset()
 
-    def _compute_losses(self, batch, batch_idx, predictions_post):
+    def _losses_from_fused_pass(self, predictions_post, predictions, targets, scale_names):
+        aux = getattr(predictions_post, 'aux', None)
+        if not aux or len(predictions) != 1 or len(targets) != 1 or self._label_smoothing != 0.0:
+            return None
+        request = aux.get('semantic_ce_request')
+        pred = predictions[0]
+        if request is None or pred is not predictions_post.get(f'{_TASK}_output') or \
+                (torch.is_grad_enabled() and pred.requires_grad):
+            return None
+        weights = self._class_weights
+        request(_TASK, weights)
+        ce = aux.get('semantic_ce')
+        if ce is None or ce['key'] != _TASK or \
+                ce['logits'] != tensor_identity(pred) or ce['target'] != tensor_identity(targets[0]) or \
+                ce['weights'] != tensor_identity(weights) or \
+                (weights is not None and ce['weights'] is None):
+            return None
+        ce['used']()
+        item, total = ce['means'].unbind(0)
+        out = PackedLosses()
+        out.packed = ce['means']
+        out[f'{_TASK}_loss_{scale_names[0]}'] = item
+        out[self.mark_as_total(_TASK)] = total
+        out.index = {f'{_TASK}_loss_{scale_names[0]}': 0, self.mark_as_total(_TASK): 1}
+        return out
+
+    def _compute_losses(self, batch, batch_idx, predictions_post, validation=False):
         side_key = None if self._disable_multiscale_supervision else f'{_TASK}_side_outputs'
         predictions, targets, scale_names = self.collect_predictions_and_targets_for_loss(
             batch=batch, batch_key=_TASK, predictions_post=predictions_post,
             predictions_post_key=f'{_TASK}_output', side_outputs_key=side_key)
+        if validation:
+            fused = self._losses_from_fused_pass(predictions_post, predictions, targets, scale_names)
+            if fused is not None:
+                return fused
         from ..loss import _multi
         items = [{'kind': 'ce', 'pred': p, 'mask': t, 'weights': self._class_weights,
                   'param': self._label_smoothing, 'total': 0} for p, t in zip(predictions, targets)]
@@ -60,7 +92,7 @@
     @append_profile_to_logs(f'{_TASK}_step_time')
     @append_detached_losses_to_logs()
     def validation_step(self, batch, batch_idx, predictions_post):
-        losses = self._compute_losses(batch, batch_idx, predictions_post)
+        losses = self._compute_losses(batch, batch_idx, predictions_post, validation=True)
         key = get_fullres_key(f'{_TASK}_segmentation_idx')
         aux = getattr(predictions_post, 'aux', {})
         self._metric_iou.update_masked_void(aux[key] if key in aux else predictions_post[key],
```

After: 31270 Mpix/s. 1.2% lower.
